# alexrozanski/llama.swift

Hardware: AMD Instinct MI355X
Metric: decode tokens/sec LLaMA-7B Q4_0 @1 GPU; % HBM-roofline on Q4_0 GEMV (higher is better)
Workload: dtype q4_0 x q4_0 -> int32 block sums, fp32 scales/accumulate; 1 GPU; LLaMA-7B Q4_0 single-token decode, greedy, n_ctx 512: `value` = 94 timed tokens at context positions 13 .. 106 (after 8 prompt + 5 warm-up tokens); BASELINE.json configs[1] proper -- the generation to the end of the 512-token context -- is config.full_context_tokens_per_s / roofline.full_context_* of bench.py --full; n_threads_semantics=8, parallelism=1 GPU

## Files before the change

llama.swift_amd/csrc/decode.hip:

```cpp
#define LH_DEFINE_PHASE_PROBE 1
#include <cmath>

#include "kcommon.hip.h"

namespace lh {

#ifndef LH_GEMV_SADDR
#define LH_GEMV_SADDR 0
#endif
#ifndef LH_GEMV_PAD
#define LH_GEMV_PAD 1
#endif

__device__ __forceinline__ float poll_tagged(const uint64_t *p, uint32_t tag, uint32_t *fault, bool short_fuse ) {
    uint64_t v;
    int spins = 0;
    for (;;) {
        v = __hip_atomic_load(p, __ATOMIC_RELAXED, __HIP_MEMORY_SCOPE_AGENT);
        if ((uint32_t) (v >> 32) == tag) break;
        __builtin_amdgcn_s_sleep(1);
        if (poll_give_up(spins, short_fuse ? (1 << 8) : (1 << 20), fault)) break;
    }
    return __builtin_bit_cast(float, (uint32_t) v);
}
__device__ __forceinline__ void store_tagged(uint64_t *p, float v, uint32_t tag) {
    __hip_atomic_store(p, (uint64_t) __builtin_bit_cast(uint32_t, v) | ((uint64_t) tag << 32), __ATOMIC_RELAXED, __HIP_MEMORY_SCOPE_WORKGROUP);
}


struct GemvArgs {
    const uint8_t *wt; int ngroups, nchunks, M, gmapF8;
    const uint32_t *qa_A; const float *qa_d;
    const float *in0, *in1; int K;
    float *y; const float *resid;
    const uint16_t *T_silu;
    uint32_t *out_A; float *out_d;
    const f64x2 *part_in; int npart; f64x2 *part_out;
    uint32_t *sync; int sync_blocks, sync_epoch;
    int lut_math;
    uint32_t *fault;
    const uint64_t *in_t;   int slot_in;
    const uint64_t *resid_t; int slot_resid;
    uint64_t *out_t;        int slot_out;
    const int32_t *pos_w;
    PickIO pick;
    int patience;
};
template <int PRE, int EPI, int D, bool RING, int PG>
__device__ __forceinline__ void gemv_body(const GemvArgs &ga, const int blk, const int nw, double *smem_d) {
    const uint8_t *__restrict__ wt = ga.wt;
    const int ngroups = ga.ngroups, nchunks = ga.nchunks, M = ga.M, gmapF8 = ga.gmapF8, K = ga.K, npart = ga.npart;
    const uint32_t *__restrict__ qa_A = ga.qa_A; const float *__restrict__ qa_d = ga.qa_d;
    const float *__restrict__ in0 = ga.in0; const float *__restrict__ in1 = ga.in1;
    float *__restrict__ y = ga.y; const float *__restrict__ resid = ga.resid;
    const uint16_t *__restrict__ T_silu = ga.T_silu;
    uint32_t *__restrict__ out_A = ga.out_A; float *__restrict__ out_d = ga.out_d;
    const f64x2 *__restrict__ part_in = ga.part_in; f64x2 *__restrict__ part_out = ga.part_out;
    constexpr bool TAGGED = (EPI == EPI_STORE_TAG || PRE == PREP_NORM_TAG || EPI == EPI_RESID_TAG || EPI == EPI_SILU_QAH);
    const uint32_t epoch_ = TAGGED ? __builtin_nontemporal_load(ga.sync) : 0u;
    const uint32_t store_tag = make_tag(epoch_, ga.sync_epoch + 1);
    const uint32_t mb_epoch_ = ((PRE == PREP_NORM_TAG || EPI == EPI_RESID_TAG) && ga.pos_w) ? (uint32_t) __builtin_nontemporal_load(ga.pos_w) + 1u : epoch_;
    const uint32_t tag_in = make_tag(mb_epoch_, ga.slot_in), tag_resid = make_tag(mb_epoch_, ga.slot_resid), tag_out = make_tag(mb_epoch_, ga.slot_out);
    uint32_t *ldsA = (uint32_t *) smem_d;
    constexpr int PADC = (LH_GEMV_PAD && RING) ? D : 0;
    float *ldsD = (float *) (ldsA + (nchunks + PADC) * 64);
    const int tid = threadIdx.x, lane = tid & 63, wave = LH_GEMV_SADDR ? __builtin_amdgcn_readfirstlane(tid >> 6) : (tid >> 6);
    constexpr bool active = true;
    const int qah_block = (blk >> 4) * 8 + (blk & 7), qah_half = (blk >> 3) & 1;
    const int g = EPI == EPI_SILU_QAH ? qah_block * 8 + (wave >> 1) * 4 + qah_half * 2 + (wave & 1) : blk * nw + wave;
    const bool valid = active && g < ngroups;
    const uint8_t *wbase = wt + (size_t) (valid ? g : 0) * (nchunks + 1) * TILE_BYTES;
    const uint32_t voff_w = (uint32_t) lane * 16u, voff_s = 1024u + (uint32_t) ((lane >> 3) * 8 + (lane & 3) * 2) * 4u;
    uint32_t vw_ = voff_w, vs_ = voff_s;
#define LH_OPAQUE_OFFSETS() { vw_ = voff_w; vs_ = voff_s; asm volatile("" : "+v"(vw_), "+v"(vs_)); }
#if LH_PHASE_PROBE == 3
    unsigned long long probe_t[5] = { 0, 0, 0, 0, 0 };
    const unsigned long long probe_wall = wall_clock64();
#elif LH_PHASE_PROBE
    unsigned long long *probe_e = nullptr;
    if (g_phase_probe && blk == (int) gridDim.x / 2 && threadIdx.x == 0) {
        unsigned long long *pb = g_phase_probe;
        const unsigned long long slot = atomicAdd(pb, 1ull);
        if (slot < pb[1]) { probe_e = pb + 8 * (1 + slot); probe_e[5] = ngroups; probe_e[6] = nchunks; probe_e[7] = PRE * 16 + EPI; }
    }
#endif
    LH_STAMP(0);

    u32x4 wq[D];
    f32x2 ws[D];
#define LH_LOADW(SLOT, CH)                                                                                   \
    {                                                                                                        \
        const int ch_ = min((CH), nchunks);         \
        const uint8_t *tp_ = wbase + (size_t) ch_ * TILE_BYTES;                                              \
        if (LH_GEMV_SADDR) {                                                                                 \
            wq[SLOT] = __builtin_nontemporal_load((const u32x4 *) (tp_ + (size_t) vw_));                     \
            ws[SLOT] = __builtin_nontemporal_load((const f32x2 *) (tp_ + (size_t) vs_));                     \
        } else {                                                                                             \
            wq[SLOT] = __builtin_nontemporal_load((const u32x4 *) (tp_ + lane * 16));                        \
            ws[SLOT] = __builtin_nontemporal_load((const f32x2 *) (tp_ + 1024 + ((lane >> 3) * 8 + (lane & 3) * 2) * 4)); \
        }                                                                                                    \
    }
    constexpr bool NORMTAG = (PRE == PREP_NORM_TAG);
    constexpr bool NORMLIKE = (PRE == PREP_NORM || PRE == PREP_NORMP || NORMTAG);
    constexpr bool REGPRE = (PRE == PRE_QA || NORMLIKE || PRE == PREP_PLAIN);
    constexpr int MAXH = (NORMLIKE || PRE == PREP_PLAIN) ? PG : 1;
    constexpr int MAXQA = (PRE == PRE_QA) ? PG : 1, MAXQD = (PG + 7) / 8;
    f32x4 xa[MAXH][4], xb[MAXH][4];
    u32x4 qg[MAXQA], qh[MAXQD];
    const int nt = nw * 64;
    const int nh = K >> 4;
    constexpr int PNP = (PRE == PREP_NORMP) ? 8 : 1;
    f64x2 pp[PNP];
    const int npl = (npart + 63) >> 6;
    float resid_v = 0.0f;
    uint64_t resid_g = 0;
    auto phase1 = [&]() {
    if ((NORMLIKE || PRE == PREP_PLAIN) && active) {
        const int ng = (nh + nt - 1) / nt;
#pragma unroll
        for (int u = 0; u < MAXH; u++) {
            if (u < ng && (tid & ~63) + u * nt < nh) {
                const int hi = min(tid + u * nt, nh - 1);
#pragma unroll
                for (int v = 0; v < 4; v++) {
                    if (!NORMTAG) xa[u][v] = ((const f32x4 *) in0)[hi * 4 + v];
                    if (NORMLIKE) xb[u][v] = ((const f32x4 *) in1)[hi * 4 + v];
                }
            } else {
#pragma unroll
                for (int v = 0; v < 4; v++) { xa[u][v] = f32x4{ 0.0f, 0.0f, 0.0f, 0.0f }; xb[u][v] = f32x4{ 0.0f, 0.0f, 0.0f, 0.0f }; }
            }
        }
        if (PRE == PREP_NORMP && wave == 0) {
#pragma unroll
            for (int u = 0; u < PNP; u++) if (u < npl) pp[u] = part_in[min(lane + u * 64, npart - 1)];
        }
    }
    if ((EPI == EPI_RESID || (EPI == EPI_RESID_TAG && !ga.resid_t)) && active) {
        int lg0 = g;
        if (gmapF8) { const int b8 = g >> 3, w8 = g & 7; lg0 = w8 < 4 ? b8 * 4 + w8 : gmapF8 + b8 * 4 + (w8 - 4); }
        resid_v = resid[min(lg0 * 8 + (lane >> 3), M - 1)];
    }
    if (EPI == EPI_RESID_TAG && ga.resid_t && active && (lane & 7) == 0) {
        int lg0 = g;
        if (gmapF8) { const int b8 = g >> 3, w8 = g & 7; lg0 = w8 < 4 ? b8 * 4 + w8 : gmapF8 + b8 * 4 + (w8 - 4); }
        resid_g = load_granule_sys(ga.resid_t + min(lg0 * 8 + (lane >> 3), M - 1));
    }
    if (PRE == PRE_QA && active) {
        const int nqa = (nchunks * 16 + nt - 1) / nt, nqd = (nchunks * 2 + nt - 1) / nt;
#pragma unroll
        for (int u = 0; u < MAXQA; u++) if (u < nqa) qg[u] = ((const u32x4 *) qa_A)[min(tid + u * nt, nchunks * 16 - 1)];
#pragma unroll
        for (int u = 0; u < MAXQD; u++) if (u < nqd) qh[u] = ((const u32x4 *) qa_d)[min(tid + u * nt, nchunks * 2 - 1)];
    }
    };
    phase1();
    __builtin_amdgcn_sched_barrier(0);
    if (active) {
#pragma unroll
        for (int i = 0; i < D; i++) LH_LOADW(i, i)
    }
    __builtin_amdgcn_sched_barrier(0);

    if (NORMTAG) {
        const uint64_t *__restrict__ xt = ga.in_t;
        const int give_up = (ga.lut_math & 0x1000) ? (1 << 8) : ((1 << 20) << ga.patience);
        if (wave == 0) {
            int spins = 0;
            for (;;) {
                bool ok = true;
                if (lane < LH_WATCH) ok = (uint32_t) (load_granule_sys(xt + ((2 * lane + 1) * K / (2 * LH_WATCH))) >> 32) == tag_in;
                if (__all(ok)) break;
                __builtin_amdgcn_s_sleep(8);
                if (++spins > (give_up >> 2) || ((spins & 255) == 0 && __hip_atomic_load(ga.fault, __ATOMIC_RELAXED, __HIP_MEMORY_SCOPE_SYSTEM) != 0u)) break;
            }
        }
        __syncthreads();
#pragma unroll
        for (int u = 0; u < MAXH; u++) {
            const int hi = tid + u * nt;
            if (active && hi < nh) {
                uint64_t gv[16];
                int spins = 0;
                for (;;) {
                    bool ok = true;
#pragma unroll
                    for (int i = 0; i < 16; i++) {
                        gv[i] = load_granule_sys(xt + hi * 16 + i);
                        ok = ok && (uint32_t) (gv[i] >> 32) == tag_in;
                    }
                    if (ok) break;
                    __builtin_amdgcn_s_sleep(1);
                    if (poll_give_up(spins, give_up, ga.fault)) break;
                }
#pragma unroll
                for (int v = 0; v < 4; v++)
                    xa[u][v] = f32x4{ __builtin_bit_cast(float, (uint32_t) gv[4 * v]), __builtin_bit_cast(float, (uint32_t) gv[4 * v + 1]),
                                      __builtin_bit_cast(float, (uint32_t) gv[4 * v + 2]), __builtin_bit_cast(float, (uint32_t) gv[4 * v + 3]) };
            } else {
#pragma unroll
                for (int v = 0; v < 4; v++) xa[u][v] = f32x4{ 0.0f, 0.0f, 0.0f, 0.0f };
            }
        }
    }

    LH_STAMP(1);
    double *red = (double *) (ldsD + (nchunks + PADC) * 8);
    for (int i = active ? tid : PADC * 72; i < PADC * 72; i += nt) {
        if (i < PADC * 64) ldsA[nchunks * 64 + i] = 0u;
        else ldsD[nchunks * 8 + (i - PADC * 64)] = 0.0f;
    }
    if (PRE == PRE_QA) {
#pragma unroll
        for (int u = 0; u < MAXQA; u++) { const int gi = tid + u * nt; if (active && gi < nchunks * 16) ((u32x4 *) ldsA)[gi] = qg[u]; }
#pragma unroll
        for (int u = 0; u < MAXQD; u++) { const int gi = tid + u * nt; if (active && gi < nchunks * 2) ((u32x4 *) ldsD)[gi] = qh[u]; }
        __syncthreads();
    } else if (REGPRE) {
        if (NORMLIKE) {
            double S1 = 0.0, S2 = 0.0;
            if (PRE == PREP_NORMP) {
                if (wave == 0) {
#pragma unroll
                    for (int u = 0; u < PNP; u++)
                        if (u < npl && lane + u * 64 < npart) { S1 += pp[u].x; S2 += pp[u].y; }
                    S1 = wave_sum_d(S1);
                    S2 = wave_sum_d(S2);
                    if (lane == 0) { red[0] = S1; red[1] = S2; }
                }
                __syncthreads();
                S1 = red[0]; S2 = red[1];
            } else {
#pragma unroll
                for (int u = 0; u < MAXH; u++)
                    if (active && tid + u * nt < nh) {
#pragma unroll
                        for (int v = 0; v < 4; v++) {
                            const double x0 = (double) xa[u][v].x, x1 = (double) xa[u][v].y, x2 = (double) xa[u][v].z, x3 = (double) xa[u][v].w;
                            S1 += x0; S1 += x1; S1 += x2; S1 += x3;
                            S2 = __builtin_fma(x0, x0, S2); S2 = __builtin_fma(x1, x1, S2); S2 = __builtin_fma(x2, x2, S2); S2 = __builtin_fma(x3, x3, S2);
                        }
                    }
                block_sum_d2(S1, S2, red, 0);
            }
            const double mean = S1 / (double) K;
            double sum2 = __builtin_fma(-mean, S1, S2);
            const bool fast = npart >= 0 && mean * S1 <= 0.25 * S2;
            LH_STAMP2(2);
            double s2 = 0.0;
#pragma unroll
            for (int u = 0; u < MAXH; u++)
                if (active && tid + u * nt < nh) {
#pragma unroll
                    for (int v = 0; v < 4; v++) {
                        const double v0 = (double) xa[u][v].x - mean, v1 = (double) xa[u][v].y - mean;
                        const double v2 = (double) xa[u][v].z - mean, v3 = (double) xa[u][v].w - mean;
                        xa[u][v].x = (float) v0; xa[u][v].y = (float) v1; xa[u][v].z = (float) v2; xa[u][v].w = (float) v3;
                        if (!fast) { s2 += v0 * v0; s2 += v1 * v1; s2 += v2 * v2; s2 += v3 * v3; }
                    }
                }
            if (!fast) sum2 = block_sum_d(s2, red, 1);
            const float scale = (float) (1.0 / sqrt(sum2 / (double) K + (double) 1e-5f));
            LH_STAMP2(3);
#pragma unroll
            for (int u = 0; u < MAXH; u++)
#pragma unroll
                for (int v = 0; v < 4; v++) {
                    xa[u][v].x = xb[u][v].x * (xa[u][v].x * scale); xa[u][v].y = xb[u][v].y * (xa[u][v].y * scale);
                    xa[u][v].z = xb[u][v].z * (xa[u][v].z * scale); xa[u][v].w = xb[u][v].w * (xa[u][v].w * scale);
                }
        }
        const int nbp = nchunks * 8;
#pragma unroll
        for (int u = 0; u < MAXH; u++) {
            const int hi = tid + u * nt;
            const bool live = active && hi < nh;
            float amax = 0.0f;
            if (live) {
#pragma unroll
                for (int v = 0; v < 4; v++)
                    amax = fmaxf(fmaxf(fmaxf(amax, fabsf(xa[u][v].x)), fabsf(xa[u][v].y)), fmaxf(fabsf(xa[u][v].z), fabsf(xa[u][v].w)));
            }
            amax = fmaxf(amax, dpp_f<DPP_QUAD_XOR1>(amax));
            const float dd = amax / 7.0f;
            const float id = (amax != 0.0f) ? 7.0f / amax : 0.0f;
            uint32_t pr[8];
#pragma unroll
            for (int v = 0; v < 4; v++) {
                const uint32_t n0 = (uint32_t) ((int) __builtin_rintf(xa[u][v].x * id)) & 0xF, n1 = (uint32_t) ((int) __builtin_rintf(xa[u][v].y * id)) & 0xF;
                const uint32_t n2 = (uint32_t) ((int) __builtin_rintf(xa[u][v].z * id)) & 0xF, n3 = (uint32_t) ((int) __builtin_rintf(xa[u][v].w * id)) & 0xF;
                pr[2 * v] = n0 | (n1 << 8);
                pr[2 * v + 1] = n2 | (n3 << 8);
            }
            const int half = hi & 1, b = hi >> 1, c = b >> 3, j = b & 7;
#pragma unroll
            for (int k = 0; k < 8; k++) {
                const uint32_t other = (uint32_t) __builtin_amdgcn_mov_dpp((int) pr[k], DPP_QUAD_XOR1, 0xF, 0xF, true);
                const uint32_t dw = (half ? (other | (pr[k] << 16)) : (pr[k] | (other << 16))) << (4 * (j & 1));
                if (live && (k >> 2) == half) ldsA[(c * 8 + k) * 8 + j] = dw;
            }
            if (live && half == 0) ldsD[b] = dd;
        }
        for (int b = active ? K / 32 + tid : nbp; b < nbp; b += nt) {
            const int c = b >> 3, j = b & 7;
#pragma unroll
            for (int k = 0; k < 8; k++) ldsA[(c * 8 + k) * 8 + j] = 0;
            ldsD[b] = 0.0f;
        }
        __syncthreads();
    } else {
        float *ybuf = (float *) (red + 32);
        make_y<PRE>(ybuf, red, in0, in1, K, T_silu);
        quantize_y(ybuf, K, nchunks * 256, ldsA, ldsD, nullptr);
        __syncthreads();
    }

    const int k = lane & 7;
    float acc = 0.0f;
    static_assert(D % 2 == 0, "the two-entry LDS operand buffer alternates by slot parity: ring depth must be even");
    u32x4 la0[2], la1[2];
    float ldl[2], ldh[2];
    const int tq = lane & 3;
#define LH_LDSLOAD(BUF, CH)                                                                        \
    {                                                                                              \
        const int cl_ = PADC ? (CH) : min((CH), nchunks - 1);                                      \
        const u32x4 *pa = (const u32x4 *) (ldsA + (cl_ * 8 + k) * 8);                              \
        la0[BUF] = pa[0]; la1[BUF] = pa[1];                                                        \
        ldl[BUF] = ldsD[cl_ * 8 + tq]; ldh[BUF] = ldsD[cl_ * 8 + 4 + tq];                          \
    }
#define LH_CONSUME(SLOT, CH)                                                                       \
    {                                                                                              \
        const u32x4 w = wq[SLOT];                                                                  \
        const f32x2 sw = ws[SLOT];                                                                 \
        const u32x4 a0 = la0[(SLOT) & 1], a1 = la1[(SLOT) & 1];                                    \
        const float plo_ = sw.x * ldl[(SLOT) & 1], phi_ = sw.y * ldh[(SLOT) & 1];                  \
        LH_LDSLOAD(((SLOT) + 1) & 1, (CH) + 1)                                                     \
         \
         \
         \
         \
        const int i0_ = __builtin_amdgcn_sdot8((int) w.x, (int) a0.x, 0x4B400000, true);           \
        const int i1_ = __builtin_amdgcn_sdot8((int) w.x, (int) a0.y, 0x4B400000, true);           \
        const int i2_ = __builtin_amdgcn_sdot8((int) w.y, (int) a0.z, 0x4B400000, true);           \
        const int i3_ = __builtin_amdgcn_sdot8((int) w.y, (int) a0.w, 0x4B400000, true);           \
        const int i4_ = __builtin_amdgcn_sdot8((int) w.z, (int) a1.x, 0x4B400000, true);           \
        const int i5_ = __builtin_amdgcn_sdot8((int) w.z, (int) a1.y, 0x4B400000, true);           \
        const int i6_ = __builtin_amdgcn_sdot8((int) w.w, (int) a1.z, 0x4B400000, true);           \
        const int i7_ = __builtin_amdgcn_sdot8((int) w.w, (int) a1.w, 0x4B400000, true);           \
        const f32x2 mg_ = { 12582912.0f, 12582912.0f };                                            \
        const f32x2 q01_ = f32x2{ __builtin_bit_cast(float, i0_), __builtin_bit_cast(float, i1_) } - mg_; \
        const f32x2 q23_ = f32x2{ __builtin_bit_cast(float, i2_), __builtin_bit_cast(float, i3_) } - mg_; \
        const f32x2 q45_ = f32x2{ __builtin_bit_cast(float, i4_), __builtin_bit_cast(float, i5_) } - mg_; \
        const f32x2 q67_ = f32x2{ __builtin_bit_cast(float, i6_), __builtin_bit_cast(float, i7_) } - mg_; \
        LH_FMAC8_DPP(acc, plo_, phi_, q01_, q23_, q45_, q67_);                                     \
    }
    LH_STAMP(2);
    LH_STAMP2(4);
    if (active) {
    LH_LDSLOAD(0, 0)
    int c0 = 0;
    if (RING) {
        do {
            if (LH_GEMV_SADDR) LH_OPAQUE_OFFSETS()
#pragma unroll
            for (int i = 0; i < D; i++) {
                LH_CONSUME(i, c0 + i)
                LH_LOADW(i, c0 + D + i)
                __builtin_amdgcn_sched_barrier(0);
            }
            c0 += D;
        } while (c0 + D < nchunks);
    }
#pragma unroll
    for (int i = 0; i < D; i++) {
        LH_CONSUME(i, c0 + i)
        __builtin_amdgcn_sched_barrier(0);
    }
    }
#undef LH_LDSLOAD
#undef LH_CONSUME
#undef LH_LOADW
#undef LH_OPAQUE_OFFSETS

    LH_STAMP(3);
    acc = fold8(acc);
    int lg = g;
    if (gmapF8) { const int b8 = g >> 3, w8 = g & 7; lg = w8 < 4 ? b8 * 4 + w8 : gmapF8 + b8 * 4 + (w8 - 4); }
    const int m = lg * 8 + (lane >> 3);
    if (EPI == EPI_SILU_QAH) {
        float *gu = (float *) red;
        __syncthreads();
        if (k == 0) gu[wave * 8 + (lane >> 3)] = acc;
        __syncthreads();
        if (wave == 0 && valid) {
            const int i = lane & 15;
            const uint16_t gh = f2h_bits(gu[i]);
            const float act = h2f_bits((ga.lut_math & 1) ? silu_math_bits(gh) : T_silu[gh]) * gu[16 + i];
            float amax = wave_max_f(lane < 16 ? fabsf(act) : 0.0f);
            uint64_t *at = (uint64_t *) ga.out_t;
            const int hb = qah_block * 2 + qah_half;
            float other = 0.0f;
            if (lane == 0) {
                store_tagged(at + hb, amax, store_tag ^ ((ga.lut_math & 0x1000) ? 1u : 0u));
                other = poll_tagged(at + (hb ^ 1), store_tag, ga.fault, (ga.lut_math & 0x1000) != 0);
            }
            other = __builtin_bit_cast(float, __builtin_amdgcn_readfirstlane(__builtin_bit_cast(int, other)));
            amax = fmaxf(amax, other);
            const float dd = amax / 7.0f;
            const float id = (amax != 0.0f) ? 7.0f / amax : 0.0f;
            const uint32_t nib = (uint32_t) ((int) __builtin_rintf(act * id)) & 0xF;
            const int kk = lane & 7;
            const uint32_t e0 = __shfl(nib, 2 * kk), e1 = __shfl(nib, 2 * kk + 1);
            const int b = qah_block, c = b >> 3, j = b & 7;
            if (lane < 8) ((uint16_t *) (out_A + (c * 8 + kk) * 8 + j))[qah_half] = (uint16_t) ((e0 | (e1 << 8)) << (4 * (j & 1)));
            if (lane == 0 && qah_half == 0) out_d[b] = dd;
        }
    } else
    if (EPI == EPI_SILU_QA) {
        float *gu = (float *) red;
        __syncthreads();
        if (k == 0) gu[wave * 8 + (lane >> 3)] = acc;
        __syncthreads();
        if (wave == 0) {
            const int i = lane & 31;
            const uint16_t gh = f2h_bits(gu[i]);
            const float act = h2f_bits((ga.lut_math & 1) ? silu_math_bits(gh) : T_silu[gh]) * gu[32 + i];
            float amax = fabsf(act);
            amax = max_lanes_0_31(amax);
            const float dd = amax / 7.0f;
            const float id = (amax != 0.0f) ? 7.0f / amax : 0.0f;
            const uint32_t nib = ((uint32_t) ((int) __builtin_rintf(act * id) + 8) - 8) & 0xF;
            const int kk = lane & 7;
            const uint32_t e0 = __shfl(nib, 2 * kk), e1 = __shfl(nib, 2 * kk + 1);
            const uint32_t e2 = __shfl(nib, 16 + 2 * kk), e3 = __shfl(nib, 17 + 2 * kk);
            const int b = blk, c = b >> 3, j = b & 7;
            const uint32_t dw = (e0 | (e1 << 8) | (e2 << 16) | (e3 << 24)) << (4 * (j & 1));
            {
                if (lane < 8) out_A[(c * 8 + kk) * 8 + j] = dw;
                if (lane == 0) out_d[b] = dd;
            }
            if (y && lane < 32) y[b * 32 + i] = act;
        }
    } else {
        const bool live = valid && k == 0 && m < M;
        if (EPI == EPI_RESID) acc = acc + resid_v;
        if (EPI == EPI_RESID_TAG) {
            float rv = resid_v;
            if (ga.resid_t) {
                rv = __builtin_bit_cast(float, (uint32_t) resid_g);
                if (live && (uint32_t) (resid_g >> 32) != tag_resid) {
                    int spins = 0;
                    uint64_t gq;
                    for (;;) {
                        gq = load_granule_sys(ga.resid_t + m);
                        if ((uint32_t) (gq >> 32) == tag_resid) break;
                        __builtin_amdgcn_s_sleep(4);
                        if (poll_give_up(spins, (ga.lut_math & 0x1000) ? (1 << 8) : ((1 << 20) << ga.patience), ga.fault)) break;
                    }
                    rv = __builtin_bit_cast(float, (uint32_t) gq);
                }
            }
            acc = acc + rv;
        }
        if (EPI == EPI_STORE_PICK) {
            if (live) y[m] = acc;
            unsigned long long key = 0ull;
            if (live && acc == acc) {
                const uint32_t b = __builtin_bit_cast(uint32_t, acc == 0.0f ? 0.0f : acc);
                const uint32_t ob = (b & 0x80000000u) ? ~b : (b | 0x80000000u);
                key = ((unsigned long long) ob << 32) | (unsigned long long) (0xFFFFFFFFu - (uint32_t) m);
            }
#pragma unroll
            for (int o = 32; o >= 1; o >>= 1) {
                const uint32_t lo_ = (uint32_t) __shfl_xor((int) (uint32_t) key, o), hi_ = (uint32_t) __shfl_xor((int) (uint32_t) (key >> 32), o);
                const unsigned long long ok = ((unsigned long long) hi_ << 32) | lo_;
                key = ok > key ? ok : key;
            }
            unsigned long long *wk = (unsigned long long *) red;
            __syncthreads();
            if (lane == 0) wk[wave] = key;
            __syncthreads();
            if (tid == 0) {
                unsigned long long k2 = wk[0];
                for (int w2_ = 1; w2_ < nw; w2_++) k2 = wk[w2_] > k2 ? wk[w2_] : k2;
                __hip_atomic_store(ga.pick.key + blk, k2, __ATOMIC_RELAXED, __HIP_MEMORY_SCOPE_AGENT);
                asm volatile("s_waitcnt vmcnt(0)" ::: "memory");
                const int nwg = (int) gridDim.x, shard = blk & 7, nsh = (nwg + 7 - shard) / 8, ntop = nwg < 8 ? nwg : 8;
                int lastwg = 0;
                if (atomicAdd(ga.pick.count + shard * 16, 1u) == (uint32_t) (nsh - 1))
                    lastwg = atomicAdd(ga.pick.count + 128, 1u) == (uint32_t) (ntop - 1);
                wk[15] = (unsigned long long) lastwg;
            }
            __syncthreads();
            if (wk[15] != 0ull) {
                unsigned long long best = 0ull;
                for (int i = tid; i < (int) gridDim.x; i += nw * 64) {
                    const unsigned long long kv = __hip_atomic_load(ga.pick.key + i, __ATOMIC_RELAXED, __HIP_MEMORY_SCOPE_AGENT);
                    best = kv > best ? kv : best;
                }
#pragma unroll
                for (int o = 32; o >= 1; o >>= 1) {
                    const uint32_t lo_ = (uint32_t) __shfl_xor((int) (uint32_t) best, o), hi_ = (uint32_t) __shfl_xor((int) (uint32_t) (best >> 32), o);
                    const unsigned long long ok = ((unsigned long long) hi_ << 32) | lo_;
                    best = ok > best ? ok : best;
                }
                __syncthreads();
                if (lane == 0) wk[wave] = best;
                __syncthreads();
                if (tid == 0) {
                    unsigned long long fin = wk[0];
                    for (int w2_ = 1; w2_ < nw; w2_++) fin = wk[w2_] > fin ? wk[w2_] : fin;
                    const int r = (fin >> 32) == 0ull ? 0 : (int) (0xFFFFFFFFu - (uint32_t) fin);
                    int32_t *st = ga.pick.state;
                    ga.pick.out[st[1]] = r;
                    if (ga.pick.next_token) *ga.pick.next_token = r;
                    st[0] += 1; st[1] += 1;
                    for (int sh = 0; sh < 8; sh++) __hip_atomic_store(ga.pick.count + sh * 16, 0u, __ATOMIC_RELAXED, __HIP_MEMORY_SCOPE_AGENT);
                    __hip_atomic_store(ga.pick.count + 128, 0u, __ATOMIC_RELAXED, __HIP_MEMORY_SCOPE_AGENT);
                    wk[14] = (unsigned long long) (r < ga.pick.n_vocab ? r : 0);
                }
                __syncthreads();
            }
            if (wk[15] != 0ull && ga.pick.emb) {
                const int tok = (int) wk[14];
                const int dE = K;
                __syncthreads();
                const uint8_t *row = ga.pick.emb + (size_t) tok * (dE / 32) * 20;
                double s1 = 0.0, s2 = 0.0;
                for (int i = tid; i < dE / 2; i += nw * 64) {
                    const int b = i >> 4, j = i & 15;
                    const uint8_t *blk_ = row + b * 20;
                    const uint32_t bits = blk_[0] | (blk_[1] << 8) | (blk_[2] << 16) | ((uint32_t) blk_[3] << 24);
                    const float dd = __builtin_bit_cast(float, bits);
                    const uint32_t q = blk_[4 + j];
                    const float v0 = (float) ((int) (q & 0xF) - 8) * dd, v1 = (float) ((int) (q >> 4) - 8) * dd;
                    ga.pick.x_next[2 * i + 0] = v0;
                    ga.pick.x_next[2 * i + 1] = v1;
                    s1 += (double) v0; s1 += (double) v1;
                    s2 += (double) v0 * (double) v0; s2 += (double) v1 * (double) v1;
                }
                s1 = block_sum_d(s1, red, 0);
                s2 = block_sum_d(s2, red, 1);
                if (tid == 0) {
                    ((f64x2 *) ga.pick.part_next)[0] = f64x2{ s1, s2 };
                    if (ga.pick.epoch) ga.pick.epoch[0] = next_epoch(ga.pick.epoch[0]);
                }
            }
        } else
        if (EPI == EPI_STORE_TAG) {
            if (live) store_tagged((uint64_t *) y + m, acc, store_tag ^ ((ga.lut_math & 0x1000) ? 1u : 0u));
        } else if (EPI == EPI_RESID_TAG) {
            if (live) {
                if (ga.out_t) store_tagged_sys(ga.out_t + m, __builtin_bit_cast(uint32_t, acc), tag_out ^ ((ga.lut_math & 0x2000) ? 1u : 0u));
                if (y) y[m] = acc;
            }
        } else
        if (live) y[m] = acc;
        if ((EPI == EPI_RESID || EPI == EPI_RESID_TAG) && part_out) {
            const double yd = live ? (double) acc : 0.0;
            const double s1 = wave_sum_d(yd), s2 = wave_sum_d(yd * yd);
            if (nw == 1) {
                if (lane == 0) part_out[blk] = f64x2{ s1, s2 };
            } else {
                if (lane == 0) { red[2 * wave] = s1; red[2 * wave + 1] = s2; }
                __syncthreads();
                if (tid == 0) {
                    double t1 = red[0], t2 = red[1];
                    for (int w2_ = 1; w2_ < nw; w2_++) { t1 += red[2 * w2_]; t2 += red[2 * w2_ + 1]; }
                    part_out[blk] = f64x2{ t1, t2 };
                }
            }
        }
    }
    LH_STAMP(4);
#if LH_PHASE_PROBE == 3
    if (g_phase_probe && threadIdx.x == 0) {
        unsigned long long *pb = g_phase_probe;
        const unsigned long long slot = atomicAdd(pb, 1ull);
        if (slot < pb[1]) {
            unsigned long long *e = pb + 8 * (1 + slot);
            for (int i = 0; i < 5; i++) e[i] = probe_t[i];
            e[5] = ((unsigned long long) (PRE * 16 + EPI) << 48) | ((unsigned long long) nchunks << 32) | (unsigned) blk;
            e[6] = wall_clock64();
            e[7] = probe_wall;
        }
    }
#endif
}


template <int PRE, int EPI, int D, bool RING, int PG>
__global__ void __launch_bounds__(EPI == EPI_SILU_QA ? 512 : 256, EPI == EPI_SILU_QA ? 4 : 1)
k_gemv(const GemvArgs ga) {
    extern __shared__ double smem_d[];
    gemv_body<PRE, EPI, D, RING, PG>(ga, blockIdx.x, blockDim.x >> 6, smem_d);
}


constexpr int DEC_TS = 32;

__global__ void __launch_bounds__(256)
k_dec_scores(const float *__restrict__ qkv, int d, int dh, const double *__restrict__ sincos_tab,
             float *__restrict__ Kc, float *__restrict__ Vc, float *__restrict__ sc, int n_ctx,
             float kq_scale, const int32_t *__restrict__ st) {
    extern __shared__ double smem_d[];
    float *qs = (float *) smem_d;
    float *kn = qs + dh;
    const int h = blockIdx.x;
#if LH_PHASE_PROBE == 3
    const unsigned long long probe_wall = wall_clock64(), probe_t0 = __builtin_readcyclecounter();
    unsigned long long probe_t1 = 0, probe_t2 = 0;
#endif
    const int n_past = st[0];
    const int t0 = blockIdx.y * DEC_TS;
    if (t0 > n_past) return;
    const int tid = threadIdx.x;
    const bool owns_new = n_past < t0 + DEC_TS;
    const double *tab = sincos_tab + (size_t) n_past * dh;
    const float *q = qkv + h * dh, *kk = qkv + d + h * dh, *vv = qkv + 2 * d + h * dh;
    const bool rot = tid < dh / 2;
    const int e = rot ? 2 * tid : 0;
    const double cs = tab[e], sn = tab[e + 1];
    const float q0 = q[e], q1 = q[e + 1];
    const float kr0 = kk[e], kr1 = kk[e + 1], vr0 = vv[e], vr1 = vv[e + 1];
    const int hw = tid >> 5, l = tid & 31;
    constexpr int KPH = DEC_TS / 8;
    const int tb = t0 + hw * KPH;
    float kv[KPH][8];
#pragma unroll
    for (int u = 0; u < KPH; u++) {
        const int t = min(tb + u, n_past);
        const float *kr = Kc + (size_t) t * d + h * dh;
#pragma unroll
        for (int i = 0; i < 8; i++) kv[u][i] = (i * 32 < dh) ? kr[min(i * 32, dh - 32) + l] : 0.0f;
    }
    if (rot) {
        const double x0 = (double) q0, x1 = (double) q1;
        qs[e] = (float) (x0 * cs - x1 * sn);
        qs[e + 1] = (float) (x0 * sn + x1 * cs);
        if (owns_new) {
            const double k0 = (double) kr0, k1 = (double) kr1;
            const float r0 = (float) (k0 * cs - k1 * sn), r1 = (float) (k0 * sn + k1 * cs);
            kn[e] = r0; kn[e + 1] = r1;
            Kc[(size_t) n_past * d + h * dh + e] = r0;
            Kc[(size_t) n_past * d + h * dh + e + 1] = r1;
            Vc[(size_t) n_past * d + h * dh + e] = vr0;
            Vc[(size_t) n_past * d + h * dh + e + 1] = vr1;
        }
    }
    __syncthreads();
#if LH_PHASE_PROBE == 3
    probe_t1 = __builtin_readcyclecounter();
#endif
#pragma unroll
    for (int u = 0; u < KPH; u++) {
        const int t = tb + u;
        float s = 0.0f;
#pragma unroll
        for (int i = 0; i < 8; i++) {
            if (i * 32 < dh) {
                const float kval = (t == n_past) ? kn[i * 32 + l] : kv[u][i];
                s = fmaf(kval, qs[i * 32 + l], s);
            }
        }
        s = tree32_to_lane0(s);
        if (l == 0 && t <= n_past) sc[(size_t) h * n_ctx + t] = s * kq_scale;
    }
#if LH_PHASE_PROBE == 3
    probe_t2 = __builtin_readcyclecounter();
    if (g_phase_probe && tid == 0) {
        unsigned long long *pb = g_phase_probe; const unsigned long long slot = atomicAdd(pb, 1ull);
        if (slot < pb[1]) { unsigned long long *e = pb + 8 * (1 + slot); e[0] = probe_t0; e[1] = probe_t1; e[2] = probe_t2; e[3] = e[4] = probe_t2;
            e[5] = (0xB2ull << 48) | ((unsigned long long) blockIdx.y << 32) | (unsigned) h; e[6] = wall_clock64(); e[7] = probe_wall; }
    }
#endif
}

__global__ void __launch_bounds__(256)
k_decn_scores(const float *__restrict__ qr, int d, int dh, const float *__restrict__ Kc, float *__restrict__ sc,
              int n_ctx, float kq_scale, int n_past, const SeqSet *__restrict__ set) {
    const int h = blockIdx.x, n = blockIdx.z, H = gridDim.x;
    const int np = set ? set->state[n][0] : n_past + n;
    if (set) Kc += set->kv_off[n];
    const int t0 = blockIdx.y * DEC_TS;
    if (t0 > np) return;
    const int tid = threadIdx.x, hw = tid >> 5, l = tid & 31;
    constexpr int KPH = DEC_TS / 8;
    const int tb = t0 + hw * KPH;
    const float *q = qr + (size_t) n * d + h * dh;
    float qv[8], kv[KPH][8];
#pragma unroll
    for (int i = 0; i < 8; i++) qv[i] = (i * 32 < dh) ? q[min(i * 32, dh - 32) + l] : 0.0f;
#pragma unroll
    for (int u = 0; u < KPH; u++) {
        const float *kr = Kc + (size_t) min(tb + u, np) * d + h * dh;
#pragma unroll
        for (int i = 0; i < 8; i++) kv[u][i] = (i * 32 < dh) ? kr[min(i * 32, dh - 32) + l] : 0.0f;
    }
#pragma unroll
    for (int u = 0; u < KPH; u++) {
        const int t = tb + u;
        float s = 0.0f;
#pragma unroll
        for (int i = 0; i < 8; i++)
            if (i * 32 < dh) s = fmaf(kv[u][i], qv[i], s);
        s = tree32_to_lane0(s);
        if (l == 0 && t <= np) sc[((size_t) n * H + h) * n_ctx + t] = s * kq_scale;
    }
}

template <bool MULTI>
__global__ void __launch_bounds__(1024)
k_dec_pv_blk(const float *__restrict__ sc, const float *__restrict__ Vc, int d, int dh, int n_ctx, int nth,
             float *__restrict__ merged, uint32_t *__restrict__ qa_A, float *__restrict__ qa_d,
             const uint16_t *__restrict__ T_exp, const int32_t *__restrict__ st,
             int n_past0, long qa_strideA, long qa_strideD, int lut_math, int chunk, const SeqSet *__restrict__ set, long m_stride) {
    extern __shared__ double smem_d[];
    double *red = smem_d;
    float *p = (float *) (smem_d + 32);
    float *part = p + n_ctx;
    const int h = blockIdx.x, cb = blockIdx.y, tid = threadIdx.x, nt = blockDim.x;
    const int n_past = MULTI ? (set ? set->state[blockIdx.z][0] : n_past0 + (int) blockIdx.z) : st[0];
    if (MULTI && set) Vc += set->kv_off[blockIdx.z];
    const int T = n_past + 1;
    const float *row = sc + (size_t) h * n_ctx;
    if (MULTI) {
        const int n = blockIdx.z;
        row = sc + ((size_t) n * gridDim.x + h) * n_ctx;
        if (merged) merged += (size_t) n * m_stride;
        qa_A += (size_t) n * qa_strideA;
        qa_d += (size_t) n * qa_strideD;
        if (h == (int) gridDim.x - 1 && cb == (int) gridDim.y - 1)
            for (int pb = d / 32 + tid; pb < (int) qa_strideD; pb += nt) {
                const int pc = pb >> 3, pj = pb & 7;
#pragma unroll
                for (int kk = 0; kk < 8; kk++) qa_A[(pc * 8 + kk) * 8 + pj] = 0;
                qa_d[pb] = 0.0f;
            }
    }
    pv_soft_max(row, p, T, tid, nt, red, T_exp, lut_math);
    const int Tpv = (MULTI && !set) ? (chunk > 0 ? n_past0 + min((int) gridDim.z, ((int) blockIdx.z / chunk + 1) * chunk) : n_past0 + (int) gridDim.z) : T;
    if (MULTI && !set)
        for (int t = T + tid; t < Tpv; t += nt) p[t] = 0.0f;
    __syncthreads();

    const int c = tid & 31, sub = tid >> 5, nsub = nt >> 5;
    const int dc = (Tpv + nth - 1) / nth;
    const int col = h * dh + cb * 32 + c;
    const float *vcol = Vc + col;
    for (int th = sub; th < nth; th += nsub) {
        const int t0 = dc * th, t1 = min(t0 + dc, Tpv);
        float acc = 0.0f;
        float va[16], vb[16];
#pragma unroll
        for (int u = 0; u < 16; u++) va[u] = vcol[(size_t) min(t0 + u, t1 - 1) * d];
        for (int tb = t0; tb < t1; tb += 32) {
#pragma unroll
            for (int u = 0; u < 16; u++) vb[u] = vcol[(size_t) min(tb + 16 + u, t1 - 1) * d];
#pragma unroll
            for (int u = 0; u < 16; u++) {
                const float pe = (tb + u < t1) ? p[min(tb + u, Tpv - 1)] : 0.0f;
                acc = fmaf(va[u], pe, acc);
            }
#pragma unroll
            for (int u = 0; u < 16; u++) va[u] = vcol[(size_t) min(tb + 32 + u, t1 - 1) * d];
#pragma unroll
            for (int u = 0; u < 16; u++) {
                const float pe = (tb + 16 + u < t1) ? p[min(tb + 16 + u, Tpv - 1)] : 0.0f;
                acc = fmaf(vb[u], pe, acc);
            }
        }
        part[th * 32 + c] = acc;
    }
    __syncthreads();
    pv_store_block(part, nth, tid, col, h, dh, cb, merged, qa_A, qa_d);
}

template <int NL>
__global__ void __launch_bounds__(1024)
k_dec_pv_stream(const float *__restrict__ sc, const float *__restrict__ Vc, int d, int dh, int n_ctx, int nth, int SR,
                float *__restrict__ merged, uint32_t *__restrict__ qa_A, float *__restrict__ qa_d,
                const uint16_t *__restrict__ T_exp, const int32_t *__restrict__ st, int lut_math,
                int H, int split, uint64_t *__restrict__ xpart, const uint32_t *__restrict__ epoch, int layer, uint32_t *__restrict__ fault) {
    typedef float f32x4 __attribute__((ext_vector_type(4)));
    extern __shared__ double smem_d[];
    double *red = smem_d;
    float *p = (float *) (smem_d + 32);
    float *part = p + ((n_ctx + 3) & ~3);
    f32x4 *stage = (f32x4 *) (part + nth * 32);
    const int tid = threadIdx.x;
#if LH_PHASE_PROBE == 3
    unsigned long long probe_t[10] = { 0, 0, 0, 0, 0, 0, 0, 0, 0, 0 };
    const unsigned long long probe_wall = wall_clock64();
#define LH_PSTAMP(IDX) do { probe_t[IDX] = __builtin_readcyclecounter(); } while (0)
#define LH_PFLUSH() do { if (g_phase_probe && tid == 0) { unsigned long long *pb = g_phase_probe; const unsigned long long wall_ = wall_clock64(); \
        for (int half_ = 0; half_ < 2; half_++) { const unsigned long long slot = atomicAdd(pb, 1ull); \
        if (slot < pb[1]) { unsigned long long *e = pb + 8 * (1 + slot); for (int i = 0; i < 5; i++) e[i] = probe_t[5 * half_ + i]; \
            e[5] = ((unsigned long long) (0xB0 + half_) << 48) | ((unsigned long long) z << 32) | (unsigned) base; e[6] = wall_; e[7] = probe_wall; } } } } while (0)
#else
#define LH_PSTAMP(IDX) do { } while (0)
#define LH_PFLUSH() do { } while (0)
#endif
    const int bid = blockIdx.x, z = (bid >> 3) % split, base = (bid / (8 * split)) * 8 + (bid & 7);
    const int h = base % H, cb = base / H;
    const int cpw = (nth + split - 1) / split, th_lo = z * cpw, nloc = min(nth, th_lo + cpw) - th_lo;
    LH_PSTAMP(0);
    const int T = st[0] + 1;
    const int dc = (T + nth - 1) / nth;
    const int nstage = (dc + SR - 1) / SR;
    const int col0 = h * dh + cb * 32;
    const int stage_quads = nloc * SR * 8;
    constexpr int PV_ROW = 4;
    const float *row = sc + (size_t) h * n_ctx;
    float rv[PV_ROW];
#pragma unroll
    for (int i = 0; i < PV_ROW; i++) rv[i] = row[min(i * 1024 + tid, T - 1)];
    auto fetch = [&](int sidx, f32x4 (&v)[NL]) {
#pragma unroll
        for (int i = 0; i < NL; i++) {
            const int e = min(i * 1024 + tid, stage_quads - 1);
            const int r = e >> 3, q = e & 7;
            const int lc = r / SR, u = r - lc * SR, th = th_lo + lc;
            const int t = min(min(dc * th + sidx * SR + u, dc * th + dc - 1), T - 1);
            v[i] = __builtin_nontemporal_load((const f32x4 *) (Vc + (size_t) t * d + col0 + q * 4));
        }
    };
    auto put = [&](int buf, const f32x4 (&v)[NL]) {
#pragma unroll
        for (int i = 0; i < NL; i++) {
            const int e = i * 1024 + tid;
            if (e < stage_quads) stage[(size_t) buf * stage_quads + e] = v[i];
        }
    };
    f32x4 va[NL], vb[NL];
    {
        float mx = -INFINITY;
#pragma unroll
        for (int i = 0; i < PV_ROW; i++) if (i * 1024 + tid < T) mx = fmaxf(mx, rv[i]);
        mx = block_max_f(mx, red, 0);
        LH_PSTAMP(1);
        fetch(0, va);
        if (nstage > 1) fetch(1, vb);
        double sum = 0.0;
#pragma unroll
        for (int i = 0; i < PV_ROW; i++) {
            if (i * 1024 + tid < T) {
                const uint16_t xh = f2h_bits(rv[i] - mx);
                rv[i] = h2f_bits((lut_math & 2) ? exp_math_bits(xh) : T_exp[xh]);
                sum += (double) rv[i];
            }
        }
        sum = block_sum_d(sum, red, 1);
        const float inv = (float) (1.0 / sum);
#pragma unroll
        for (int i = 0; i < PV_ROW; i++) if (i * 1024 + tid < T) p[i * 1024 + tid] = rv[i] * inv;
    }
    LH_PSTAMP(2);
    const int lc = tid >> 5, c = tid & 31, th = th_lo + lc;
    const bool owner = lc < nloc;
    const int t0 = dc * th, t1 = min(t0 + dc, T);
    float acc = 0.0f;
    auto consume = [&](int sidx, int buf) {
        if (!owner) return;
        const float *vs = (const float *) (stage + (size_t) buf * stage_quads) + (size_t) lc * SR * 32 + c;
        const int tb = t0 + sidx * SR, n = min(SR, t1 - tb);
        int u = 0;
        for (; u + 16 <= n; u += 16) {
            float v[16], w[16];
#pragma unroll
            for (int k = 0; k < 16; k++) { v[k] = vs[(u + k) * 32]; w[k] = p[tb + u + k]; }
#pragma unroll
            for (int k = 0; k < 16; k++) acc = fmaf(v[k], w[k], acc);
        }
        for (; u < n; u++) acc = fmaf(vs[u * 32], p[tb + u], acc);
    };
    for (int sidx = 0; sidx < nstage; sidx += 2) {
        put(0, va);
        __syncthreads();
        if (sidx == 0) LH_PSTAMP(3); else if (sidx == 2) LH_PSTAMP(7);
        if (sidx + 2 < nstage) fetch(sidx + 2, va);
        consume(sidx, 0);
        if (sidx == 0) LH_PSTAMP(4);
        if (sidx + 1 < nstage) {
            put(1, vb);
            __syncthreads();
            if (sidx == 0) LH_PSTAMP(5);
            if (sidx + 3 < nstage) fetch(sidx + 3, vb);
            consume(sidx + 1, 1);
            if (sidx == 0) LH_PSTAMP(6);
        }
    }
    LH_PSTAMP(8);
    if (z + 1 < split) {
        if (owner) store_tagged(xpart + ((size_t) base * nth + th) * 32 + c, acc, make_tag(epoch[0], layer + 1) ^ ((lut_math & 0x1000) ? 1u : 0u));
        LH_PSTAMP(9);
        LH_PFLUSH();
        return;
    }
    if (owner) part[th * 32 + c] = acc;
    if (split > 1 && tid < th_lo * 32)
        part[tid] = poll_tagged(xpart + (size_t) base * nth * 32 + tid, make_tag(epoch[0], layer + 1), fault, (lut_math & 0x1000) != 0);
    __syncthreads();
    pv_store_block(part, nth, tid, col0 + tid, h, dh, cb, merged, qa_A, qa_d);
    LH_PSTAMP(9);
    LH_PFLUSH();
}
#undef LH_PSTAMP
#undef LH_PFLUSH

#ifndef LH_PVD_ABLATE
#define LH_PVD_ABLATE 0
#endif
constexpr int PVD_SR = 8;
template <int N> __device__ __forceinline__ void pvd_wait_vmcnt() { asm volatile("s_waitcnt vmcnt(%0)" :: "n"(N) : "memory"); }
__device__ __forceinline__ void pvd_barrier() {
    asm volatile("s_waitcnt lgkmcnt(0)\n\ts_barrier" ::: "memory");
}
__device__ __forceinline__ void pvd_worker_barrier(uint32_t *ctr, uint32_t &round, int lane, uint32_t *fault) {
    round += 6;
    if (lane == 0) __hip_atomic_fetch_add(ctr, 1u, __ATOMIC_RELEASE, __HIP_MEMORY_SCOPE_WORKGROUP);
    int spins = 0;
    while (__hip_atomic_load(ctr, __ATOMIC_ACQUIRE, __HIP_MEMORY_SCOPE_WORKGROUP) < round) { __builtin_amdgcn_s_sleep(0); if (poll_give_up(spins, 1 << 24, fault)) break; }
}
__global__ void __launch_bounds__(512)
k_dec_pv_dma(const float *__restrict__ sc, const float *__restrict__ Vc, int d, int n_ctx, int nth, int NS,
             float *__restrict__ merged, uint32_t *__restrict__ qa_A, float *__restrict__ qa_d,
             const uint16_t *__restrict__ T_exp, const int32_t *__restrict__ st, int lut_math,
             int H, int split, uint64_t *__restrict__ xpart, const uint32_t *__restrict__ epoch, int layer, uint32_t *__restrict__ fault) {
    constexpr int dh = 128;
    extern __shared__ double smem_d[];
    double *red = smem_d;
    float *p = (float *) (smem_d + 32);
    float *part = p + ((n_ctx + 3) & ~3);
    uint32_t *flags = (uint32_t *) (part + nth * dh);
    float *ring = (float *) (flags + 16);
    const int tid = threadIdx.x, lane = tid & 63, wave = __builtin_amdgcn_readfirstlane(tid >> 6);
    const int bid = blockIdx.x, z = (bid >> 3) % split, h = (bid / (8 * split)) * 8 + (bid & 7);
    const int cpw = (nth + split - 1) / split, th_lo = z * cpw, nloc = min(nth, th_lo + cpw) - th_lo;
    const int T = st[0] + 1;
    const int dc = (T + nth - 1) / nth;
    const int nstage = (dc + PVD_SR - 1) / PVD_SR;
    const int col0 = h * dh;
    const int ncw = 2 * nloc;
    const int limit = (lut_math & 0x1000) ? (1 << 8) : (1 << 22);
    if (tid < 16) flags[tid] = 0u;
    constexpr int PV_ROW = 11, NWT = 384;
    const float *row = sc + (size_t) h * n_ctx;
    float rv[PV_ROW];
    const int wt = tid - 128;
    float mx = -INFINITY;
    if (wave > 1) {
#pragma unroll
        for (int i = 0; i < PV_ROW; i++) rv[i] = row[min(i * NWT + wt, T - 1)];
#pragma unroll
        for (int i = 0; i < PV_ROW; i++) if (i * NWT + wt < T) mx = fmaxf(mx, rv[i]);
        mx = wave_max_f(mx);
        if (lane == 0) ((float *) red)[wave] = mx;
    }
    pvd_barrier();
    if (wave < 2) {
        const uint32_t ring_lds = (uint32_t) (uintptr_t) (__attribute__((address_space(3))) float *) ring;
        const uint64_t vbase = (uint64_t) (uintptr_t) (Vc + col0);
        const int u = lane >> 5, q = lane & 31;
        uint32_t off[3];
#pragma unroll
        for (int j = 0; j < 3; j++) off[j] = (uint32_t) ((size_t) min(dc * (th_lo + min(j, nloc - 1)) + 2 * wave + u, n_ctx - 1) * d * 4 + q * 16);
        const uint32_t step = (uint32_t) ((size_t) PVD_SR * d * 4), four = (uint32_t) ((size_t) 4 * d * 4);
        const uint32_t off_max = (uint32_t) ((size_t) (n_ctx - 1) * d * 4 + q * 16);
        uint32_t pub = 0;
        int slot = 0;
        auto min_done = [&]() { uint32_t m = 0xffffffffu; for (int w = 0; w < ncw; w++) m = min(m, __hip_atomic_load(flags + 2 + w, __ATOMIC_ACQUIRE, __HIP_MEMORY_SCOPE_WORKGROUP)); return m; };
        const int F = 60 / (2 * nloc);
        for (int s = 0; s < nstage; s++) {
            if (s >= NS && min_done() < (uint32_t) (s - NS + 1)) {
                pvd_wait_vmcnt<0>();
                if ((uint32_t) s > pub) { pub = (uint32_t) s; __hip_atomic_store(flags + wave, pub, __ATOMIC_RELEASE, __HIP_MEMORY_SCOPE_WORKGROUP); }
                int spins = 0;
                while (min_done() < (uint32_t) (s - NS + 1)) { __builtin_amdgcn_s_sleep(1); if (poll_give_up(spins, limit, fault)) break; }
            }
            const bool tail = (s + 2) * PVD_SR + dc * nth > n_ctx;
#pragma unroll
            for (int j = 0; j < 3; j++) {
                if (j < nloc) {
#pragma unroll
                    for (int i = 0; i < 2; i++) {
                        const uint32_t o = off[j] + (i ? four : 0u);
                        const uint32_t voff = tail ? min(o, off_max) : o;
                        const uint32_t dst = ring_lds + (uint32_t) ((slot * nloc + j) * 4096 + (wave + 2 * i) * 1024);
                        uint32_t keep;
                        asm volatile("s_mov_b32 %0, m0\n\ts_mov_b32 m0, %2\n\ts_nop 0\n\tglobal_load_lds_dwordx4 %1, %3 nt\n\ts_mov_b32 m0, %0"
                                     : "=&s"(keep) : "v"(voff), "s"(dst), "s"(vbase) : "memory");
                    }
                    off[j] += step;
                }
            }
            slot = slot + 1 == NS ? 0 : slot + 1;
            if (s + 1 > F) {
                if (nloc == 1) pvd_wait_vmcnt<60>(); else if (nloc == 2) pvd_wait_vmcnt<60>(); else pvd_wait_vmcnt<60>();
                if ((uint32_t) (s + 1 - F) > pub) { pub = (uint32_t) (s + 1 - F); __hip_atomic_store(flags + wave, pub, __ATOMIC_RELEASE, __HIP_MEMORY_SCOPE_WORKGROUP); }
            }
        }
        pvd_wait_vmcnt<0>();
        __hip_atomic_store(flags + wave, (uint32_t) nstage, __ATOMIC_RELEASE, __HIP_MEMORY_SCOPE_WORKGROUP);
        return;
    }
    uint32_t wround = 0;
    {
        float m2 = ((float *) red)[2];
        for (int w = 3; w < 8; w++) m2 = fmaxf(m2, ((float *) red)[w]);
        double sum = 0.0;
#pragma unroll
        for (int i = 0; i < PV_ROW; i++) {
#if LH_PVD_ABLATE == 1
            if (i * NWT + wt < T && (i * NWT + wt < dc * th_lo || i * NWT + wt >= dc * (th_lo + nloc))) rv[i] = 0.0f; else
#endif
            if (i * NWT + wt < T) {
                const uint16_t xh = f2h_bits(rv[i] - m2);
                rv[i] = h2f_bits((lut_math & 2) ? exp_math_bits(xh) : T_exp[xh]);
                sum += (double) rv[i];
            }
        }
        sum = wave_sum_d(sum);
        if (lane == 0) red[8 + wave] = sum;
    }
    pvd_worker_barrier(flags + 8, wround, lane, fault);
    float acc = 0.0f;
    const int lc = (tid - 128) >> 7, c = (tid - 128) & 127, th = th_lo + lc;
    const bool owner = lc < nloc;
    {
        double tot = red[10];
        for (int w = 3; w < 8; w++) tot += red[8 + w];
        const float inv = (float) (1.0 / tot);
#pragma unroll
        for (int i = 0; i < PV_ROW; i++) if (i * NWT + wt < T) p[i * NWT + wt] = rv[i] * inv;
    }
    pvd_worker_barrier(flags + 8, wround, lane, fault);
    if (wave - 2 < ncw) {
        const int t0 = dc * th, t1 = min(t0 + dc, T);
        uint32_t landed_seen = 0;
        int slot = 0;
        for (int s = 0; s < nstage; s++) {
            if ((uint32_t) s >= landed_seen) {
                int spins = 0;
                for (;;) {
                    landed_seen = min(__hip_atomic_load(flags, __ATOMIC_ACQUIRE, __HIP_MEMORY_SCOPE_WORKGROUP), __hip_atomic_load(flags + 1, __ATOMIC_ACQUIRE, __HIP_MEMORY_SCOPE_WORKGROUP));
                    if (landed_seen > (uint32_t) s) break;
                    __builtin_amdgcn_s_sleep(1);
                    if (poll_give_up(spins, limit, fault)) break;
                }
            }
            {
                const float *vs = ring + (size_t) (slot * nloc + lc) * 1024 + c;
                const int tb = t0 + s * PVD_SR, n = min(PVD_SR, t1 - tb);
                if (n == PVD_SR) {
                    float v[PVD_SR], w[PVD_SR];
#pragma unroll
                    for (int k = 0; k < PVD_SR; k++) { v[k] = vs[k * dh]; w[k] = p[tb + k]; }
#pragma unroll
                    for (int k = 0; k < PVD_SR; k++) acc = fmaf(v[k], w[k], acc);
                } else {
                    for (int k = 0; k < n; k++) acc = fmaf(vs[k * dh], p[tb + k], acc);
                }
            }
            asm volatile("" ::: "memory");
            if (lane == 0) __hip_atomic_store(flags + wave, (uint32_t) (s + 1), __ATOMIC_RELEASE, __HIP_MEMORY_SCOPE_WORKGROUP);
            slot = slot + 1 == NS ? 0 : slot + 1;
        }
    }
    const uint32_t ptag = make_tag(epoch[0], layer + 1);
    if (z + 1 < split) {
        if (owner) store_tagged(xpart + ((size_t) h * nth + th) * dh + c, acc, ptag ^ ((lut_math & 0x1000) ? 1u : 0u));
        return;
    }
    if (owner) part[th * dh + c] = acc;
    for (int i = wt; i < th_lo * dh; i += NWT)
        part[i] = poll_tagged(xpart + (size_t) h * nth * dh + i, ptag, fault, (lut_math & 0x1000) != 0);
    pvd_worker_barrier(flags + 8, wround, lane, fault);
    if (wave >= 2 && wave < 6 && lane < 32) {
        const int cb = wave - 2, cc0 = cb * 32 + lane;
        float s_ = part[cc0];
        for (int t2 = 1; t2 < nth; t2++) s_ += part[t2 * dh + cc0];
        if (merged) merged[col0 + cc0] = s_;
        float amax = fabsf(s_);
        amax = max_lanes_0_31(amax);
        const float dd = amax / 7.0f;
        const float id = (amax != 0.0f) ? 7.0f / amax : 0.0f;
        const uint32_t nib = (uint32_t) ((int) __builtin_rintf(s_ * id)) & 0xF;
        const int kk = lane & 7;
        const uint32_t e0 = __shfl(nib, 2 * kk), e1 = __shfl(nib, 2 * kk + 1);
        const uint32_t e2 = __shfl(nib, 16 + 2 * kk), e3 = __shfl(nib, 17 + 2 * kk);
        const int b = h * (dh / 32) + cb, cc = b >> 3, j = b & 7;
        if (lane < 8) qa_A[(cc * 8 + kk) * 8 + j] = (e0 | (e1 << 8) | (e2 << 16) | (e3 << 24)) << (4 * (j & 1));
        if (lane == 0) qa_d[b] = dd;
    }
}

__device__ __forceinline__ float load_f32_sc1(const float *p) {
    return __builtin_bit_cast(float, __hip_atomic_load((const uint32_t *) p, __ATOMIC_RELAXED, __HIP_MEMORY_SCOPE_AGENT));
}

#ifndef LH_ATTN_ABLATE
#define LH_ATTN_ABLATE 0
#endif
struct AttnXArgs {
    const float *qkv; int d, dh; const double *sincos_tab; float *Kc, *Vc, *sc; int n_ctx, nth; float kq_scale;
    float *merged; uint32_t *qa_A; float *qa_d; const uint16_t *T_exp; const int32_t *st; uint32_t *sync, *fault; int lut_math;
    const uint64_t *qkv2; uint64_t *sc2; const uint32_t *epoch; int layer;
};
template <bool QKV_WAIT>
__device__ __forceinline__ void attn_x_body(const AttnXArgs &aa, const int h, const int yy, double *smem_d) {
    const float *__restrict__ qkv = aa.qkv; const int d = aa.d, dh = aa.dh; const double *__restrict__ sincos_tab = aa.sincos_tab;
    float *__restrict__ Kc = aa.Kc, *__restrict__ Vc = aa.Vc; float *sc = aa.sc; const int n_ctx = aa.n_ctx, nth = aa.nth; const float kq_scale = aa.kq_scale;
    float *__restrict__ merged = aa.merged; uint32_t *__restrict__ qa_A = aa.qa_A; float *__restrict__ qa_d = aa.qa_d;
    const uint16_t *__restrict__ T_exp = aa.T_exp; const int32_t *__restrict__ st = aa.st; uint32_t *sync = aa.sync, *fault = aa.fault; const int lut_math = aa.lut_math;
    const int ncb = dh / 32, tid = threadIdx.x;
#if LH_PHASE_PROBE == 3
    unsigned long long probe_t[5] = { 0, 0, 0, 0, 0 };
    const unsigned long long probe_wall = wall_clock64();
#define LH_ASTAMP(IDX) do { probe_t[IDX] = __builtin_readcyclecounter(); } while (0)
#define LH_AFLUSH(KIND) do { if (g_phase_probe && tid == 0) { unsigned long long *pb = g_phase_probe; const unsigned long long slot = atomicAdd(pb, 1ull); \
        if (slot < pb[1]) { unsigned long long *e = pb + 8 * (1 + slot); for (int i = 0; i < 5; i++) e[i] = probe_t[i]; \
            e[5] = ((unsigned long long) (KIND) << 48) | ((unsigned long long) yy << 32) | (unsigned) h; e[6] = wall_clock64(); e[7] = probe_wall; } } } while (0)
#else
#define LH_ASTAMP(IDX) do { } while (0)
#define LH_AFLUSH(KIND) do { } while (0)
#endif
    LH_ASTAMP(0);
    const int n_past = st[0];
    uint32_t *cnt = sync + h * 32;
    if (yy >= ncb) {
        const int t0 = (yy - ncb) * DEC_TS;
        if (t0 > n_past) return;
        float *qs = (float *) smem_d, *kn = qs + dh;
        const bool owns_new = n_past < t0 + DEC_TS;
        const double *tab = sincos_tab + (size_t) n_past * dh;
        const float *q = qkv + h * dh, *kk = qkv + d + h * dh, *vv = qkv + 2 * d + h * dh;
        const int hw = tid >> 5, l = tid & 31;
        constexpr int KPH = DEC_TS / 8;
        const int tb = t0 + hw * KPH;
        float kv[KPH][8];
        auto load_keys = [&]() {
#pragma unroll
            for (int u = 0; u < KPH; u++) {
                const int t = min(tb + u, n_past);
                const float *kr = Kc + (size_t) t * d + h * dh;
#pragma unroll
                for (int i = 0; i < 8; i++) kv[u][i] = (i * 32 < dh) ? kr[min(i * 32, dh - 32) + l] : 0.0f;
            }
        };
        const bool nowait = (lut_math & 0x1000) != 0;
        const uint32_t tag = QKV_WAIT ? (make_tag(aa.epoch[0], aa.layer + 1)) : 0u;
        if (QKV_WAIT) load_keys();
        if (tid < dh / 2) {
            const int e = 2 * tid;
            const double cs = tab[e], sn = tab[e + 1];
            const uint64_t *q2 = aa.qkv2 + h * dh, *k2 = q2 + d, *v2 = q2 + 2 * d;
            float gq0, gq1, gk0 = 0.0f, gk1 = 0.0f, gv0 = 0.0f, gv1 = 0.0f;
            if (QKV_WAIT) {
                uint64_t g_[6] = { 0, 0, 0, 0, 0, 0 };
                int spins = 0;
                for (;;) {
                    g_[0] = __hip_atomic_load(q2 + e, __ATOMIC_RELAXED, __HIP_MEMORY_SCOPE_AGENT);
                    g_[1] = __hip_atomic_load(q2 + e + 1, __ATOMIC_RELAXED, __HIP_MEMORY_SCOPE_AGENT);
                    if (owns_new) {
                        g_[2] = __hip_atomic_load(k2 + e, __ATOMIC_RELAXED, __HIP_MEMORY_SCOPE_AGENT);
                        g_[3] = __hip_atomic_load(k2 + e + 1, __ATOMIC_RELAXED, __HIP_MEMORY_SCOPE_AGENT);
                        g_[4] = __hip_atomic_load(v2 + e, __ATOMIC_RELAXED, __HIP_MEMORY_SCOPE_AGENT);
                        g_[5] = __hip_atomic_load(v2 + e + 1, __ATOMIC_RELAXED, __HIP_MEMORY_SCOPE_AGENT);
                    }
                    bool ok = (uint32_t) (g_[0] >> 32) == tag && (uint32_t) (g_[1] >> 32) == tag;
                    if (owns_new) ok = ok && (uint32_t) (g_[2] >> 32) == tag && (uint32_t) (g_[3] >> 32) == tag && (uint32_t) (g_[4] >> 32) == tag && (uint32_t) (g_[5] >> 32) == tag;
                    if (ok) break;
                    __builtin_amdgcn_s_sleep(1);
                    if (poll_give_up(spins, nowait ? (1 << 8) : (1 << 20), fault)) break;
                }
                gq0 = __builtin_bit_cast(float, (uint32_t) g_[0]); gq1 = __builtin_bit_cast(float, (uint32_t) g_[1]);
                gk0 = __builtin_bit_cast(float, (uint32_t) g_[2]); gk1 = __builtin_bit_cast(float, (uint32_t) g_[3]);
                gv0 = __builtin_bit_cast(float, (uint32_t) g_[4]); gv1 = __builtin_bit_cast(float, (uint32_t) g_[5]);
            } else {
                gq0 = q[e]; gq1 = q[e + 1];
                if (owns_new) { gk0 = kk[e]; gk1 = kk[e + 1]; gv0 = vv[e]; gv1 = vv[e + 1]; }
            }
            const double x0 = (double) gq0, x1 = (double) gq1;
            qs[e] = (float) (x0 * cs - x1 * sn);
            qs[e + 1] = (float) (x0 * sn + x1 * cs);
            if (owns_new) {
                const double k0 = (double) gk0, k1 = (double) gk1;
                const float r0 = (float) (k0 * cs - k1 * sn), r1 = (float) (k0 * sn + k1 * cs);
                kn[e] = r0; kn[e + 1] = r1;
                Kc[(size_t) n_past * d + h * dh + e] = r0;
                Kc[(size_t) n_past * d + h * dh + e + 1] = r1;
                Vc[(size_t) n_past * d + h * dh + e] = gv0;
                Vc[(size_t) n_past * d + h * dh + e + 1] = gv1;
                if (QKV_WAIT) asm volatile("s_waitcnt vmcnt(0)" ::: "memory");
            }
        }
        __syncthreads();
        LH_ASTAMP(1);
        if (!QKV_WAIT) load_keys();
#pragma unroll
        for (int u = 0; u < KPH; u++) {
            const int t = tb + u;
            float s = 0.0f;
#pragma unroll
            for (int i = 0; i < 8; i++) {
                if (i * 32 < dh) {
                    const float kval = (t == n_past) ? kn[i * 32 + l] : kv[u][i];
                    s = fmaf(kval, qs[i * 32 + l], s);
                }
            }
            s = tree32_to_lane0(s);
            if (l == 0 && t <= n_past) {
                if (QKV_WAIT) store_tagged(aa.sc2 + (size_t) h * n_ctx + t, s * kq_scale, tag);
                else sc[(size_t) h * n_ctx + t] = s * kq_scale;
            }
        }
        if (QKV_WAIT) { LH_ASTAMP(2); LH_ASTAMP(3); LH_ASTAMP(4); LH_AFLUSH(0xA0); return; }
        LH_ASTAMP(2);
        asm volatile("s_waitcnt vmcnt(0)" ::: "memory");
        __syncthreads();
        LH_ASTAMP(3);
        if (tid == 0) __hip_atomic_fetch_add(cnt, 1u, __ATOMIC_RELAXED, __HIP_MEMORY_SCOPE_WORKGROUP);
#if LH_PHASE_PROBE == 3
        asm volatile("s_waitcnt vmcnt(0)" ::: "memory");
#endif
        LH_ASTAMP(4);
        LH_AFLUSH(0xA0);
        return;
    }
    const int cb = yy, nt = 256;
    const int T = n_past + 1;
    const int c = tid & 31, sub = tid >> 5, nsub = nt >> 5;
    const int dc = (T + nth - 1) / nth;
    const int col = h * dh + cb * 32 + c;
    const float *vcol = Vc + col;
    const int ta0 = dc * sub, t10 = min(ta0 + dc, T);
    constexpr int VB = 16;
    const bool early = sub < nth && ta0 < t10 && min(ta0 + 2 * VB - 1, t10 - 1) < n_past;
    float va[VB], vb[VB];
    if (early) {
#pragma unroll
        for (int u = 0; u < VB; u++) va[u] = vcol[(size_t) min(ta0 + u, t10 - 1) * d];
#pragma unroll
        for (int u = 0; u < VB; u++) vb[u] = vcol[(size_t) min(ta0 + VB + u, t10 - 1) * d];
    }
    if (!QKV_WAIT) {
        if (tid == 0) {
            const uint32_t need = (uint32_t) (n_past / DEC_TS + 1);
            int spins = 0;
            while (__hip_atomic_load(cnt, __ATOMIC_RELAXED, __HIP_MEMORY_SCOPE_AGENT) < need) {
                __builtin_amdgcn_s_sleep(1);
                if (++spins > (1 << 20)) { __hip_atomic_store(fault, 1u, __ATOMIC_RELAXED, __HIP_MEMORY_SCOPE_SYSTEM); break; }
            }
        }
        __syncthreads();
    }
    LH_ASTAMP(1);
    double *red = smem_d;
    float *p = (float *) (smem_d + 32);
    float *part = p + n_ctx;
    const float *row = sc + (size_t) h * n_ctx;
    float mx = -INFINITY;
    if (QKV_WAIT) {
        const uint32_t tag = make_tag(aa.epoch[0], aa.layer + 1);
        const bool nowait = (lut_math & 0x1000) != 0;
#if LH_ATTN_ABLATE == 2
        for (int t0 = tid; t0 < T; t0 += nt) p[t0] = 0.0f;
        for (int t0 = T; t0 < T; t0 += 4 * nt) {
#else
        for (int t0 = tid; t0 < T; t0 += 4 * nt) {
#endif
            uint64_t g_[4] = { 0, 0, 0, 0 };
            int spins = 0;
            for (;;) {
                bool ok = true;
#pragma unroll
                for (int i = 0; i < 4; i++) {
                    const int t = t0 + i * nt;
                    if (t < T) { g_[i] = __hip_atomic_load(aa.sc2 + (size_t) h * n_ctx + t, __ATOMIC_RELAXED, __HIP_MEMORY_SCOPE_AGENT); ok = ok && (uint32_t) (g_[i] >> 32) == tag; }
                }
                if (ok) break;
                __builtin_amdgcn_s_sleep(1);
                if (poll_give_up(spins, nowait ? (1 << 8) : (1 << 20), fault)) break;
            }
#pragma unroll
            for (int i = 0; i < 4; i++) {
                const int t = t0 + i * nt;
                if (t < T) { const float v = __builtin_bit_cast(float, (uint32_t) g_[i]); p[t] = v; mx = fmaxf(mx, v); }
            }
        }
    } else
    for (int t = tid; t < T; t += nt) { const float v = load_f32_sc1(row + t); p[t] = v; mx = fmaxf(mx, v); }
#if LH_ATTN_ABLATE == 1 || LH_ATTN_ABLATE == 2
    if (!QKV_WAIT) {
#endif
    mx = block_max_f(mx, red, 0);
    double sum = 0.0;
    for (int t = tid; t < T; t += nt) {
        const uint16_t xh = f2h_bits(p[t] - mx);
        const float e = h2f_bits((lut_math & 2) ? exp_math_bits(xh) : T_exp[xh]);
        p[t] = e;
        sum += (double) e;
    }
    sum = block_sum_d(sum, red, 1);
    const float inv = (float) (1.0 / sum);
    for (int t = tid; t < T; t += nt) p[t] *= inv;
#if LH_ATTN_ABLATE == 1 || LH_ATTN_ABLATE == 2
    }
#endif
    __syncthreads();
    LH_ASTAMP(2);
    for (int th = sub; th < nth; th += nsub) {
        const int ta = dc * th, t1 = min(ta + dc, T);
        float acc = 0.0f;
        if (!(early && th == sub)) {
#pragma unroll
            for (int u = 0; u < VB; u++) va[u] = vcol[(size_t) min(ta + u, t1 - 1) * d];
#pragma unroll
            for (int u = 0; u < VB; u++) vb[u] = vcol[(size_t) min(ta + VB + u, t1 - 1) * d];
        }
        for (int tb = ta; tb < t1; tb += 2 * VB) {
#pragma unroll
            for (int u = 0; u < VB; u++) {
                const float pe = (tb + u < t1) ? p[min(tb + u, T - 1)] : 0.0f;
                acc = fmaf(va[u], pe, acc);
            }
#pragma unroll
            for (int u = 0; u < VB; u++) va[u] = vcol[(size_t) min(tb + 2 * VB + u, t1 - 1) * d];
#pragma unroll
            for (int u = 0; u < VB; u++) {
                const float pe = (tb + VB + u < t1) ? p[min(tb + VB + u, T - 1)] : 0.0f;
                acc = fmaf(vb[u], pe, acc);
            }
#pragma unroll
            for (int u = 0; u < VB; u++) vb[u] = vcol[(size_t) min(tb + 3 * VB + u, t1 - 1) * d];
        }
        part[th * 32 + c] = acc;
    }
    __syncthreads();
    LH_ASTAMP(3);
    if (tid < 32) {
        float s = part[tid];
        for (int th = 1; th < nth; th++) s += part[th * 32 + tid];
        if (merged) merged[col] = s;
        float amax = fabsf(s);
        amax = max_lanes_0_31(amax);
        const float dd = amax / 7.0f;
        const float id = (amax != 0.0f) ? 7.0f / amax : 0.0f;
        const uint32_t nib = (uint32_t) ((int) __builtin_rintf(s * id)) & 0xF;
        const int kk = tid & 7;
        const uint32_t e0 = __shfl(nib, 2 * kk), e1 = __shfl(nib, 2 * kk + 1);
        const uint32_t e2 = __shfl(nib, 16 + 2 * kk), e3 = __shfl(nib, 17 + 2 * kk);
        const int b = h * (dh / 32) + cb, cc = b >> 3, j = b & 7;
        const uint32_t dwq = (e0 | (e1 << 8) | (e2 << 16) | (e3 << 24)) << (4 * (j & 1));
        if (tid < 8) qa_A[(cc * 8 + kk) * 8 + j] = dwq;
        if (tid == 0) qa_d[b] = dd;
    }
    if (!QKV_WAIT && tid == 0) {
        const uint32_t done = __hip_atomic_fetch_add(cnt + 1, 1u, __ATOMIC_RELAXED, __HIP_MEMORY_SCOPE_WORKGROUP);
        if (done == (uint32_t) (ncb - 1)) {
            __hip_atomic_exchange(cnt, 0u, __ATOMIC_RELAXED, __HIP_MEMORY_SCOPE_WORKGROUP);
            __hip_atomic_exchange(cnt + 1, 0u, __ATOMIC_RELAXED, __HIP_MEMORY_SCOPE_WORKGROUP);
        }
    }
    LH_ASTAMP(4);
    LH_AFLUSH(0xA1);
}
#undef LH_ASTAMP
#undef LH_AFLUSH

__global__ void __launch_bounds__(256)
k_dec_attn_x(const AttnXArgs aa) {
    extern __shared__ double smem_d[];
    attn_x_body<false>(aa, blockIdx.x, blockIdx.y, smem_d);
}

template <int PRE, int D, int PG>
__global__ void __launch_bounds__(256) __attribute__((amdgpu_waves_per_eu(PRE == PREP_NORM ? (PG == 1 ? 3 : 2) : (PG == 1 ? 4 : 3))))
k_qkv_attn(const GemvArgs ga, const AttnXArgs aa, const int gridA, const int H) {
    extern __shared__ double smem_d[];
    const int b = blockIdx.x;
    if (b < gridA) {
        const int ncb = aa.dh / 32, wph = 3 * ncb;
        const int xcd = b & 7, slot = b >> 3, j = slot / wph, part = slot % wph, mat = part / ncb, sub = part % ncb;
        const int h = xcd + 8 * j;
        gemv_body<PRE, EPI_STORE_TAG, D, true, PG>(ga, mat * (aa.d / 32) + h * ncb + sub, 4, smem_d);
        return;
    }
    const int a = b - gridA, h = a % H, y = a / H;
    attn_x_body<true>(aa, h, y, smem_d);
}

__global__ void k_xcd_selftest(uint32_t *out) {
    if (threadIdx.x == 0) {
        uint32_t id;
        asm volatile("s_getreg_b32 %0, hwreg(HW_REG_XCC_ID)" : "=s"(id));
        out[blockIdx.x + gridDim.x * blockIdx.y] = id & 0xf;
    }
}

__device__ __forceinline__ void argmax_take(float &v, int &i, float ov, int oi) {
    if (ov > v || (ov == v && oi < i)) { v = ov; i = oi; }
}
template <int CTRL>
__device__ __forceinline__ void argmax_dpp(float &v, int &i) {
    const float ov = dpp_f<CTRL>(v);
    const int oi = __builtin_amdgcn_mov_dpp(i, CTRL, 0xF, 0xF, true);
    argmax_take(v, i, ov, oi);
}
__global__ void __launch_bounds__(1024)
k_argmax(const float *__restrict__ logits, int V, int32_t *__restrict__ out, int out_idx,
         int32_t *__restrict__ next_token, int32_t *__restrict__ st, uint64_t *token_mb) {
    __shared__ float bv[16];
    __shared__ int bi[16];
    const int tid = threadIdx.x, nt = blockDim.x;
    float best = -INFINITY;
    int idx = 0x7fffffff;
    for (int i0 = tid; i0 < V; i0 += 32 * nt) {
        float v[32];
#pragma unroll
        for (int u = 0; u < 32; u++) v[u] = logits[min(i0 + u * nt, V - 1)];
#pragma unroll
        for (int u = 0; u < 32; u++) {
            const int i = i0 + u * nt;
            if (i < V) argmax_take(best, idx, v[u], i);
        }
    }
    argmax_dpp<DPP_QUAD_XOR1>(best, idx);
    argmax_dpp<DPP_QUAD_XOR2>(best, idx);
    argmax_dpp<DPP_ROW_HALF_MIRROR>(best, idx);
    argmax_dpp<DPP_ROW_MIRROR>(best, idx);
    {
        const int vb = __builtin_bit_cast(int, best);
        float wv = __builtin_bit_cast(float, __builtin_amdgcn_readlane(vb, 0));
        int wi = __builtin_amdgcn_readlane(idx, 0);
        argmax_take(wv, wi, __builtin_bit_cast(float, __builtin_amdgcn_readlane(vb, 16)), __builtin_amdgcn_readlane(idx, 16));
        argmax_take(wv, wi, __builtin_bit_cast(float, __builtin_amdgcn_readlane(vb, 32)), __builtin_amdgcn_readlane(idx, 32));
        argmax_take(wv, wi, __builtin_bit_cast(float, __builtin_amdgcn_readlane(vb, 48)), __builtin_amdgcn_readlane(idx, 48));
        if ((tid & 63) == 0) { bv[tid >> 6] = wv; bi[tid >> 6] = wi; }
    }
    __syncthreads();
    if (tid == 0) {
        float v = bv[0];
        int i = bi[0];
        for (int w = 1; w < (nt >> 6); w++) argmax_take(v, i, bv[w], bi[w]);
        const int r = i == 0x7fffffff ? 0 : i;
        out[st ? st[1] : out_idx] = r;
        if (next_token) *next_token = r;
        if (token_mb && st) store_tagged_sys(token_mb, (uint32_t) r, make_tag((uint32_t) st[0] + 2u, 0));
        if (st) { st[0] += 1; st[1] += 1; }
    }
}

__device__ __forceinline__ unsigned long long dpp_max_u64(unsigned long long v, unsigned long long o) { return o > v ? o : v; }
template <int CTRL>
__device__ __forceinline__ unsigned long long dpp_u64(unsigned long long v) {
    const int lo = __builtin_amdgcn_mov_dpp((int) (uint32_t) v, CTRL, 0xF, 0xF, true);
    const int hi = __builtin_amdgcn_mov_dpp((int) (uint32_t) (v >> 32), CTRL, 0xF, 0xF, true);
    return ((unsigned long long) (uint32_t) hi << 32) | (uint32_t) lo;
}

__global__ void k_advance(int32_t *__restrict__ st) {
    if (threadIdx.x == 0) { st[0] += 1; st[1] += 1; }
}

__global__ void __launch_bounds__(1024)
k_argmax_set(const float *__restrict__ logits, int V, const SeqSet *__restrict__ set) {
    __shared__ float bv[16];
    __shared__ int bi[16];
    const int b = blockIdx.x, tid = threadIdx.x, nt = blockDim.x;
    logits += (size_t) b * V;
    float best = -INFINITY;
    int idx = 0x7fffffff;
    for (int i0 = tid; i0 < V; i0 += 32 * nt) {
        float v[32];
#pragma unroll
        for (int u = 0; u < 32; u++) v[u] = logits[min(i0 + u * nt, V - 1)];
#pragma unroll
        for (int u = 0; u < 32; u++) {
            const int i = i0 + u * nt;
            if (i < V) argmax_take(best, idx, v[u], i);
        }
    }
    argmax_dpp<DPP_QUAD_XOR1>(best, idx);
    argmax_dpp<DPP_QUAD_XOR2>(best, idx);
    argmax_dpp<DPP_ROW_HALF_MIRROR>(best, idx);
    argmax_dpp<DPP_ROW_MIRROR>(best, idx);
    {
        const int vb = __builtin_bit_cast(int, best);
        float wv = __builtin_bit_cast(float, __builtin_amdgcn_readlane(vb, 0));
        int wi = __builtin_amdgcn_readlane(idx, 0);
        argmax_take(wv, wi, __builtin_bit_cast(float, __builtin_amdgcn_readlane(vb, 16)), __builtin_amdgcn_readlane(idx, 16));
        argmax_take(wv, wi, __builtin_bit_cast(float, __builtin_amdgcn_readlane(vb, 32)), __builtin_amdgcn_readlane(idx, 32));
        argmax_take(wv, wi, __builtin_bit_cast(float, __builtin_amdgcn_readlane(vb, 48)), __builtin_amdgcn_readlane(idx, 48));
        if ((tid & 63) == 0) { bv[tid >> 6] = wv; bi[tid >> 6] = wi; }
    }
    __syncthreads();
    if (tid == 0) {
        float v = bv[0];
        int i = bi[0];
        for (int w = 1; w < (nt >> 6); w++) argmax_take(v, i, bv[w], bi[w]);
        const int r = i == 0x7fffffff ? 0 : i;
        int32_t *st = set->state[b];
        set->trace[b][st[1]] = r;
        if (set->tok_out[b]) *set->tok_out[b] = r;
        st[0] += 1; st[1] += 1;
    }
}
__global__ void k_advance_set(const SeqSet *__restrict__ set, int n) {
    const int b = threadIdx.x;
    if (b < n) { int32_t *st = set->state[b]; st[0] += 1; st[1] += 1; }
}

hipError_t set_phase_probe(unsigned long long *dev_buf) {
    return hipMemcpyToSymbol(HIP_SYMBOL(g_phase_probe), &dev_buf, sizeof(dev_buf));
}


static int pick_waves(int ngroups) {
    if (ngroups >= 4 * 512) return 4;
    if (ngroups >= 2 * 512) return 2;
    return 1;
}

static int pick_depth(int nchunks, int ngroups) {
    static const int very_shallow[] = { 4 }, shallow[] = { 10, 8 }, deep[] = { 10, 14, 16, 18, 22, 8 };
    const int *cand = ngroups >= 2048 ? very_shallow : ngroups >= 1024 ? shallow : deep;
    const int n = ngroups >= 2048 ? 1 : ngroups >= 1024 ? 2 : 6;
    int best = cand[0], best_waste = 1 << 30;
    for (int i = 0; i < n; i++) {
        const int d = cand[i];
        const int waste = (nchunks + d - 1) / d * d - nchunks;
        if (waste * 5 <= nchunks) return d;
        if (waste < best_waste) { best_waste = waste; best = d; }
    }
    return best;
}

GemvPlan gemv_plan(const QMat &w, int pre, int epi) {
    GemvPlan p = { 0, 0, 0, true, 0, 0 };
    const int need = pre == PRE_QA ? w.nchunks * 16 : w.K / 16;
    int nw = 0, pg = 0;
    if (epi == EPI_SILU_QA || epi == EPI_SILU_QAH) {
        if (!w.gmapF8 || w.ngroups % 8 != 0 || w.K / 16 > 512) return p;
        if (epi == EPI_SILU_QA) {
            if (pre == PRE_QA && need > 512) return p;
            nw = 8; pg = 1;
        } else {
            if (w.nchunks <= 4 || w.ngroups < 2048) return p;
            nw = 4; pg = need <= 256 ? 1 : 2;
        }
    } else if (pre == PRE_QA) {
        nw = w.ngroups >= 1024 ? 4 : w.ngroups >= 512 ? 2 : 1;
        while (!(pg = need <= 4 * nw * 64 ? 4 : need <= 12 * nw * 64 ? 12 : 0) && nw < 4) nw *= 2;
        if (!pg) return p;
    } else if (pre == PREP_SILU_MUL) {
        nw = pick_waves(w.ngroups); pg = 1;
    } else {
        nw = pick_waves(w.ngroups);
        while (nw < 4 && need > nw * 64) nw *= 2;
        pg = need <= nw * 64 ? 1 : need <= 2 * nw * 64 ? 2 : 0;
        if (!pg) return p;
    }
    p.ring = epi == EPI_SILU_QAH || w.nchunks > 16 || (w.nchunks == 16 && w.ngroups >= 1024);
    p.depth = p.ring ? pick_depth(w.nchunks, w.ngroups) : 16;
    if (epi == EPI_STORE_PICK && (nw != 4 || !p.ring || (p.depth != 4 && p.depth != 8 && p.depth != 10))) return p;
    p.grid = epi == EPI_SILU_QAH ? (w.ngroups / 8 + 7) / 8 * 16
                                 : (w.ngroups + nw - 1) / nw;
    p.lds = (size_t) w.nchunks * 64 * 4 + (size_t) w.nchunks * 8 * 4 + 32 * sizeof(double);
    if (pre == PREP_SILU_MUL) p.lds += prep_lds_bytes(w.K);
    p.lds = ((p.lds + 15) & ~(size_t) 15) + ((LH_GEMV_PAD && p.ring) ? (size_t) p.depth * 288 : 0);
    p.nw = nw; p.pg = pg;
    return p;
}

using GemvKernel = void (*)(const GemvArgs);
template <int PRE, int EPI, int PG>
static GemvKernel gemv_kernel_at(int depth, bool ring) {
    constexpr bool ALL = EPI != EPI_STORE_PICK && EPI != EPI_SILU_QAH;
    if (!ring) {
        if constexpr (ALL) if (depth == 16) return k_gemv<PRE, EPI, 16, false, PG>;
        return nullptr;
    }
    if (depth == 4) return k_gemv<PRE, EPI, 4, true, PG>;
    if constexpr (EPI != EPI_SILU_QAH) {
        if (depth == 8) return k_gemv<PRE, EPI, 8, true, PG>;
        if (depth == 10) return k_gemv<PRE, EPI, 10, true, PG>;
        if constexpr (ALL) {
            if (depth == 14) return k_gemv<PRE, EPI, 14, true, PG>;
            if (depth == 16) return k_gemv<PRE, EPI, 16, true, PG>;
            if (depth == 18) return k_gemv<PRE, EPI, 18, true, PG>;
            if (depth == 22) return k_gemv<PRE, EPI, 22, true, PG>;
        }
    }
    return nullptr;
}
template <int PRE, int EPI, int PG0, int PG1 = 0>
static GemvKernel gemv_kernel_pg(const GemvPlan &p) {
    if (p.pg == PG0) return gemv_kernel_at<PRE, EPI, PG0>(p.depth, p.ring);
    if constexpr (PG1 != 0) if (p.pg == PG1) return gemv_kernel_at<PRE, EPI, PG1>(p.depth, p.ring);
    return nullptr;
}
static GemvKernel gemv_kernel(int pre, int epi, const GemvPlan &p) {
    if (pre == PRE_QA && epi == EPI_STORE)             return gemv_kernel_pg<PRE_QA, EPI_STORE, 4, 12>(p);
    if (pre == PRE_QA && epi == EPI_RESID)             return gemv_kernel_pg<PRE_QA, EPI_RESID, 4, 12>(p);
    if (pre == PRE_QA && epi == EPI_RESID_TAG)         return gemv_kernel_pg<PRE_QA, EPI_RESID_TAG, 4, 12>(p);
    if (pre == PRE_QA && epi == EPI_SILU_QA)           return gemv_kernel_pg<PRE_QA, EPI_SILU_QA, 1>(p);
    if (pre == PREP_NORM && epi == EPI_STORE)          return gemv_kernel_pg<PREP_NORM, EPI_STORE, 1, 2>(p);
    if (pre == PREP_NORM && epi == EPI_SILU_QA)        return gemv_kernel_pg<PREP_NORM, EPI_SILU_QA, 1>(p);
    if (pre == PREP_NORM && epi == EPI_SILU_QAH)       return gemv_kernel_pg<PREP_NORM, EPI_SILU_QAH, 1, 2>(p);
    if (pre == PREP_NORM && epi == EPI_STORE_PICK)     return gemv_kernel_pg<PREP_NORM, EPI_STORE_PICK, 1, 2>(p);
    if (pre == PREP_NORMP && epi == EPI_STORE)         return gemv_kernel_pg<PREP_NORMP, EPI_STORE, 1, 2>(p);
    if (pre == PREP_NORMP && epi == EPI_SILU_QA)       return gemv_kernel_pg<PREP_NORMP, EPI_SILU_QA, 1>(p);
    if (pre == PREP_NORMP && epi == EPI_SILU_QAH)      return gemv_kernel_pg<PREP_NORMP, EPI_SILU_QAH, 1, 2>(p);
    if (pre == PREP_NORMP && epi == EPI_STORE_PICK)    return gemv_kernel_pg<PREP_NORMP, EPI_STORE_PICK, 1, 2>(p);
    if (pre == PREP_NORM_TAG && epi == EPI_STORE)      return gemv_kernel_pg<PREP_NORM_TAG, EPI_STORE, 1, 2>(p);
    if (pre == PREP_PLAIN && epi == EPI_RESID)         return gemv_kernel_pg<PREP_PLAIN, EPI_RESID, 1, 2>(p);
    if (pre == PREP_SILU_MUL && epi == EPI_RESID)      return gemv_kernel_pg<PREP_SILU_MUL, EPI_RESID, 1>(p);
    return nullptr;
}
bool gemv_plan_has_kernel(int pre, int epi, const GemvPlan &p) { return p.nw && gemv_kernel(pre, epi, p); }
int gemv_resid_parts(const QMat &w) { return gemv_plan(w, PRE_QA, EPI_RESID).grid; }

bool norm_mode_resolve(int *pre, NormPart *np) {
    static const int norm_mode = [] { const char *e = getenv("LLAMAHIP_NORM_MODE"); return e ? atoi(e) : 2; }();
    if (pre) {
        if (norm_mode < 2) *np = NormPart();
        if (*pre == PREP_NORM && np->in && np->n_in > 0 && np->n_in <= NORM_PART_MAX) *pre = PREP_NORMP;
        else { np->in = nullptr; np->n_in = norm_mode == 0 ? -1 : 0; }
    }
    return norm_mode >= 2;
}

static hipError_t launch_gemv_plan(const QMat &w, int pre, int epi, const NormPart *npp, const MailboxIO *mb, GemvArgs ga, hipStream_t st) {
    NormPart np = npp ? *npp : NormPart();
    norm_mode_resolve(&pre, &np);
    if (mb) {
        if (mb->in_t && (pre == PREP_NORM || pre == PREP_NORMP) && epi == EPI_STORE) pre = PREP_NORM_TAG;
        else if ((mb->resid_t || mb->out_t) && pre == PRE_QA && epi == EPI_RESID) epi = EPI_RESID_TAG;
        else return hipErrorInvalidValue;
        ga.in_t = mb->in_t; ga.resid_t = mb->resid_t; ga.out_t = mb->out_t;
        ga.pos_w = mb->pos_w; ga.patience = 3; ga.fault = mb->fault; ga.sync = mb->epoch; ga.lut_math = mb->test_bits;
    }
    const GemvPlan p = gemv_plan(w, pre, epi);
    const GemvKernel k = gemv_kernel(pre, epi, p);
    if (!p.nw || !k || (np.out && p.grid > NORM_PART_MAX)) return hipErrorInvalidValue;
    ga.wt = w.tiles; ga.ngroups = w.ngroups; ga.nchunks = w.nchunks; ga.M = w.M; ga.gmapF8 = w.gmapF8; ga.K = w.K;
    ga.part_in = (const f64x2 *) np.in; ga.npart = np.n_in; ga.part_out = (f64x2 *) np.out;
    ga.lut_math |= g_lut_math;
    hipLaunchKernelGGL(k, dim3(p.grid), dim3(p.nw * 64), p.lds, st, ga);
    LH_LAUNCH_CHECK();
    return hipSuccess;
}

hipError_t launch_gemv(const QMat &w, int pre, int epi, const uint32_t *qa_A, const float *qa_d,
                       const float *in0, const float *in1, float *y, const float *resid,
                       const uint16_t *T_silu,
                       uint32_t *out_A, float *out_d, hipStream_t st, const NormPart *np, const MailboxIO *mb) {
    if (pre == PREP_NORM_TAG || epi >= EPI_STORE_TAG) return hipErrorInvalidValue;
    GemvArgs ga = {};
    ga.qa_A = qa_A; ga.qa_d = qa_d; ga.in0 = in0; ga.in1 = in1; ga.y = y; ga.resid = resid; ga.T_silu = T_silu; ga.out_A = out_A; ga.out_d = out_d;
    return launch_gemv_plan(w, pre, epi, np, mb, ga, st);
}

bool gemv_pick_applies(const QMat &w) { return gemv_plan(w, PREP_NORM, EPI_STORE_PICK).nw != 0; }
hipError_t launch_gemv_pick(const QMat &w, const float *in0, const float *in1, float *y, const uint16_t *T_silu, hipStream_t st,
                            const NormPart *np, const PickIO &pick) {
    GemvArgs ga = {};
    ga.in0 = in0; ga.in1 = in1; ga.y = y; ga.T_silu = T_silu; ga.pick = pick;
    return launch_gemv_plan(w, PREP_NORM, EPI_STORE_PICK, np, nullptr, ga, st);
}
bool gemv_silu_half_applies(const QMat &w) {
    static const bool off = getenv("LLAMAHIP_NO_W13_HALF") != nullptr;
    static const bool force = getenv("LLAMAHIP_W13_HALF") && atoi(getenv("LLAMAHIP_W13_HALF")) == 1;
    static const int ncu = [] { int dev = 0; hipDeviceProp_t p; return (hipGetDevice(&dev) == hipSuccess && hipGetDeviceProperties(&p, dev) == hipSuccess && p.multiProcessorCount > 0) ? p.multiProcessorCount : 256; }();
    if (off || !gemv_plan(w, PREP_NORM, EPI_SILU_QAH).nw) return false;
    if (force) return true;
    const double nb = w.ngroups / 8.0;
    const double r_blocks = std::ceil(nb / ncu) / (nb / ncu), r_halves = std::ceil(2.0 * nb / ncu) / (2.0 * nb / ncu);
    return r_halves < r_blocks - 0.02;
}
hipError_t launch_gemv_silu_half(const QMat &w, const float *in0, const float *in1, const uint16_t *T_silu, uint32_t *out_A, float *out_d, hipStream_t st,
                                 const NormPart *np, uint64_t *amax_t, uint32_t *epoch, int layer, uint32_t *fault) {
    static const int fault_test = (getenv("LLAMAHIP_HANDOFF_FAULT_TEST") && atoi(getenv("LLAMAHIP_HANDOFF_FAULT_TEST")) == 6) ? 0x1000 : 0;
    GemvArgs ga = {};
    ga.in0 = in0; ga.in1 = in1; ga.T_silu = T_silu; ga.out_A = out_A; ga.out_d = out_d;
    ga.sync = epoch; ga.sync_epoch = layer; ga.lut_math = fault_test; ga.fault = fault; ga.out_t = amax_t;
    return launch_gemv_plan(w, PREP_NORM, EPI_SILU_QAH, np, nullptr, ga, st);
}

hipError_t launch_attn_short(const float *qr, const float *Kc, const float *Vc, float *sc, float *merged,
                             uint32_t *qa_A, float *qa_d, int n_past, int N, int d, int H, int n_ctx, int nth,
                             const uint16_t *T_exp, hipStream_t st, int chunk, const SeqSet *set, int set_keys, long merged_stride) {
    const int dh = d / H, T = set ? (set_keys > 0 && set_keys < n_ctx ? set_keys : n_ctx) : n_past + N;
    const float kq_scale = 1.0f / sqrtf((float) d / (float) H);
    const int Kp = (d + 255) / 256 * 256;
    hipLaunchKernelGGL(k_decn_scores, dim3(H, (T + DEC_TS - 1) / DEC_TS, N), dim3(256), 0, st, qr, d, dh, Kc, sc, n_ctx, kq_scale, n_past, set);
    LH_LAUNCH_CHECK();
    const int nt = (32 * (nth < 32 ? nth : 32) + 63) / 64 * 64;
    const size_t lds = 32 * sizeof(double) + ((size_t) n_ctx + (size_t) nth * 32 + 16) * sizeof(float);
    hipLaunchKernelGGL(k_dec_pv_blk<true>, dim3(H, dh / 32, N), dim3(nt), lds, st, sc, Vc, d, dh, n_ctx, nth, merged, qa_A, qa_d, T_exp,
                       (const int32_t *) nullptr, n_past, (long) Kp / 4, (long) Kp / 32, g_lut_math, chunk, set, merged_stride > 0 ? merged_stride : (long) d);
    LH_LAUNCH_CHECK();
    return hipSuccess;
}


bool xcd_selftest(int H, int Y, hipStream_t st) {
    uint32_t *d_out = nullptr;
    const size_t n = (size_t) H * Y;
    if (hipMalloc((void **) &d_out, n * 4) != hipSuccess) return false;
    std::vector<uint32_t> out(n, 0xffffffffu);
    bool ok = hipMemsetAsync(d_out, 0xff, n * 4, st) == hipSuccess;
    if (ok) {
        hipLaunchKernelGGL(k_xcd_selftest, dim3(H, Y), dim3(64), 0, st, d_out);
        ok = hipGetLastError() == hipSuccess && hipMemcpyAsync(out.data(), d_out, n * 4, hipMemcpyDeviceToHost, st) == hipSuccess &&
             hipStreamSynchronize(st) == hipSuccess;
    }
    if (ok) {
        for (int h = 0; h < H; h++)
            for (int y = 0; y < Y; y++)
                if (out[h + (size_t) H * y] != out[h] || out[h] > 15u) ok = false;
    }
    if (ok) {
        std::fill(out.begin(), out.end(), 0xffffffffu);
        ok = hipMemsetAsync(d_out, 0xff, n * 4, st) == hipSuccess;
        if (ok) {
            hipLaunchKernelGGL(k_xcd_selftest, dim3((unsigned) n), dim3(256), 0, st, d_out);
            ok = hipGetLastError() == hipSuccess && hipMemcpyAsync(out.data(), d_out, n * 4, hipMemcpyDeviceToHost, st) == hipSuccess &&
                 hipStreamSynchronize(st) == hipSuccess;
        }
        for (size_t b = 0; ok && b < n; b++)
            if (out[b] != out[b & 7] || out[b] > 15u) ok = false;
    }
    (void) hipFree(d_out);
    return ok;
}

static const int g_pv_fault_test = (getenv("LLAMAHIP_HANDOFF_FAULT_TEST") && atoi(getenv("LLAMAHIP_HANDOFF_FAULT_TEST")) == 4) ? 0x1000 : 0;
static bool th_split_ok(int nth, int split, int cpw) { return split >= 1 && cpw >= 1 && (split - 1) * cpw < nth; }
static_assert(DEC_ATTN_TS == DEC_TS, "dec_attn_plan.h mirrors the keys per score workgroup");

hipError_t launch_dec_attn(const float *qkv, int d, int H, int n_ctx, int nth, const double *tab, float *Kc, float *Vc,
                           float *sc, float *part, float *merged, uint32_t *qa_A, float *qa_d,
                           const uint16_t *T_exp, const int32_t *state, hipStream_t st, uint32_t *xsync, uint32_t *fault, bool long_ctx,
                           uint64_t *xpart, const uint32_t *epoch, int layer, const DecAttnForce *force) {
    const int dh = d / H;
    const float kq_scale = 1.0f / sqrtf((float) d / (float) H);
    (void) part;
    const DecAttnPlan p = dec_attn_plan(d, H, n_ctx, nth, long_ctx, xsync && fault, xpart && epoch && fault, force);
    if (p.kernel < 0) return hipErrorInvalidValue;
    if (p.kernel == DEC_ATTN_X) {
        const AttnXArgs aa = { qkv, d, dh, tab, Kc, Vc, sc, n_ctx, nth, kq_scale, merged, qa_A, qa_d, T_exp, state, xsync, fault, g_lut_math, nullptr, nullptr, nullptr, 0 };
        hipLaunchKernelGGL(k_dec_attn_x, dim3(p.gx, p.gy), dim3(p.threads), p.lds, st, aa);
        LH_LAUNCH_CHECK();
        return hipSuccess;
    }
    const int nsl = (n_ctx + DEC_TS - 1) / DEC_TS;
    hipLaunchKernelGGL(k_dec_scores, dim3(H, nsl), dim3(256), 2 * dh * sizeof(float), st, qkv, d, dh, tab, Kc, Vc, sc, n_ctx, kq_scale, state);
    LH_LAUNCH_CHECK();
    if (p.kernel == DEC_ATTN_PV_DMA)
        hipLaunchKernelGGL(k_dec_pv_dma, dim3(p.gx), dim3(p.threads), p.lds, st, sc, Vc, d, n_ctx, nth, p.NS, merged, qa_A, qa_d, T_exp, state, g_lut_math | g_pv_fault_test, H, p.split, xpart, epoch, layer, fault);
    else if (p.kernel == DEC_ATTN_PV_STREAM)
        hipLaunchKernelGGL(k_dec_pv_stream<4>, dim3(p.gx), dim3(p.threads), p.lds, st, sc, Vc, d, dh, n_ctx, nth, p.SR, merged, qa_A, qa_d, T_exp, state, g_lut_math | g_pv_fault_test, H, p.split, xpart, epoch, layer, fault);
    else
        hipLaunchKernelGGL(k_dec_pv_blk<false>, dim3(p.gx, p.gy), dim3(p.threads), p.lds, st, sc, Vc, d, dh, n_ctx, nth, merged, qa_A, qa_d, T_exp, state, 0, 0L, 0L, g_lut_math, 0, (const SeqSet *) nullptr, 0L);
    LH_LAUNCH_CHECK();
    return hipSuccess;
}

using QkvAttnKernel = void (*)(const GemvArgs, const AttnXArgs, const int, const int);
template <int PRE>
static QkvAttnKernel qkv_attn_kernel_at(int depth, int pg) {
    if (depth == 8 && pg == 1) return k_qkv_attn<PRE, 8, 1>;
    if (depth == 10 && pg == 2) return k_qkv_attn<PRE, 10, 2>;
    if (depth == 4 && pg == 2) return k_qkv_attn<PRE, 4, 2>;
    return nullptr;
}
static QkvAttnKernel qkv_attn_kernel(int pre, int depth, int pg) {
    return pre == PREP_NORM ? qkv_attn_kernel_at<PREP_NORM>(depth, pg) : pre == PREP_NORMP ? qkv_attn_kernel_at<PREP_NORMP>(depth, pg)
         : pre == PREP_NORM_TAG ? qkv_attn_kernel_at<PREP_NORM_TAG>(depth, pg) : nullptr;
}
static GemvPlan qkv_attn_plan(const QMat &w) {
    GemvPlan p = gemv_plan(w, PREP_NORM, EPI_STORE);
    if (!qkv_attn_instance(p.nw, p.ring, p.depth, p.pg) || !qkv_attn_kernel(PREP_NORM, p.depth, p.pg)) p.nw = 0;
    return p;
}
bool qkv_attn_applies(const QMat &w, int d, int H, int nth) {
    static const bool off = getenv("LLAMAHIP_NO_QKV_ATTN") != nullptr;
    if (off || !qkv_attn_shape_ok(d, H, nth, w.M, w.K, w.ngroups, w.gmapF8)) return false;
    return qkv_attn_plan(w).nw != 0;
}
bool qkv_attn_launch_query(const QMat &w, const NormPart &npp, int d, int H, int n_ctx, int nth, long out[5]) {
    const GemvPlan p = qkv_attn_plan(w);
    NormPart np = npp;
    int pre = PREP_NORM;
    norm_mode_resolve(&pre, &np);
    if (!p.nw || !qkv_attn_kernel(pre, p.depth, p.pg)) return false;
    const QkvAttnGeom g = qkv_attn_geom(p.grid, p.lds, d, H, n_ctx, nth);
    out[0] = pre; out[1] = p.depth; out[2] = p.pg; out[3] = g.grid; out[4] = (long) g.lds;
    return true;
}
hipError_t launch_qkv_attn(const QMat &w, const float *x, const float *norm_w, const NormPart &npp, uint64_t *qkv2, uint64_t *sc2, uint32_t *epoch, int layer,
                           int d, int H, int n_ctx, int nth, const double *tab, float *Kc, float *Vc, float *merged, uint32_t *qa_A, float *qa_d,
                           const uint16_t *T_silu, const uint16_t *T_exp, const int32_t *state, uint32_t *fault, hipStream_t st,
                           const MailboxIO *mb) {
    const uint64_t *x_t = mb ? mb->in_t : nullptr;
    const GemvPlan p = qkv_attn_plan(w);
    NormPart np = npp;
    int pre = x_t ? PREP_NORM_TAG : PREP_NORM;
    norm_mode_resolve(&pre, &np);
    const QkvAttnKernel k = qkv_attn_kernel(pre, p.depth, p.pg);
    if (!p.nw || !k) return hipErrorInvalidValue;
    const int dh = d / H, gridA = p.grid;
    const float kq_scale = 1.0f / sqrtf((float) d / (float) H);
    const QkvAttnGeom g = qkv_attn_geom(p.grid, p.lds, d, H, n_ctx, nth);
    static const int fault_test = (getenv("LLAMAHIP_HANDOFF_FAULT_TEST") && atoi(getenv("LLAMAHIP_HANDOFF_FAULT_TEST")) < 2) ? 0x1000 : 0;
    GemvArgs ga = { w.tiles, w.ngroups, w.nchunks, w.M, w.gmapF8, nullptr, nullptr, x, norm_w, w.K, (float *) qkv2, nullptr, T_silu, nullptr, nullptr,
                    (const f64x2 *) np.in, np.n_in, nullptr, epoch, 0, layer, g_lut_math | fault_test, fault };
    if (x_t) { ga.in_t = x_t; ga.slot_in = 0; ga.pos_w = mb->pos_w; ga.patience = 3; ga.lut_math |= mb->test_bits; }
    const AttnXArgs aa = { nullptr, d, dh, tab, Kc, Vc, nullptr, n_ctx, nth, kq_scale, merged, qa_A, qa_d, T_exp, state, nullptr, fault, g_lut_math | fault_test,
                           qkv2, sc2, epoch, layer };
    hipLaunchKernelGGL(k, dim3(g.grid), dim3(256), g.lds, st, ga, aa, gridA, H);
    LH_LAUNCH_CHECK();
    return hipSuccess;
}

__global__ void k_bump_epoch(uint32_t *epoch) { epoch[0] = next_epoch(epoch[0]); }
hipError_t launch_bump_epoch(uint32_t *epoch, hipStream_t st) {
    hipLaunchKernelGGL(k_bump_epoch, dim3(1), dim3(1), 0, st, epoch);
    LH_LAUNCH_CHECK();
    return hipSuccess;
}


__device__ __forceinline__ void
topk_keys_row(const float *__restrict__ logits, int V, const int32_t *__restrict__ window, int n_window, double scale, double repeat_penalty,
              unsigned long long *__restrict__ keys, unsigned long long *__restrict__ gmax, uint32_t *__restrict__ badw) {
    __shared__ uint32_t seen[1024];
    const int tid = threadIdx.x, i = blockIdx.x * 1024 + tid;
    seen[tid] = 0u;
    __syncthreads();
    if (tid < n_window) { const int id = window[tid]; if (id >= 0 && id < V) atomicOr(&seen[id >> 5], 1u << (id & 31)); }
    __syncthreads();
    unsigned long long kk = 0ull;
    if (i < V) {
        const float lf = logits[i];
        double sc;
        if ((seen[i >> 5] >> (i & 31)) & 1u) sc = lf < 0.0f ? (double) lf * scale * repeat_penalty : (double) lf * scale / repeat_penalty;
        else sc = (double) lf * scale;
        if (sc != sc) atomicOr(badw, 1u);
        const unsigned long long b = (unsigned long long) __double_as_longlong(sc);
        kk = (b >> 63) ? ~b : (b | 0x8000000000000000ull);
        if (kk == 0ull) kk = 1ull;
    }
    keys[i] = kk;
    unsigned long long best = kk;
    best = dpp_max_u64(best, dpp_u64<DPP_QUAD_XOR1>(best));
    best = dpp_max_u64(best, dpp_u64<DPP_QUAD_XOR2>(best));
    best = dpp_max_u64(best, dpp_u64<DPP_ROW_HALF_MIRROR>(best));
    best = dpp_max_u64(best, dpp_u64<DPP_ROW_MIRROR>(best));
    if ((tid & 15) == 0 && best != 0ull) atomicMax(&gmax[tid >> 4], best);
}

__global__ void __launch_bounds__(1024)
k_topk_keys(const float *__restrict__ logits, int V, const int32_t *__restrict__ window, int n_window, double scale, double repeat_penalty,
            unsigned long long *__restrict__ keys, unsigned long long *__restrict__ gmax, uint32_t *__restrict__ badw) {
    topk_keys_row(logits, V, window, n_window, scale, repeat_penalty, keys, gmax, badw);
}

__device__ __forceinline__ void
topk_select_row(int V, int k, unsigned long long *__restrict__ keys, unsigned long long *__restrict__ gmax, uint32_t *__restrict__ badw,
                double *__restrict__ out_score, int32_t *__restrict__ out_id, int32_t *__restrict__ flags, bool force_host) {
    constexpr int NPT = 32, LCAP = 768;
    constexpr unsigned long long KEY_PZ = 0x8000000000000000ull, KEY_NZ = 0x7fffffffffffffffull;
    __shared__ unsigned long long list_key[LCAP];
    __shared__ int32_t list_id[LCAP];
    __shared__ uint32_t n_list, bad;
    const int tid = threadIdx.x;
    if (tid == 0) { n_list = 0u; bad = badw[0]; }
    unsigned long long key[NPT];
#pragma unroll
    for (int u = 0; u < NPT; u++) key[u] = keys[tid + u * 1024];
    __shared__ unsigned long long s_T;
    if (tid == 0) s_T = 0ull;
    __syncthreads();
    if (tid < 64) {
        const unsigned long long v = gmax[tid];
        int r = 0;
#pragma unroll
        for (int j = 0; j < 64; j++) { const unsigned long long o = gmax[j]; r += (o > v || (o == v && j < tid)) ? 1 : 0; }
        if (r == k - 1) s_T = v;
    }
    __syncthreads();
    const unsigned long long T = s_T == KEY_PZ ? KEY_NZ : s_T;
    if (tid < 64) gmax[tid] = 0ull;
    if (tid == 0) badw[0] = 0u;
    if (T == 0ull || force_host) {
        if (tid == 0) { flags[0] = 0; flags[1] = 0; }
        return;
    }
    {
        uint32_t cnt = 0;
        unsigned long long pass[NPT];
#pragma unroll
        for (int u = 0; u < NPT; u++) { pass[u] = __ballot(key[u] >= T); cnt += (uint32_t) __popcll(pass[u]); }
        uint32_t base = 0;
        if ((tid & 63) == 0 && cnt) base = atomicAdd(&n_list, cnt);
        base = (uint32_t) __builtin_amdgcn_readfirstlane((int) base);
        const unsigned long long lt = (1ull << (tid & 63)) - 1ull;
#pragma unroll
        for (int u = 0; u < NPT; u++) {
            if (key[u] >= T) {
                const uint32_t at = base + (uint32_t) __popcll(pass[u] & lt);
                if (at < (uint32_t) LCAP) { list_key[at] = key[u] == KEY_NZ ? KEY_PZ : key[u]; list_id[at] = tid + u * 1024; }
            }
            base += (uint32_t) __popcll(pass[u]);
        }
    }
    __syncthreads();
    const int n = (int) (n_list < (uint32_t) LCAP ? n_list : (uint32_t) LCAP);
    if (n_list > (uint32_t) LCAP) bad = 1u;
    if (tid < n) {
        const unsigned long long mine = list_key[tid];
        const int my_id = list_id[tid];
        int rank = 0;
        bool dup = false;
        int j = 0;
        for (; j + 8 <= n; j += 8) {
            unsigned long long o[8]; int oid[8];
#pragma unroll
            for (int u = 0; u < 8; u++) { o[u] = list_key[j + u]; oid[u] = list_id[j + u]; }
#pragma unroll
            for (int u = 0; u < 8; u++) {
                dup = dup || (j + u != tid && o[u] == mine);
                rank += (o[u] > mine || (o[u] == mine && oid[u] < my_id)) ? 1 : 0;
            }
        }
        for (; j < n; j++) {
            const unsigned long long o = list_key[j];
            dup = dup || (j != tid && o == mine);
            rank += (o > mine || (o == mine && list_id[j] < my_id)) ? 1 : 0;
        }
        if (rank <= k && dup) bad = 1u;
        if (rank < k) {
            const unsigned long long own = mine == KEY_PZ ? keys[my_id] : mine;
            const unsigned long long b = (own >> 63) ? (own & 0x7fffffffffffffffull) : ~own;
            out_score[rank] = __longlong_as_double((long long) b);
            out_id[rank] = my_id;
        }
    }
    __syncthreads();
    if (tid == 0) { flags[0] = (bad == 0u && n >= k) ? 1 : 0; flags[1] = n; }
}

__global__ void __launch_bounds__(1024)
k_topk_select(int V, int k, unsigned long long *__restrict__ keys, unsigned long long *__restrict__ gmax, uint32_t *__restrict__ badw,
              double *__restrict__ out_score, int32_t *__restrict__ out_id, int32_t *__restrict__ flags) {
    topk_select_row(V, k, keys, gmax, badw, out_score, out_id, flags, false);
}

__global__ void __launch_bounds__(1024)
k_topk_keys_rows(const float *__restrict__ logits, int V, const int32_t *__restrict__ windows, const int32_t *__restrict__ n_last, double scale,
                 double repeat_penalty, char *__restrict__ ws) {
    const int r = blockIdx.y;
    unsigned long long *keys = (unsigned long long *) (ws + (size_t) r * TOPK_WS_BYTES), *gmax = keys + 32768;
    const int nw = n_last[r];
    topk_keys_row(logits + (size_t) r * V, V, windows + (size_t) r * 1024, nw < 0 ? 0 : (nw > 1024 ? 1024 : nw), scale, repeat_penalty,
                  keys, gmax, (uint32_t *) (gmax + 64));
}

__global__ void __launch_bounds__(1024)
k_topk_keys_slide(const float *__restrict__ logits, int V, const int32_t *__restrict__ ids, int n_last, double scale, double repeat_penalty,
                  char *__restrict__ ws) {
    const int r = blockIdx.y;
    unsigned long long *keys = (unsigned long long *) (ws + (size_t) r * TOPK_WS_BYTES), *gmax = keys + 32768;
    topk_keys_row(logits + (size_t) r * V, V, ids + r, n_last, scale, repeat_penalty, keys, gmax, (uint32_t *) (gmax + 64));
}

__global__ void __launch_bounds__(1024)
k_topk_keys_slide_set(const float *__restrict__ logits, int V, const int32_t *__restrict__ ids, const int32_t *__restrict__ row_off,
                      const int32_t *__restrict__ row_n_last, double scale, double repeat_penalty, char *__restrict__ ws) {
    const int r = blockIdx.y;
    unsigned long long *keys = (unsigned long long *) (ws + (size_t) r * TOPK_WS_BYTES), *gmax = keys + 32768;
    const int nw = row_n_last[r];
    topk_keys_row(logits + (size_t) r * V, V, ids + row_off[r], nw < 0 || nw > 1024 ? 0 : nw, scale, repeat_penalty, keys, gmax,
                  (uint32_t *) (gmax + 64));
}

__global__ void __launch_bounds__(1024)
k_topk_select_rows(int V, int k, const int32_t *__restrict__ n_last, char *__restrict__ ws, TopkOut *__restrict__ out) {
    const int r = blockIdx.x;
    unsigned long long *keys = (unsigned long long *) (ws + (size_t) r * TOPK_WS_BYTES), *gmax = keys + 32768;
    const int nw = n_last ? n_last[r] : 0;
    topk_select_row(V, k, keys, gmax, (uint32_t *) (gmax + 64), out[r].sc, out[r].id, out[r].fl, nw < 0 || nw > 1024);
}

__global__ void __launch_bounds__(1024)
k_topk_spill(const float *__restrict__ logits, int V, const TopkOut *__restrict__ out, float *__restrict__ spill) {
    const int r = blockIdx.y;
    if (out[r].fl[0] != 0) return;
    const float *src = logits + (size_t) r * V;
    float *dst = spill + (size_t) r * V;
    const int i0 = blockIdx.x * 4096 + threadIdx.x;
#pragma unroll
    for (int u = 0; u < 4; u++) { const int i = i0 + u * 1024; if (i < V) dst[i] = src[i]; }
}

hipError_t launch_topk_rows(const float *logits, int R, int V, const int32_t *windows, const int32_t *n_last, double scale, double repeat_penalty,
                            int k, TopkOut *out, float *spill, hipStream_t st, void *ws) {
    if (R < 1 || V < 1 || V > 32768 || k < 1 || k > 64 || !ws || !out) return hipErrorInvalidValue;
    hipLaunchKernelGGL(k_topk_keys_rows, dim3((V + 1023) / 1024, R), dim3(1024), 0, st, logits, V, windows, n_last, scale, repeat_penalty, (char *) ws);
    LH_LAUNCH_CHECK();
    hipLaunchKernelGGL(k_topk_select_rows, dim3(R), dim3(1024), 0, st, V, k, n_last, (char *) ws, out);
    LH_LAUNCH_CHECK();
    if (spill) {
        hipLaunchKernelGGL(k_topk_spill, dim3((V + 4095) / 4096, R), dim3(1024), 0, st, logits, V, out, spill);
        LH_LAUNCH_CHECK();
    }
    return hipSuccess;
}

hipError_t launch_topk_slide(const float *logits, int R, int V, const int32_t *ids, int n_last, double scale, double repeat_penalty, int k,
                             TopkOut *out, hipStream_t st, void *ws) {
    if (R < 1 || V < 1 || V > 32768 || k < 1 || k > 64 || n_last < 0 || n_last > 1024 || !ws || !out || !logits || (!ids && n_last > 0)) return hipErrorInvalidValue;
    hipLaunchKernelGGL(k_topk_keys_slide, dim3((V + 1023) / 1024, R), dim3(1024), 0, st, logits, V, ids, n_last, scale, repeat_penalty, (char *) ws);
    LH_LAUNCH_CHECK();
    hipLaunchKernelGGL(k_topk_select_rows, dim3(R), dim3(1024), 0, st, V, k, (const int32_t *) nullptr, (char *) ws, out);
    LH_LAUNCH_CHECK();
    return hipSuccess;
}

hipError_t launch_topk_slide_set(const float *logits, int R, int V, const int32_t *ids, const int32_t *row_off, const int32_t *row_n_last, double scale,
                                 double repeat_penalty, int k, TopkOut *out, hipStream_t st, void *ws) {
    if (R < 1 || R > 16 || V < 1 || V > 32768 || k < 1 || k > 64 || !ws || !out || !logits || !row_off || !row_n_last) return hipErrorInvalidValue;
    hipLaunchKernelGGL(k_topk_keys_slide_set, dim3((V + 1023) / 1024, R), dim3(1024), 0, st, logits, V, ids, row_off, row_n_last, scale, repeat_penalty, (char *) ws);
    LH_LAUNCH_CHECK();
    hipLaunchKernelGGL(k_topk_select_rows, dim3(R), dim3(1024), 0, st, V, k, row_n_last, (char *) ws, out);
    LH_LAUNCH_CHECK();
    return hipSuccess;
}

hipError_t launch_topk_candidates(const float *logits, int V, const int32_t *window, int n_window, double scale, double repeat_penalty, int k,
                                  double *out_score, int32_t *out_id, int32_t *flags, hipStream_t st, void *ws) {
    if (V > 32768 || k < 1 || k > 64 || n_window > 1024) return hipErrorInvalidValue;
    if (!ws) return hipErrorInvalidValue;
    unsigned long long *keys = (unsigned long long *) ws, *gmax = keys + 32768;
    uint32_t *badw = (uint32_t *) (gmax + 64);
    hipLaunchKernelGGL(k_topk_keys, dim3((V + 1023) / 1024), dim3(1024), 0, st, logits, V, window, n_window, scale, repeat_penalty, keys, gmax, badw);
    LH_LAUNCH_CHECK();
    hipLaunchKernelGGL(k_topk_select, dim3(1), dim3(1024), 0, st, V, k, keys, gmax, badw, out_score, out_id, flags);
    LH_LAUNCH_CHECK();
    return hipSuccess;
}

hipError_t launch_argmax(const float *logits, int V, int32_t *out, int out_idx, int32_t *next_token, int32_t *state, hipStream_t st, uint64_t *token_mb) {
    hipLaunchKernelGGL(k_argmax, dim3(1), dim3(1024), 0, st, logits, V, out, out_idx, next_token, state, token_mb);
    LH_LAUNCH_CHECK();
    return hipSuccess;
}


hipError_t launch_argmax_set(const float *logits, int V, const SeqSet *set, int n, hipStream_t st) {
    hipLaunchKernelGGL(k_argmax_set, dim3(n), dim3(1024), 0, st, logits, V, set);
    LH_LAUNCH_CHECK();
    return hipSuccess;
}
hipError_t launch_advance_set(const SeqSet *set, int n, hipStream_t st) {
    hipLaunchKernelGGL(k_advance_set, dim3(1), dim3(64), 0, st, set, n);
    LH_LAUNCH_CHECK();
    return hipSuccess;
}
hipError_t launch_advance(int32_t *state, hipStream_t st) {
    hipLaunchKernelGGL(k_advance, dim3(1), dim3(64), 0, st, state);
    LH_LAUNCH_CHECK();
    return hipSuccess;
}


hipError_t init_attrs_prep();
hipError_t init_attrs_prompt_attn();
hipError_t init_attrs_rows_attn();
hipError_t init_attrs_decode();
hipError_t init_kernel_attrs() {
    hipError_t e;
    if ((e = init_attrs_prep()) != hipSuccess) return e;
    if ((e = init_attrs_decode()) != hipSuccess) return e;
    if ((e = init_attrs_gemv_set()) != hipSuccess) return e;
    if ((e = init_attrs_rows_attn()) != hipSuccess) return e;
    if ((e = init_attrs_dense()) != hipSuccess) return e;
    return init_attrs_prompt_attn();
}

hipError_t init_attrs_decode() {
    const int cap = 160 * 1024;
    auto raise = [](const void *kernel) { return kernel ? hipFuncSetAttribute(kernel, hipFuncAttributeMaxDynamicSharedMemorySize, cap) : hipSuccess; };
    hipError_t e;
    for (int pre = PRE_QA; pre <= PREP_NORM_TAG; pre++)
        for (int depth = 4; depth <= 22; depth += 2)
            for (int pg : { 1, 2, 4, 12 }) {
                for (int epi = EPI_STORE; epi <= EPI_SILU_QAH; epi++)
                    for (int ring = 0; ring < 2; ring++)
                        if ((e = raise((const void *) gemv_kernel(pre, epi, GemvPlan{ 4, pg, depth, ring != 0, 0, 0 }))) != hipSuccess) return e;
                if ((e = raise((const void *) qkv_attn_kernel(pre, depth, pg))) != hipSuccess) return e;
            }
    for (const void *kernel : { (const void *) k_dec_pv_blk<false>, (const void *) k_dec_pv_blk<true>, (const void *) k_dec_pv_stream<4>, (const void *) k_dec_pv_dma, (const void *) k_dec_attn_x })
        if ((e = raise(kernel)) != hipSuccess) return e;
    return hipSuccess;
}

}
```

llama.swift_amd/csrc/kcommon.hip.h:

```cpp
#pragma once
#include <hip/hip_runtime.h>
#include <hip/hip_fp16.h>
#include <stdint.h>
#include <stdio.h>
#include <stdlib.h>

#include <algorithm>
#include <vector>

#include "llamahip_internal.h"

namespace lh {

typedef uint32_t u32x4 __attribute__((ext_vector_type(4)));
typedef float    f32x4 __attribute__((ext_vector_type(4)));
typedef float    f32x2 __attribute__((ext_vector_type(2)));
typedef double   f64x2 __attribute__((ext_vector_type(2)));

#define LH_LAUNCH_CHECK() do { hipError_t e_ = hipGetLastError(); if (e_ != hipSuccess) return e_; } while (0)


__device__ __forceinline__ uint16_t f2h_bits(float f) {
    return __half_as_ushort(__float2half_rn(f));
}
__device__ __forceinline__ float h2f_bits(uint16_t h) {
    return __half2float(__ushort_as_half(h));
}

__device__ __forceinline__ uint16_t silu_math_bits(uint16_t h) {
    const float f = h2f_bits(h);
    return f2h_bits((float) ((double) f / (1.0 + exp((double) -f))));
}
__device__ __forceinline__ uint16_t exp_math_bits(uint16_t h) {
    return f2h_bits((float) exp((double) h2f_bits(h)));
}

__device__ __forceinline__ void store_tagged_agent(uint64_t *p, uint32_t bits, uint32_t tag) {
    __hip_atomic_store(p, (uint64_t) bits | ((uint64_t) tag << 32), __ATOMIC_RELAXED, __HIP_MEMORY_SCOPE_AGENT);
}
__device__ __forceinline__ bool poll_give_up(int &spins, int limit, uint32_t *fault) {
    if (++spins > limit) { __hip_atomic_store(fault, 1u, __ATOMIC_RELAXED, __HIP_MEMORY_SCOPE_SYSTEM); return true; }
    return (spins & 1023) == 0 && __hip_atomic_load(fault, __ATOMIC_RELAXED, __HIP_MEMORY_SCOPE_SYSTEM) != 0u;
}
__device__ __forceinline__ void store_tagged_sys(uint64_t *p, uint32_t bits, uint32_t tag) {
    __hip_atomic_store(p, (uint64_t) bits | ((uint64_t) tag << 32), __ATOMIC_RELAXED, __HIP_MEMORY_SCOPE_SYSTEM);
}
__device__ __forceinline__ uint64_t load_granule_sys(const uint64_t *p) {
    return __hip_atomic_load(p, __ATOMIC_RELAXED, __HIP_MEMORY_SCOPE_SYSTEM);
}
#ifndef LH_WATCH
#define LH_WATCH 4
#endif
__device__ __forceinline__ uint32_t make_tag(uint32_t epoch, int slot) { return (epoch << 8) | (uint32_t) slot; }
__device__ __forceinline__ uint32_t next_epoch(uint32_t e) { e += 1u; if ((e & 0xFFFFFFu) == 0u) e += 1u; return e; }

template <int Q>
__device__ __forceinline__ float quad_bcast(float v) {
    return __builtin_bit_cast(float, __builtin_amdgcn_mov_dpp(__builtin_bit_cast(int, v), Q | (Q << 2) | (Q << 4) | (Q << 6), 0xF, 0xF, true));
}

__device__ __forceinline__ double shfl_xor_d(double v, int m) {
    int lo = __double2loint(v), hi = __double2hiint(v);
    lo = __shfl_xor(lo, m);
    hi = __shfl_xor(hi, m);
    return __hiloint2double(hi, lo);
}

template <int CTRL>
__device__ __forceinline__ double dpp_d(double v) {
    const int lo = __builtin_amdgcn_mov_dpp(__double2loint(v), CTRL, 0xF, 0xF, true);
    const int hi = __builtin_amdgcn_mov_dpp(__double2hiint(v), CTRL, 0xF, 0xF, true);
    return __hiloint2double(hi, lo);
}
template <int CTRL>
__device__ __forceinline__ float dpp_f(float v) {
    return __builtin_bit_cast(float, __builtin_amdgcn_mov_dpp(__builtin_bit_cast(int, v), CTRL, 0xF, 0xF, true));
}
constexpr int DPP_QUAD_XOR1 = 0xB1;
constexpr int DPP_QUAD_XOR2 = 0x4E;
constexpr int DPP_ROW_HALF_MIRROR = 0x141;
constexpr int DPP_ROW_MIRROR = 0x140;

__device__ __forceinline__ double wave_sum_d(double v) {
    v += dpp_d<DPP_QUAD_XOR1>(v);
    v += dpp_d<DPP_QUAD_XOR2>(v);
    v += dpp_d<DPP_ROW_HALF_MIRROR>(v);
    v += dpp_d<DPP_ROW_MIRROR>(v);
    const int lo = __double2loint(v), hi = __double2hiint(v);
    const double r0 = __hiloint2double(__builtin_amdgcn_readlane(hi, 0), __builtin_amdgcn_readlane(lo, 0));
    const double r1 = __hiloint2double(__builtin_amdgcn_readlane(hi, 16), __builtin_amdgcn_readlane(lo, 16));
    const double r2 = __hiloint2double(__builtin_amdgcn_readlane(hi, 32), __builtin_amdgcn_readlane(lo, 32));
    const double r3 = __hiloint2double(__builtin_amdgcn_readlane(hi, 48), __builtin_amdgcn_readlane(lo, 48));
    return (r0 + r1) + (r2 + r3);
}
__device__ __forceinline__ float wave_max_f(float v) {
    v = fmaxf(v, dpp_f<DPP_QUAD_XOR1>(v));
    v = fmaxf(v, dpp_f<DPP_QUAD_XOR2>(v));
    v = fmaxf(v, dpp_f<DPP_ROW_HALF_MIRROR>(v));
    v = fmaxf(v, dpp_f<DPP_ROW_MIRROR>(v));
    const int b = __builtin_bit_cast(int, v);
    const float r0 = __builtin_bit_cast(float, __builtin_amdgcn_readlane(b, 0)), r1 = __builtin_bit_cast(float, __builtin_amdgcn_readlane(b, 16));
    const float r2 = __builtin_bit_cast(float, __builtin_amdgcn_readlane(b, 32)), r3 = __builtin_bit_cast(float, __builtin_amdgcn_readlane(b, 48));
    return fmaxf(fmaxf(r0, r1), fmaxf(r2, r3));
}

__device__ __forceinline__ float tree32_to_lane0(float s) {
    s += dpp_f<0x108>(s);
    s += __shfl_xor(s, 16);
    s += dpp_f<0x104>(s);
    s += dpp_f<DPP_QUAD_XOR1>(s);
    s += dpp_f<DPP_QUAD_XOR2>(s);
    return s;
}

__device__ __forceinline__ float max_lanes_0_31(float v) {
    v = fmaxf(v, dpp_f<DPP_QUAD_XOR1>(v));
    v = fmaxf(v, dpp_f<DPP_QUAD_XOR2>(v));
    v = fmaxf(v, dpp_f<DPP_ROW_HALF_MIRROR>(v));
    v = fmaxf(v, dpp_f<DPP_ROW_MIRROR>(v));
    const int b = __builtin_bit_cast(int, v);
    return fmaxf(__builtin_bit_cast(float, __builtin_amdgcn_readlane(b, 0)), __builtin_bit_cast(float, __builtin_amdgcn_readlane(b, 16)));
}

static __device__ double block_sum_d(double v, double *red, int phase = 0) {
    v = wave_sum_d(v);
    const int w = threadIdx.x >> 6, nw = (blockDim.x + 63) >> 6;
    double *r = red + (phase & 1) * 16;
    if ((threadIdx.x & 63) == 0) r[w] = v;
    __syncthreads();
    double s = 0.0;
    for (int i = 0; i < nw; i++) s += r[i];
    return s;
}
static __device__ void block_sum_d2(double &a, double &b, double *red, int phase = 0) {
    a = wave_sum_d(a);
    b = wave_sum_d(b);
    const int w = threadIdx.x >> 6, nw = (blockDim.x + 63) >> 6;
    double *r = red + (phase & 1) * 16;
    if ((threadIdx.x & 63) == 0) { r[2 * w] = a; r[2 * w + 1] = b; }
    __syncthreads();
    double sa = 0.0, sb = 0.0;
    for (int i = 0; i < nw; i++) { sa += r[2 * i]; sb += r[2 * i + 1]; }
    a = sa; b = sb;
}
static __device__ float block_max_f(float v, double *red, int phase = 0) {
    v = wave_max_f(v);
    const int w = threadIdx.x >> 6, nw = (blockDim.x + 63) >> 6;
    float *r = (float *) (red + (phase & 1) * 16);
    if ((threadIdx.x & 63) == 0) r[w] = v;
    __syncthreads();
    float s = r[0];
    for (int i = 1; i < nw; i++) s = fmaxf(s, r[i]);
    return s;
}

__device__ __forceinline__ float quant_block(const float *v, int parity, uint32_t *chain , uint8_t *raw ) {
    float amax = 0.0f;
#pragma unroll
    for (int l = 0; l < 32; l++) amax = fmaxf(amax, fabsf(v[l]));
    const float d = amax / 7.0f;
    const float id = (amax != 0.0f) ? 7.0f / amax : 0.0f;
    uint32_t q[32];
#pragma unroll
    for (int l = 0; l < 32; l++) q[l] = (uint32_t) ((int) __builtin_rintf(v[l] * id) + 8);
#pragma unroll
    for (int k = 0; k < 8; k++) {
        const uint32_t e0 = (q[2 * k] - 8) & 0xF, e1 = (q[2 * k + 1] - 8) & 0xF;
        const uint32_t e2 = (q[16 + 2 * k] - 8) & 0xF, e3 = (q[17 + 2 * k] - 8) & 0xF;
        chain[k] = (e0 | (e1 << 8) | (e2 << 16) | (e3 << 24)) << (4 * parity);
    }
    if (raw) {
#pragma unroll
        for (int j = 0; j < 16; j++) raw[j] = (uint8_t) (q[2 * j] | (q[2 * j + 1] << 4));
    }
    return d;
}

__device__ __forceinline__ int pidx(int i) { return i + (i >> 5); }

constexpr int LB_DEFAULT = 8;

#ifdef LH_DEFINE_PHASE_PROBE
__device__ unsigned long long *g_phase_probe = nullptr;
#endif
#if LH_PHASE_PROBE
#if LH_PHASE_PROBE == 3
#define LH_STAMP(IDX) do { probe_t[IDX] = __builtin_readcyclecounter(); } while (0)
#define LH_STAMP2(IDX) do { } while (0)
#elif LH_PHASE_PROBE == 2
#define LH_STAMP(IDX) do { if (probe_e && (IDX) < 2) probe_e[IDX] = __builtin_readcyclecounter(); } while (0)
#define LH_STAMP2(IDX) do { if (probe_e) probe_e[IDX] = __builtin_readcyclecounter(); } while (0)
#else
#define LH_STAMP(IDX) do { if (probe_e) probe_e[IDX] = __builtin_readcyclecounter(); } while (0)
#define LH_STAMP2(IDX) do { } while (0)
#endif
#else
#define LH_STAMP(IDX) do { } while (0)
#define LH_STAMP2(IDX) do { } while (0)
#endif


template <int MODE, int LB = LB_DEFAULT>
static __device__ void make_y(float *ybuf, double *red, const float *__restrict__ in0, const float *__restrict__ in1,
                       int K, const uint16_t *__restrict__ T_silu) {
    const int tid = threadIdx.x, nt = blockDim.x;
    const int n4 = K >> 2;
    const f32x4 *a4 = (const f32x4 *) in0;
    const f32x4 *b4 = (const f32x4 *) in1;
    if (MODE == PREP_PLAIN) {
        for (int base = tid; base < n4; base += nt * LB) {
            f32x4 v[LB];
#pragma unroll
            for (int u = 0; u < LB; u++) v[u] = a4[min(base + u * nt, n4 - 1)];
#pragma unroll
            for (int u = 0; u < LB; u++) {
                const int g = base + u * nt;
                if (g < n4) { float *o = ybuf + pidx(4 * g); o[0] = v[u].x; o[1] = v[u].y; o[2] = v[u].z; o[3] = v[u].w; }
            }
        }
    } else if (MODE == PREP_SILU_MUL) {
        for (int base = tid; base < n4; base += nt * LB) {
            f32x4 ga[LB], up[LB];
#pragma unroll
            for (int u = 0; u < LB; u++) { const int g = min(base + u * nt, n4 - 1); ga[u] = a4[g]; up[u] = b4[g]; }
            uint16_t lut[LB][4];
#pragma unroll
            for (int u = 0; u < LB; u++) {
                lut[u][0] = T_silu[f2h_bits(ga[u].x)]; lut[u][1] = T_silu[f2h_bits(ga[u].y)];
                lut[u][2] = T_silu[f2h_bits(ga[u].z)]; lut[u][3] = T_silu[f2h_bits(ga[u].w)];
            }
#pragma unroll
            for (int u = 0; u < LB; u++) {
                const int g = base + u * nt;
                if (g < n4) {
                    float *o = ybuf + pidx(4 * g);
                    o[0] = h2f_bits(lut[u][0]) * up[u].x; o[1] = h2f_bits(lut[u][1]) * up[u].y;
                    o[2] = h2f_bits(lut[u][2]) * up[u].z; o[3] = h2f_bits(lut[u][3]) * up[u].w;
                }
            }
        }
    } else {
        double s = 0.0;
        for (int base = tid; base < n4; base += nt * LB) {
            f32x4 v[LB];
#pragma unroll
            for (int u = 0; u < LB; u++) v[u] = a4[min(base + u * nt, n4 - 1)];
#pragma unroll
            for (int u = 0; u < LB; u++) {
                const int g = base + u * nt;
                if (g < n4) {
                    float *o = ybuf + pidx(4 * g);
                    o[0] = v[u].x; o[1] = v[u].y; o[2] = v[u].z; o[3] = v[u].w;
                    s += (double) v[u].x; s += (double) v[u].y; s += (double) v[u].z; s += (double) v[u].w;
                }
            }
        }
        const double mean = block_sum_d(s, red, 0) / (double) K;
        double s2 = 0.0;
        for (int i = tid; i < K; i += nt) {
            const double v = (double) ybuf[pidx(i)] - mean;
            ybuf[pidx(i)] = (float) v;
            s2 += v * v;
        }
        const double sum2 = block_sum_d(s2, red, 1);
        const float scale = (float) (1.0 / sqrt(sum2 / (double) K + (double) 1e-5f));
        for (int base = tid; base < n4; base += nt * LB) {
            f32x4 w[LB];
#pragma unroll
            for (int u = 0; u < LB; u++) w[u] = b4[min(base + u * nt, n4 - 1)];
#pragma unroll
            for (int u = 0; u < LB; u++) {
                const int g = base + u * nt;
                if (g < n4) {
                    float *o = ybuf + pidx(4 * g);
                    o[0] = w[u].x * (o[0] * scale); o[1] = w[u].y * (o[1] * scale);
                    o[2] = w[u].z * (o[2] * scale); o[3] = w[u].w * (o[3] * scale);
                }
            }
        }
    }
    __syncthreads();
}

__device__ __forceinline__ void copy_g2l(uint32_t *dst, const uint32_t *__restrict__ src, int n4) {
    constexpr int LB = LB_DEFAULT;
    const u32x4 *s4 = (const u32x4 *) src;
    u32x4 *d4 = (u32x4 *) dst;
    for (int base = threadIdx.x; base < n4; base += blockDim.x * LB) {
        u32x4 v[LB];
#pragma unroll
        for (int u = 0; u < LB; u++) v[u] = s4[min(base + u * (int) blockDim.x, n4 - 1)];
#pragma unroll
        for (int u = 0; u < LB; u++) { const int g = base + u * (int) blockDim.x; if (g < n4) d4[g] = v[u]; }
    }
}

static __device__ void quantize_y(const float *ybuf, int K, int Kp, uint32_t *A, float *da, uint8_t *raw_out) {
    const int nb = K / 32, nbp = Kp / 32;
    for (int b = threadIdx.x; b < nbp; b += blockDim.x) {
        const int c = b >> 3, j = b & 7;
        const float *v = ybuf + b * 33;
        float d = 0.0f, id = 0.0f;
        if (b < nb) {
            float amax = 0.0f;
#pragma unroll 8
            for (int l = 0; l < 32; l++) amax = fmaxf(amax, fabsf(v[l]));
            d = amax / 7.0f;
            id = (amax != 0.0f) ? 7.0f / amax : 0.0f;
        }
        uint8_t *o = raw_out ? raw_out + (size_t) b * 20 : nullptr;
        if (o && b < nb) {
            const uint32_t bits = __builtin_bit_cast(uint32_t, d);
            o[0] = bits & 0xFF; o[1] = (bits >> 8) & 0xFF; o[2] = (bits >> 16) & 0xFF; o[3] = bits >> 24;
        }
#pragma unroll
        for (int k = 0; k < 8; k++) {
            uint32_t dw = 0;
            if (b < nb) {
                const int q0 = (int) __builtin_rintf(v[2 * k] * id), q1 = (int) __builtin_rintf(v[2 * k + 1] * id);
                const int q2 = (int) __builtin_rintf(v[16 + 2 * k] * id), q3 = (int) __builtin_rintf(v[17 + 2 * k] * id);
                dw = ((uint32_t) (q0 & 0xF) | ((uint32_t) (q1 & 0xF) << 8) | ((uint32_t) (q2 & 0xF) << 16) | ((uint32_t) (q3 & 0xF) << 24)) << (4 * (j & 1));
                if (o) {
                    o[4 + k] = (uint8_t) ((q0 + 8) | ((q1 + 8) << 4));
                    o[12 + k] = (uint8_t) ((q2 + 8) | ((q3 + 8) << 4));
                }
            }
            A[(c * 8 + k) * 8 + j] = dw;
        }
        da[b] = d;
    }
}

#define LH_FMAC8_DPP(ACC, PLO, PHI, Q01, Q23, Q45, Q67)                                            \
    asm("s_nop 1\n\t"                                                                              \
        "v_fmac_f32_dpp %0, %1, %3 quad_perm:[0,0,0,0] row_mask:0xf bank_mask:0xf\n\t"             \
        "v_fmac_f32_dpp %0, %1, %4 quad_perm:[1,1,1,1] row_mask:0xf bank_mask:0xf\n\t"             \
        "v_fmac_f32_dpp %0, %1, %5 quad_perm:[2,2,2,2] row_mask:0xf bank_mask:0xf\n\t"             \
        "v_fmac_f32_dpp %0, %1, %6 quad_perm:[3,3,3,3] row_mask:0xf bank_mask:0xf\n\t"             \
        "v_fmac_f32_dpp %0, %2, %7 quad_perm:[0,0,0,0] row_mask:0xf bank_mask:0xf\n\t"             \
        "v_fmac_f32_dpp %0, %2, %8 quad_perm:[1,1,1,1] row_mask:0xf bank_mask:0xf\n\t"             \
        "v_fmac_f32_dpp %0, %2, %9 quad_perm:[2,2,2,2] row_mask:0xf bank_mask:0xf\n\t"             \
        "v_fmac_f32_dpp %0, %2, %10 quad_perm:[3,3,3,3] row_mask:0xf bank_mask:0xf"                 \
        : "+v"(ACC)                                                                                \
        : "v"(PLO), "v"(PHI), "v"((Q01).x), "v"((Q01).y), "v"((Q23).x), "v"((Q23).y),              \
          "v"((Q45).x), "v"((Q45).y), "v"((Q67).x), "v"((Q67).y))

#define LH_STEP(J, WD, AD, DA)                                                                     \
    {                                                                                              \
        const float sc_ = quad_bcast<((J) & 3)>((J) < 4 ? sw.x : sw.y) * (DA);                     \
         \
         \
         \
        const int p_ = __builtin_amdgcn_sdot8((int) (WD), (int) (AD), 0x4B400000, true);           \
        acc = fmaf(sc_, __builtin_bit_cast(float, p_) - 12582912.0f, acc);                         \
    }

__device__ __forceinline__ float fold8(float acc) {
    acc += dpp_f<0x104>(acc);
    acc += dpp_f<DPP_QUAD_XOR2>(acc);
    acc += dpp_f<DPP_QUAD_XOR1>(acc);
    return acc;
}

static __device__ __forceinline__ void pv_soft_max(const float *__restrict__ row, float *p, int T, int tid, int nt, double *red,
                                                   const uint16_t *__restrict__ T_exp, int lut_math) {
    float mx = -INFINITY;
    for (int t = tid; t < T; t += nt) { const float v = row[t]; p[t] = v; mx = fmaxf(mx, v); }
    mx = block_max_f(mx, red, 0);
    double sum = 0.0;
    for (int t = tid; t < T; t += nt) {
        const uint16_t xh = f2h_bits(p[t] - mx);
        const float e = h2f_bits((lut_math & 2) ? exp_math_bits(xh) : T_exp[xh]);
        p[t] = e;
        sum += (double) e;
    }
    sum = block_sum_d(sum, red, 1);
    const float inv = (float) (1.0 / sum);
    for (int t = tid; t < T; t += nt) p[t] *= inv;
}
static __device__ __forceinline__ void pv_store_block(const float *part, int nth, int tid, int col, int h, int dh, int cb,
                                                      float *__restrict__ merged, uint32_t *__restrict__ qa_A, float *__restrict__ qa_d) {
    if (tid < 32) {
        float s = part[tid];
        for (int th = 1; th < nth; th++) s += part[th * 32 + tid];
        if (merged) merged[col] = s;
        float amax = fabsf(s);
        amax = max_lanes_0_31(amax);
        const float dd = amax / 7.0f;
        const float id = (amax != 0.0f) ? 7.0f / amax : 0.0f;
        const uint32_t nib = (uint32_t) ((int) __builtin_rintf(s * id)) & 0xF;
        const int kk = tid & 7;
        const uint32_t e0 = __shfl(nib, 2 * kk), e1 = __shfl(nib, 2 * kk + 1);
        const uint32_t e2 = __shfl(nib, 16 + 2 * kk), e3 = __shfl(nib, 17 + 2 * kk);
        const int b = h * (dh / 32) + cb, cc = b >> 3, j = b & 7;
        if (tid < 8) qa_A[(cc * 8 + kk) * 8 + j] = (e0 | (e1 << 8) | (e2 << 16) | (e3 << 24)) << (4 * (j & 1));
        if (tid == 0) qa_d[b] = dd;
    }
}


}
```

Measured before the change: 767.9 tokens/s.

## Split GEMV kernel arguments into aligned hot and cold blocks

Reorganizes the mat-vec (and fused QKV/attention) kernel arguments into a 64-byte-aligned hot struct that fits two scalar-cache lines, plus a cold struct passed only to variants that need tagged handoff or pick state. It also removes several redundant bound clamps and derived counts, and passes the wave count explicitly instead of reading blockDim. The aim is to cut kernarg scalar loads and per-kernel prologue latency in the many small decode launches. The change touches many launch sites and kernel signatures, so mismatched argument packing is a correctness risk.

```diff
diff --git a/llama.swift_amd/csrc/decode.hip b/llama.swift_amd/csrc/decode.hip
--- a/llama.swift_amd/csrc/decode.hip
+++ b/llama.swift_amd/csrc/decode.hip
@@ -28,39 +28,55 @@
 }
 
 
-struct GemvArgs {
-    const uint8_t *wt; int ngroups, nchunks, M, gmapF8;
-    const uint32_t *qa_A; const float *qa_d;
-    const float *in0, *in1; int K;
+struct alignas(64) GemvHot {
+    const uint8_t *wt;
+    const void *op0, *op1;
     float *y; const float *resid;
     const uint16_t *T_silu;
     uint32_t *out_A; float *out_d;
-    const f64x2 *part_in; int npart; f64x2 *part_out;
-    uint32_t *sync; int sync_blocks, sync_epoch;
+    const f64x2 *part_in; f64x2 *part_out;
+    const uint32_t *epoch;
+    uint64_t *amax_t;
+    int ngroups, nchunks, M, gmapF8, K, npart;
     int lut_math;
+    uint16_t layer, nw;
+};
+static_assert(sizeof(GemvHot) <= 128 && alignof(GemvHot) == 64, "the hot block of a decode mat-vec is two scalar-cache lines");
+struct GemvCold {
     uint32_t *fault;
     const uint64_t *in_t;   int slot_in;
     const uint64_t *resid_t; int slot_resid;
     uint64_t *out_t;        int slot_out;
     const int32_t *pos_w;
     PickIO pick;
+    int nwg;
     int patience;
 };
+constexpr bool gemv_needs_cold(int pre, int epi) { return pre == PREP_NORM_TAG || epi == EPI_RESID_TAG || epi == EPI_STORE_PICK || epi == EPI_SILU_QAH; }
+
+__device__ __forceinline__ void gemv_entry(const GemvHot &gh) {
+    asm volatile("" :: "s"(gh.wt), "s"(gh.op0), "s"(gh.op1), "s"(gh.y), "s"(gh.resid), "s"(gh.T_silu), "s"(gh.out_A), "s"(gh.out_d),
+                       "s"(gh.part_in), "s"(gh.part_out), "s"(gh.epoch), "s"(gh.amax_t),
+                       "s"(gh.ngroups), "s"(gh.nchunks), "s"(gh.M), "s"(gh.gmapF8), "s"(gh.K), "s"(gh.npart), "s"(gh.lut_math),
+                       "s"((uint32_t) gh.layer | ((uint32_t) gh.nw << 16)));
+}
+
 template <int PRE, int EPI, int D, bool RING, int PG>
-__device__ __forceinline__ void gemv_body(const GemvArgs &ga, const int blk, const int nw, double *smem_d) {
-    const uint8_t *__restrict__ wt = ga.wt;
-    const int ngroups = ga.ngroups, nchunks = ga.nchunks, M = ga.M, gmapF8 = ga.gmapF8, K = ga.K, npart = ga.npart;
-    const uint32_t *__restrict__ qa_A = ga.qa_A; const float *__restrict__ qa_d = ga.qa_d;
-    const float *__restrict__ in0 = ga.in0; const float *__restrict__ in1 = ga.in1;
-    float *__restrict__ y = ga.y; const float *__restrict__ resid = ga.resid;
-    const uint16_t *__restrict__ T_silu = ga.T_silu;
-    uint32_t *__restrict__ out_A = ga.out_A; float *__restrict__ out_d = ga.out_d;
-    const f64x2 *__restrict__ part_in = ga.part_in; f64x2 *__restrict__ part_out = ga.part_out;
+__device__ __forceinline__ void gemv_body(const GemvHot &gh, const GemvCold &gc, const int blk, const int nw, double *smem_d) {
+    const uint8_t *__restrict__ wt = gh.wt;
+    const int ngroups = gh.ngroups, nchunks = gh.nchunks, M = gh.M, gmapF8 = gh.gmapF8, K = gh.K, npart = gh.npart, lut_math = gh.lut_math;
+    const uint32_t *__restrict__ qa_A = (const uint32_t *) gh.op0; const float *__restrict__ qa_d = (const float *) gh.op1;
+    const float *__restrict__ in0 = (const float *) gh.op0; const float *__restrict__ in1 = (const float *) gh.op1;
+    float *__restrict__ y = gh.y; const float *__restrict__ resid = gh.resid;
+    const uint16_t *__restrict__ T_silu = gh.T_silu;
+    uint32_t *__restrict__ out_A = gh.out_A; float *__restrict__ out_d = gh.out_d;
+    const f64x2 *__restrict__ part_in = gh.part_in; f64x2 *__restrict__ part_out = gh.part_out;
+    uint64_t *amax_t = gh.amax_t;
     constexpr bool TAGGED = (EPI == EPI_STORE_TAG || PRE == PREP_NORM_TAG || EPI == EPI_RESID_TAG || EPI == EPI_SILU_QAH);
-    const uint32_t epoch_ = TAGGED ? __builtin_nontemporal_load(ga.sync) : 0u;
-    const uint32_t store_tag = make_tag(epoch_, ga.sync_epoch + 1);
-    const uint32_t mb_epoch_ = ((PRE == PREP_NORM_TAG || EPI == EPI_RESID_TAG) && ga.pos_w) ? (uint32_t) __builtin_nontemporal_load(ga.pos_w) + 1u : epoch_;
-    const uint32_t tag_in = make_tag(mb_epoch_, ga.slot_in), tag_resid = make_tag(mb_epoch_, ga.slot_resid), tag_out = make_tag(mb_epoch_, ga.slot_out);
+    const uint32_t epoch_ = TAGGED ? __builtin_nontemporal_load(gh.epoch) : 0u;
+    const uint32_t store_tag = make_tag(epoch_, (int) gh.layer + 1);
+    const uint32_t mb_epoch_ = ((PRE == PREP_NORM_TAG || EPI == EPI_RESID_TAG) && gc.pos_w) ? (uint32_t) __builtin_nontemporal_load(gc.pos_w) + 1u : epoch_;
+    const uint32_t tag_in = make_tag(mb_epoch_, gc.slot_in), tag_resid = make_tag(mb_epoch_, gc.slot_resid), tag_out = make_tag(mb_epoch_, gc.slot_out);
     uint32_t *ldsA = (uint32_t *) smem_d;
     constexpr int PADC = (LH_GEMV_PAD && RING) ? D : 0;
     float *ldsD = (float *) (ldsA + (nchunks + PADC) * 64);
@@ -111,15 +127,13 @@
     const int nh = K >> 4;
     constexpr int PNP = (PRE == PREP_NORMP) ? 8 : 1;
     f64x2 pp[PNP];
-    const int npl = (npart + 63) >> 6;
     float resid_v = 0.0f;
     uint64_t resid_g = 0;
     auto phase1 = [&]() {
     if ((NORMLIKE || PRE == PREP_PLAIN) && active) {
-        const int ng = (nh + nt - 1) / nt;
 #pragma unroll
         for (int u = 0; u < MAXH; u++) {
-            if (u < ng && (tid & ~63) + u * nt < nh) {
+            if ((tid & ~63) + u * nt < nh) {
                 const int hi = min(tid + u * nt, nh - 1);
 #pragma unroll
                 for (int v = 0; v < 4; v++) {
@@ -133,25 +147,24 @@
         }
         if (PRE == PREP_NORMP && wave == 0) {
 #pragma unroll
-            for (int u = 0; u < PNP; u++) if (u < npl) pp[u] = part_in[min(lane + u * 64, npart - 1)];
-        }
-    }
-    if ((EPI == EPI_RESID || (EPI == EPI_RESID_TAG && !ga.resid_t)) && active) {
+            for (int u = 0; u < PNP; u++) if (lane + u * 64 < npart) pp[u] = part_in[lane + u * 64];
+        }
+    }
+    if ((EPI == EPI_RESID || (EPI == EPI_RESID_TAG && !gc.resid_t)) && active) {
         int lg0 = g;
         if (gmapF8) { const int b8 = g >> 3, w8 = g & 7; lg0 = w8 < 4 ? b8 * 4 + w8 : gmapF8 + b8 * 4 + (w8 - 4); }
         resid_v = resid[min(lg0 * 8 + (lane >> 3), M - 1)];
     }
-    if (EPI == EPI_RESID_TAG && ga.resid_t && active && (lane & 7) == 0) {
+    if (EPI == EPI_RESID_TAG && gc.resid_t && active && (lane & 7) == 0) {
         int lg0 = g;
         if (gmapF8) { const int b8 = g >> 3, w8 = g & 7; lg0 = w8 < 4 ? b8 * 4 + w8 : gmapF8 + b8 * 4 + (w8 - 4); }
-        resid_g = load_granule_sys(ga.resid_t + min(lg0 * 8 + (lane >> 3), M - 1));
+        resid_g = load_granule_sys(gc.resid_t + min(lg0 * 8 + (lane >> 3), M - 1));
     }
     if (PRE == PRE_QA && active) {
-        const int nqa = (nchunks * 16 + nt - 1) / nt, nqd = (nchunks * 2 + nt - 1) / nt;
-#pragma unroll
-        for (int u = 0; u < MAXQA; u++) if (u < nqa) qg[u] = ((const u32x4 *) qa_A)[min(tid + u * nt, nchunks * 16 - 1)];
-#pragma unroll
-        for (int u = 0; u < MAXQD; u++) if (u < nqd) qh[u] = ((const u32x4 *) qa_d)[min(tid + u * nt, nchunks * 2 - 1)];
+#pragma unroll
+        for (int u = 0; u < MAXQA; u++) if (tid + u * nt < nchunks * 16) qg[u] = ((const u32x4 *) qa_A)[tid + u * nt];
+#pragma unroll
+        for (int u = 0; u < MAXQD; u++) if (tid + u * nt < nchunks * 2) qh[u] = ((const u32x4 *) qa_d)[tid + u * nt];
     }
     };
     phase1();
@@ -163,8 +176,8 @@
     __builtin_amdgcn_sched_barrier(0);
 
     if (NORMTAG) {
-        const uint64_t *__restrict__ xt = ga.in_t;
-        const int give_up = (ga.lut_math & 0x1000) ? (1 << 8) : ((1 << 20) << ga.patience);
+        const uint64_t *__restrict__ xt = gc.in_t;
+        const int give_up = (lut_math & 0x1000) ? (1 << 8) : ((1 << 20) << gc.patience);
         if (wave == 0) {
             int spins = 0;
             for (;;) {
@@ -172,7 +185,7 @@
                 if (lane < LH_WATCH) ok = (uint32_t) (load_granule_sys(xt + ((2 * lane + 1) * K / (2 * LH_WATCH))) >> 32) == tag_in;
                 if (__all(ok)) break;
                 __builtin_amdgcn_s_sleep(8);
-                if (++spins > (give_up >> 2) || ((spins & 255) == 0 && __hip_atomic_load(ga.fault, __ATOMIC_RELAXED, __HIP_MEMORY_SCOPE_SYSTEM) != 0u)) break;
+                if (++spins > (give_up >> 2) || ((spins & 255) == 0 && __hip_atomic_load(gc.fault, __ATOMIC_RELAXED, __HIP_MEMORY_SCOPE_SYSTEM) != 0u)) break;
             }
         }
         __syncthreads();
@@ -191,7 +204,7 @@
                     }
                     if (ok) break;
                     __builtin_amdgcn_s_sleep(1);
-                    if (poll_give_up(spins, give_up, ga.fault)) break;
+                    if (poll_give_up(spins, give_up, gc.fault)) break;
                 }
 #pragma unroll
                 for (int v = 0; v < 4; v++)
@@ -223,7 +236,7 @@
                 if (wave == 0) {
 #pragma unroll
                     for (int u = 0; u < PNP; u++)
-                        if (u < npl && lane + u * 64 < npart) { S1 += pp[u].x; S2 += pp[u].y; }
+                        if (lane + u * 64 < npart) { S1 += pp[u].x; S2 += pp[u].y; }
                     S1 = wave_sum_d(S1);
                     S2 = wave_sum_d(S2);
                     if (lane == 0) { red[0] = S1; red[1] = S2; }
@@ -241,7 +254,7 @@
                             S2 = __builtin_fma(x0, x0, S2); S2 = __builtin_fma(x1, x1, S2); S2 = __builtin_fma(x2, x2, S2); S2 = __builtin_fma(x3, x3, S2);
                         }
                     }
-                block_sum_d2(S1, S2, red, 0);
+                block_sum_d2(S1, S2, red, 0, nw);
             }
             const double mean = S1 / (double) K;
             double sum2 = __builtin_fma(-mean, S1, S2);
@@ -259,7 +272,7 @@
                         if (!fast) { s2 += v0 * v0; s2 += v1 * v1; s2 += v2 * v2; s2 += v3 * v3; }
                     }
                 }
-            if (!fast) sum2 = block_sum_d(s2, red, 1);
+            if (!fast) sum2 = block_sum_d(s2, red, 1, nw);
             const float scale = (float) (1.0 / sqrt(sum2 / (double) K + (double) 1e-5f));
             LH_STAMP2(3);
 #pragma unroll
@@ -395,14 +408,14 @@
         if (wave == 0 && valid) {
             const int i = lane & 15;
             const uint16_t gh = f2h_bits(gu[i]);
-            const float act = h2f_bits((ga.lut_math & 1) ? silu_math_bits(gh) : T_silu[gh]) * gu[16 + i];
+            const float act = h2f_bits((lut_math & 1) ? silu_math_bits(gh) : T_silu[gh]) * gu[16 + i];
             float amax = wave_max_f(lane < 16 ? fabsf(act) : 0.0f);
-            uint64_t *at = (uint64_t *) ga.out_t;
+            uint64_t *at = amax_t;
             const int hb = qah_block * 2 + qah_half;
             float other = 0.0f;
             if (lane == 0) {
-                store_tagged(at + hb, amax, store_tag ^ ((ga.lut_math & 0x1000) ? 1u : 0u));
-                other = poll_tagged(at + (hb ^ 1), store_tag, ga.fault, (ga.lut_math & 0x1000) != 0);
+                store_tagged(at + hb, amax, store_tag ^ ((lut_math & 0x1000) ? 1u : 0u));
+                other = poll_tagged(at + (hb ^ 1), store_tag, gc.fault, (lut_math & 0x1000) != 0);
             }
             other = __builtin_bit_cast(float, __builtin_amdgcn_readfirstlane(__builtin_bit_cast(int, other)));
             amax = fmaxf(amax, other);
@@ -424,7 +437,7 @@
         if (wave == 0) {
             const int i = lane & 31;
             const uint16_t gh = f2h_bits(gu[i]);
-            const float act = h2f_bits((ga.lut_math & 1) ? silu_math_bits(gh) : T_silu[gh]) * gu[32 + i];
+            const float act = h2f_bits((lut_math & 1) ? silu_math_bits(gh) : T_silu[gh]) * gu[32 + i];
             float amax = fabsf(act);
             amax = max_lanes_0_31(amax);
             const float dd = amax / 7.0f;
@@ -446,16 +459,16 @@
         if (EPI == EPI_RESID) acc = acc + resid_v;
         if (EPI == EPI_RESID_TAG) {
             float rv = resid_v;
-            if (ga.resid_t) {
+            if (gc.resid_t) {
                 rv = __builtin_bit_cast(float, (uint32_t) resid_g);
                 if (live && (uint32_t) (resid_g >> 32) != tag_resid) {
                     int spins = 0;
                     uint64_t gq;
                     for (;;) {
-                        gq = load_granule_sys(ga.resid_t + m);
+                        gq = load_granule_sys(gc.resid_t + m);
                         if ((uint32_t) (gq >> 32) == tag_resid) break;
                         __builtin_amdgcn_s_sleep(4);
-                        if (poll_give_up(spins, (ga.lut_math & 0x1000) ? (1 << 8) : ((1 << 20) << ga.patience), ga.fault)) break;
+                        if (poll_give_up(spins, (lut_math & 0x1000) ? (1 << 8) : ((1 << 20) << gc.patience), gc.fault)) break;
                     }
                     rv = __builtin_bit_cast(float, (uint32_t) gq);
                 }
@@ -483,19 +496,19 @@
             if (tid == 0) {
                 unsigned long long k2 = wk[0];
                 for (int w2_ = 1; w2_ < nw; w2_++) k2 = wk[w2_] > k2 ? wk[w2_] : k2;
-                __hip_atomic_store(ga.pick.key + blk, k2, __ATOMIC_RELAXED, __HIP_MEMORY_SCOPE_AGENT);
+                __hip_atomic_store(gc.pick.key + blk, k2, __ATOMIC_RELAXED, __HIP_MEMORY_SCOPE_AGENT);
                 asm volatile("s_waitcnt vmcnt(0)" ::: "memory");
-                const int nwg = (int) gridDim.x, shard = blk & 7, nsh = (nwg + 7 - shard) / 8, ntop = nwg < 8 ? nwg : 8;
+                const int nwg = gc.nwg, shard = blk & 7, nsh = (nwg + 7 - shard) / 8, ntop = nwg < 8 ? nwg : 8;
                 int lastwg = 0;
-                if (atomicAdd(ga.pick.count + shard * 16, 1u) == (uint32_t) (nsh - 1))
-                    lastwg = atomicAdd(ga.pick.count + 128, 1u) == (uint32_t) (ntop - 1);
+                if (atomicAdd(gc.pick.count + shard * 16, 1u) == (uint32_t) (nsh - 1))
+                    lastwg = atomicAdd(gc.pick.count + 128, 1u) == (uint32_t) (ntop - 1);
                 wk[15] = (unsigned long long) lastwg;
             }
             __syncthreads();
             if (wk[15] != 0ull) {
                 unsigned long long best = 0ull;
-                for (int i = tid; i < (int) gridDim.x; i += nw * 64) {
-                    const unsigned long long kv = __hip_atomic_load(ga.pick.key + i, __ATOMIC_RELAXED, __HIP_MEMORY_SCOPE_AGENT);
+                for (int i = tid; i < gc.nwg; i += nw * 64) {
+                    const unsigned long long kv = __hip_atomic_load(gc.pick.key + i, __ATOMIC_RELAXED, __HIP_MEMORY_SCOPE_AGENT);
                     best = kv > best ? kv : best;
                 }
 #pragma unroll
@@ -511,21 +524,21 @@
                     unsigned long long fin = wk[0];
                     for (int w2_ = 1; w2_ < nw; w2_++) fin = wk[w2_] > fin ? wk[w2_] : fin;
                     const int r = (fin >> 32) == 0ull ? 0 : (int) (0xFFFFFFFFu - (uint32_t) fin);
-                    int32_t *st = ga.pick.state;
-                    ga.pick.out[st[1]] = r;
-                    if (ga.pick.next_token) *ga.pick.next_token = r;
+                    int32_t *st = gc.pick.state;
+                    gc.pick.out[st[1]] = r;
+                    if (gc.pick.next_token) *gc.pick.next_token = r;
                     st[0] += 1; st[1] += 1;
-                    for (int sh = 0; sh < 8; sh++) __hip_atomic_store(ga.pick.count + sh * 16, 0u, __ATOMIC_RELAXED, __HIP_MEMORY_SCOPE_AGENT);
-                    __hip_atomic_store(ga.pick.count + 128, 0u, __ATOMIC_RELAXED, __HIP_MEMORY_SCOPE_AGENT);
-                    wk[14] = (unsigned long long) (r < ga.pick.n_vocab ? r : 0);
+                    for (int sh = 0; sh < 8; sh++) __hip_atomic_store(gc.pick.count + sh * 16, 0u, __ATOMIC_RELAXED, __HIP_MEMORY_SCOPE_AGENT);
+                    __hip_atomic_store(gc.pick.count + 128, 0u, __ATOMIC_RELAXED, __HIP_MEMORY_SCOPE_AGENT);
+                    wk[14] = (unsigned long long) (r < gc.pick.n_vocab ? r : 0);
                 }
                 __syncthreads();
             }
-            if (wk[15] != 0ull && ga.pick.emb) {
+            if (wk[15] != 0ull && gc.pick.emb) {
                 const int tok = (int) wk[14];
                 const int dE = K;
                 __syncthreads();
-                const uint8_t *row = ga.pick.emb + (size_t) tok * (dE / 32) * 20;
+                const uint8_t *row = gc.pick.emb + (size_t) tok * (dE / 32) * 20;
                 double s1 = 0.0, s2 = 0.0;
                 for (int i = tid; i < dE / 2; i += nw * 64) {
                     const int b = i >> 4, j = i & 15;
@@ -534,24 +547,24 @@
                     const float dd = __builtin_bit_cast(float, bits);
                     const uint32_t q = blk_[4 + j];
                     const float v0 = (float) ((int) (q & 0xF) - 8) * dd, v1 = (float) ((int) (q >> 4) - 8) * dd;
-                    ga.pick.x_next[2 * i + 0] = v0;
-                    ga.pick.x_next[2 * i + 1] = v1;
+                    gc.pick.x_next[2 * i + 0] = v0;
+                    gc.pick.x_next[2 * i + 1] = v1;
                     s1 += (double) v0; s1 += (double) v1;
                     s2 += (double) v0 * (double) v0; s2 += (double) v1 * (double) v1;
                 }
-                s1 = block_sum_d(s1, red, 0);
-                s2 = block_sum_d(s2, red, 1);
+                s1 = block_sum_d(s1, red, 0, nw);
+                s2 = block_sum_d(s2, red, 1, nw);
                 if (tid == 0) {
-                    ((f64x2 *) ga.pick.part_next)[0] = f64x2{ s1, s2 };
-                    if (ga.pick.epoch) ga.pick.epoch[0] = next_epoch(ga.pick.epoch[0]);
+                    ((f64x2 *) gc.pick.part_next)[0] = f64x2{ s1, s2 };
+                    if (gc.pick.epoch) gc.pick.epoch[0] = next_epoch(gc.pick.epoch[0]);
                 }
             }
         } else
         if (EPI == EPI_STORE_TAG) {
-            if (live) store_tagged((uint64_t *) y + m, acc, store_tag ^ ((ga.lut_math & 0x1000) ? 1u : 0u));
+            if (live) store_tagged((uint64_t *) y + m, acc, store_tag ^ ((lut_math & 0x1000) ? 1u : 0u));
         } else if (EPI == EPI_RESID_TAG) {
             if (live) {
-                if (ga.out_t) store_tagged_sys(ga.out_t + m, __builtin_bit_cast(uint32_t, acc), tag_out ^ ((ga.lut_math & 0x2000) ? 1u : 0u));
+                if (gc.out_t) store_tagged_sys(gc.out_t + m, __builtin_bit_cast(uint32_t, acc), tag_out ^ ((lut_math & 0x2000) ? 1u : 0u));
                 if (y) y[m] = acc;
             }
         } else
@@ -591,9 +604,18 @@
 
 template <int PRE, int EPI, int D, bool RING, int PG>
 __global__ void __launch_bounds__(EPI == EPI_SILU_QA ? 512 : 256, EPI == EPI_SILU_QA ? 4 : 1)
-k_gemv(const GemvArgs ga) {
+k_gemv(const GemvHot gh) {
     extern __shared__ double smem_d[];
-    gemv_body<PRE, EPI, D, RING, PG>(ga, blockIdx.x, blockDim.x >> 6, smem_d);
+    gemv_entry(gh);
+    const GemvCold none = {};
+    gemv_body<PRE, EPI, D, RING, PG>(gh, none, blockIdx.x, gh.nw, smem_d);
+}
+template <int PRE, int EPI, int D, bool RING, int PG>
+__global__ void __launch_bounds__(EPI == EPI_SILU_QA ? 512 : 256, EPI == EPI_SILU_QA ? 4 : 1)
+k_gemv(const GemvHot gh, const GemvCold gc) {
+    extern __shared__ double smem_d[];
+    gemv_entry(gh);
+    gemv_body<PRE, EPI, D, RING, PG>(gh, gc, blockIdx.x, gh.nw, smem_d);
 }
 
 
@@ -1102,17 +1124,29 @@
 #ifndef LH_ATTN_ABLATE
 #define LH_ATTN_ABLATE 0
 #endif
-struct AttnXArgs {
-    const float *qkv; int d, dh; const double *sincos_tab; float *Kc, *Vc, *sc; int n_ctx, nth; float kq_scale;
-    float *merged; uint32_t *qa_A; float *qa_d; const uint16_t *T_exp; const int32_t *st; uint32_t *sync, *fault; int lut_math;
-    const uint64_t *qkv2; uint64_t *sc2; const uint32_t *epoch; int layer;
+struct alignas(64) AttnHot {
+    const int32_t *st;
+    uint32_t *word;
+    float *Kc, *Vc; const double *sincos_tab;
+    const void *qkv; void *sc;
+    const uint16_t *T_exp; float *merged; uint32_t *qa_A; float *qa_d; uint32_t *fault;
+    int n_ctx; float kq_scale; int lut_math;
+    int gridA;
+    uint16_t d, dh, H, nth, layer;
 };
+static_assert(sizeof(AttnHot) <= 128 && alignof(AttnHot) == 64, "the hot block of a decode attention launch is two scalar-cache lines");
+__device__ __forceinline__ void attn_entry(const AttnHot &aa) {
+    asm volatile("" :: "s"(aa.st), "s"(aa.word), "s"(aa.Kc), "s"(aa.Vc), "s"(aa.sincos_tab), "s"(aa.qkv), "s"(aa.sc), "s"(aa.T_exp),
+                       "s"(aa.merged), "s"(aa.qa_A), "s"(aa.qa_d), "s"(aa.fault), "s"(aa.n_ctx), "s"(aa.kq_scale), "s"(aa.lut_math), "s"(aa.gridA),
+                       "s"((uint32_t) aa.d | ((uint32_t) aa.dh << 16)), "s"((uint32_t) aa.H | ((uint32_t) aa.nth << 16)), "s"((uint32_t) aa.layer));
+}
 template <bool QKV_WAIT>
-__device__ __forceinline__ void attn_x_body(const AttnXArgs &aa, const int h, const int yy, double *smem_d) {
-    const float *__restrict__ qkv = aa.qkv; const int d = aa.d, dh = aa.dh; const double *__restrict__ sincos_tab = aa.sincos_tab;
-    float *__restrict__ Kc = aa.Kc, *__restrict__ Vc = aa.Vc; float *sc = aa.sc; const int n_ctx = aa.n_ctx, nth = aa.nth; const float kq_scale = aa.kq_scale;
+__device__ __forceinline__ void attn_x_body(const AttnHot &aa, const int h, const int yy, double *smem_d) {
+    const float *__restrict__ qkv = (const float *) aa.qkv; const int d = aa.d, dh = aa.dh; const double *__restrict__ sincos_tab = aa.sincos_tab;
+    float *__restrict__ Kc = aa.Kc, *__restrict__ Vc = aa.Vc; float *sc = (float *) aa.sc; const int n_ctx = aa.n_ctx, nth = aa.nth; const float kq_scale = aa.kq_scale;
     float *__restrict__ merged = aa.merged; uint32_t *__restrict__ qa_A = aa.qa_A; float *__restrict__ qa_d = aa.qa_d;
-    const uint16_t *__restrict__ T_exp = aa.T_exp; const int32_t *__restrict__ st = aa.st; uint32_t *sync = aa.sync, *fault = aa.fault; const int lut_math = aa.lut_math;
+    const uint16_t *__restrict__ T_exp = aa.T_exp; const int32_t *__restrict__ st = aa.st; uint32_t *sync = aa.word, *fault = aa.fault; const int lut_math = aa.lut_math;
+    const uint64_t *qkv2 = (const uint64_t *) aa.qkv; uint64_t *sc2 = (uint64_t *) aa.sc;
     const int ncb = dh / 32, tid = threadIdx.x;
 #if LH_PHASE_PROBE == 3
     unsigned long long probe_t[5] = { 0, 0, 0, 0, 0 };
@@ -1127,6 +1161,7 @@
 #endif
     LH_ASTAMP(0);
     const int n_past = st[0];
+    const uint32_t epoch_ = QKV_WAIT ? __builtin_nontemporal_load(aa.word) : 0u;
     uint32_t *cnt = sync + h * 32;
     if (yy >= ncb) {
         const int t0 = (yy - ncb) * DEC_TS;
@@ -1149,12 +1184,12 @@
             }
         };
         const bool nowait = (lut_math & 0x1000) != 0;
-        const uint32_t tag = QKV_WAIT ? (make_tag(aa.epoch[0], aa.layer + 1)) : 0u;
+        const uint32_t tag = make_tag(epoch_, (int) aa.layer + 1);
         if (QKV_WAIT) load_keys();
         if (tid < dh / 2) {
             const int e = 2 * tid;
             const double cs = tab[e], sn = tab[e + 1];
-            const uint64_t *q2 = aa.qkv2 + h * dh, *k2 = q2 + d, *v2 = q2 + 2 * d;
+            const uint64_t *q2 = qkv2 + h * dh, *k2 = q2 + d, *v2 = q2 + 2 * d;
             float gq0, gq1, gk0 = 0.0f, gk1 = 0.0f, gv0 = 0.0f, gv1 = 0.0f;
             if (QKV_WAIT) {
                 uint64_t g_[6] = { 0, 0, 0, 0, 0, 0 };
@@ -1211,7 +1246,7 @@
             }
             s = tree32_to_lane0(s);
             if (l == 0 && t <= n_past) {
-                if (QKV_WAIT) store_tagged(aa.sc2 + (size_t) h * n_ctx + t, s * kq_scale, tag);
+                if (QKV_WAIT) store_tagged(sc2 + (size_t) h * n_ctx + t, s * kq_scale, tag);
                 else sc[(size_t) h * n_ctx + t] = s * kq_scale;
             }
         }
@@ -1262,7 +1297,7 @@
     const float *row = sc + (size_t) h * n_ctx;
     float mx = -INFINITY;
     if (QKV_WAIT) {
-        const uint32_t tag = make_tag(aa.epoch[0], aa.layer + 1);
+        const uint32_t tag = make_tag(epoch_, (int) aa.layer + 1);
         const bool nowait = (lut_math & 0x1000) != 0;
 #if LH_ATTN_ABLATE == 2
         for (int t0 = tid; t0 < T; t0 += nt) p[t0] = 0.0f;
@@ -1277,7 +1312,7 @@
 #pragma unroll
                 for (int i = 0; i < 4; i++) {
                     const int t = t0 + i * nt;
-                    if (t < T) { g_[i] = __hip_atomic_load(aa.sc2 + (size_t) h * n_ctx + t, __ATOMIC_RELAXED, __HIP_MEMORY_SCOPE_AGENT); ok = ok && (uint32_t) (g_[i] >> 32) == tag; }
+                    if (t < T) { g_[i] = __hip_atomic_load(sc2 + (size_t) h * n_ctx + t, __ATOMIC_RELAXED, __HIP_MEMORY_SCOPE_AGENT); ok = ok && (uint32_t) (g_[i] >> 32) == tag; }
                 }
                 if (ok) break;
                 __builtin_amdgcn_s_sleep(1);
@@ -1294,7 +1329,7 @@
 #if LH_ATTN_ABLATE == 1 || LH_ATTN_ABLATE == 2
     if (!QKV_WAIT) {
 #endif
-    mx = block_max_f(mx, red, 0);
+    mx = block_max_f(mx, red, 0, nt / 64);
     double sum = 0.0;
     for (int t = tid; t < T; t += nt) {
         const uint16_t xh = f2h_bits(p[t] - mx);
@@ -1302,7 +1337,7 @@
         p[t] = e;
         sum += (double) e;
     }
-    sum = block_sum_d(sum, red, 1);
+    sum = block_sum_d(sum, red, 1, nt / 64);
     const float inv = (float) (1.0 / sum);
     for (int t = tid; t < T; t += nt) p[t] *= inv;
 #if LH_ATTN_ABLATE == 1 || LH_ATTN_ABLATE == 2
@@ -1370,26 +1405,42 @@
 #undef LH_AFLUSH
 
 __global__ void __launch_bounds__(256)
-k_dec_attn_x(const AttnXArgs aa) {
+k_dec_attn_x(const AttnHot aa) {
     extern __shared__ double smem_d[];
+    attn_entry(aa);
     attn_x_body<false>(aa, blockIdx.x, blockIdx.y, smem_d);
 }
 
+#define LH_QKV_ATTN_OCC __launch_bounds__(256) __attribute__((amdgpu_waves_per_eu(PRE == PREP_NORM ? (PG == 1 ? 3 : 2) : (PG == 1 ? 4 : 3))))
 template <int PRE, int D, int PG>
-__global__ void __launch_bounds__(256) __attribute__((amdgpu_waves_per_eu(PRE == PREP_NORM ? (PG == 1 ? 3 : 2) : (PG == 1 ? 4 : 3))))
-k_qkv_attn(const GemvArgs ga, const AttnXArgs aa, const int gridA, const int H) {
-    extern __shared__ double smem_d[];
+__device__ __forceinline__ void qkv_attn_body(const AttnHot &aa, const GemvHot &gh, const GemvCold &gc, double *smem_d) {
+    attn_entry(aa);
+    gemv_entry(gh);
     const int b = blockIdx.x;
-    if (b < gridA) {
+    if (b < aa.gridA) {
         const int ncb = aa.dh / 32, wph = 3 * ncb;
         const int xcd = b & 7, slot = b >> 3, j = slot / wph, part = slot % wph, mat = part / ncb, sub = part % ncb;
         const int h = xcd + 8 * j;
-        gemv_body<PRE, EPI_STORE_TAG, D, true, PG>(ga, mat * (aa.d / 32) + h * ncb + sub, 4, smem_d);
+        gemv_body<PRE, EPI_STORE_TAG, D, true, PG>(gh, gc, mat * (aa.d / 32) + h * ncb + sub, 4, smem_d);
         return;
     }
-    const int a = b - gridA, h = a % H, y = a / H;
+    const int H = aa.H, a = b - aa.gridA, h = a % H, y = a / H;
     attn_x_body<true>(aa, h, y, smem_d);
 }
+template <int PRE, int D, int PG>
+__global__ void LH_QKV_ATTN_OCC
+k_qkv_attn(const AttnHot aa, const GemvHot gh) {
+    extern __shared__ double smem_d[];
+    const GemvCold none = {};
+    qkv_attn_body<PRE, D, PG>(aa, gh, none, smem_d);
+}
+template <int PRE, int D, int PG>
+__global__ void LH_QKV_ATTN_OCC
+k_qkv_attn(const AttnHot aa, const GemvHot gh, const GemvCold gc) {
+    extern __shared__ double smem_d[];
+    qkv_attn_body<PRE, D, PG>(aa, gh, gc, smem_d);
+}
+#undef LH_QKV_ATTN_OCC
 
 __global__ void k_xcd_selftest(uint32_t *out) {
     if (threadIdx.x == 0) {
@@ -1574,23 +1625,28 @@
     return p;
 }
 
-using GemvKernel = void (*)(const GemvArgs);
+using GemvKernel = const void *;
+template <int PRE, int EPI, int D, bool RING, int PG>
+static GemvKernel gemv_instance() {
+    if constexpr (gemv_needs_cold(PRE, EPI)) return (const void *) (void (*)(const GemvHot, const GemvCold)) k_gemv<PRE, EPI, D, RING, PG>;
+    else return (const void *) (void (*)(const GemvHot)) k_gemv<PRE, EPI, D, RING, PG>;
+}
 template <int PRE, int EPI, int PG>
 static GemvKernel gemv_kernel_at(int depth, bool ring) {
     constexpr bool ALL = EPI != EPI_STORE_PICK && EPI != EPI_SILU_QAH;
     if (!ring) {
-        if constexpr (ALL) if (depth == 16) return k_gemv<PRE, EPI, 16, false, PG>;
+        if constexpr (ALL) if (depth == 16) return gemv_instance<PRE, EPI, 16, false, PG>();
         return nullptr;
     }
-    if (depth == 4) return k_gemv<PRE, EPI, 4, true, PG>;
+    if (depth == 4) return gemv_instance<PRE, EPI, 4, true, PG>();
     if constexpr (EPI != EPI_SILU_QAH) {
-        if (depth == 8) return k_gemv<PRE, EPI, 8, true, PG>;
-        if (depth == 10) return k_gemv<PRE, EPI, 10, true, PG>;
+        if (depth == 8) return gemv_instance<PRE, EPI, 8, true, PG>();
+        if (depth == 10) return gemv_instance<PRE, EPI, 10, true, PG>();
         if constexpr (ALL) {
-            if (depth == 14) return k_gemv<PRE, EPI, 14, true, PG>;
-            if (depth == 16) return k_gemv<PRE, EPI, 16, true, PG>;
-            if (depth == 18) return k_gemv<PRE, EPI, 18, true, PG>;
-            if (depth == 22) return k_gemv<PRE, EPI, 22, true, PG>;
+            if (depth == 14) return gemv_instance<PRE, EPI, 14, true, PG>();
+            if (depth == 16) return gemv_instance<PRE, EPI, 16, true, PG>();
+            if (depth == 18) return gemv_instance<PRE, EPI, 18, true, PG>();
+            if (depth == 22) return gemv_instance<PRE, EPI, 22, true, PG>();
         }
     }
     return nullptr;
@@ -1632,23 +1688,27 @@
     return norm_mode >= 2;
 }
 
-static hipError_t launch_gemv_plan(const QMat &w, int pre, int epi, const NormPart *npp, const MailboxIO *mb, GemvArgs ga, hipStream_t st) {
+static hipError_t launch_gemv_plan(const QMat &w, int pre, int epi, const NormPart *npp, const MailboxIO *mb, GemvHot gh, GemvCold gc, hipStream_t st) {
     NormPart np = npp ? *npp : NormPart();
     norm_mode_resolve(&pre, &np);
     if (mb) {
         if (mb->in_t && (pre == PREP_NORM || pre == PREP_NORMP) && epi == EPI_STORE) pre = PREP_NORM_TAG;
         else if ((mb->resid_t || mb->out_t) && pre == PRE_QA && epi == EPI_RESID) epi = EPI_RESID_TAG;
         else return hipErrorInvalidValue;
-        ga.in_t = mb->in_t; ga.resid_t = mb->resid_t; ga.out_t = mb->out_t;
-        ga.pos_w = mb->pos_w; ga.patience = 3; ga.fault = mb->fault; ga.sync = mb->epoch; ga.lut_math = mb->test_bits;
+        gc.in_t = mb->in_t; gc.resid_t = mb->resid_t; gc.out_t = mb->out_t;
+        gc.pos_w = mb->pos_w; gc.patience = 3; gc.fault = mb->fault; gh.epoch = mb->epoch; gh.lut_math = mb->test_bits;
     }
     const GemvPlan p = gemv_plan(w, pre, epi);
     const GemvKernel k = gemv_kernel(pre, epi, p);
     if (!p.nw || !k || (np.out && p.grid > NORM_PART_MAX)) return hipErrorInvalidValue;
-    ga.wt = w.tiles; ga.ngroups = w.ngroups; ga.nchunks = w.nchunks; ga.M = w.M; ga.gmapF8 = w.gmapF8; ga.K = w.K;
-    ga.part_in = (const f64x2 *) np.in; ga.npart = np.n_in; ga.part_out = (f64x2 *) np.out;
-    ga.lut_math |= g_lut_math;
-    hipLaunchKernelGGL(k, dim3(p.grid), dim3(p.nw * 64), p.lds, st, ga);
+    gh.wt = w.tiles; gh.ngroups = w.ngroups; gh.nchunks = w.nchunks; gh.M = w.M; gh.gmapF8 = w.gmapF8; gh.K = w.K;
+    gh.part_in = (const f64x2 *) np.in; gh.npart = np.n_in; gh.part_out = (f64x2 *) np.out;
+    gh.lut_math |= g_lut_math;
+    gh.nw = (uint16_t) p.nw;
+    gc.nwg = p.grid;
+    void *args[] = { &gh, &gc };
+    const hipError_t le = hipLaunchKernel(k, dim3(p.grid), dim3(p.nw * 64), args, p.lds, st);
+    if (le != hipSuccess) return le;
     LH_LAUNCH_CHECK();
     return hipSuccess;
 }
@@ -1658,17 +1718,19 @@
                        const uint16_t *T_silu,
                        uint32_t *out_A, float *out_d, hipStream_t st, const NormPart *np, const MailboxIO *mb) {
     if (pre == PREP_NORM_TAG || epi >= EPI_STORE_TAG) return hipErrorInvalidValue;
-    GemvArgs ga = {};
-    ga.qa_A = qa_A; ga.qa_d = qa_d; ga.in0 = in0; ga.in1 = in1; ga.y = y; ga.resid = resid; ga.T_silu = T_silu; ga.out_A = out_A; ga.out_d = out_d;
-    return launch_gemv_plan(w, pre, epi, np, mb, ga, st);
+    GemvHot gh = {};
+    if (pre == PRE_QA) { gh.op0 = qa_A; gh.op1 = qa_d; } else { gh.op0 = in0; gh.op1 = in1; }
+    gh.y = y; gh.resid = resid; gh.T_silu = T_silu; gh.out_A = out_A; gh.out_d = out_d;
+    return launch_gemv_plan(w, pre, epi, np, mb, gh, GemvCold{}, st);
 }
 
 bool gemv_pick_applies(const QMat &w) { return gemv_plan(w, PREP_NORM, EPI_STORE_PICK).nw != 0; }
 hipError_t launch_gemv_pick(const QMat &w, const float *in0, const float *in1, float *y, const uint16_t *T_silu, hipStream_t st,
                             const NormPart *np, const PickIO &pick) {
-    GemvArgs ga = {};
-    ga.in0 = in0; ga.in1 = in1; ga.y = y; ga.T_silu = T_silu; ga.pick = pick;
-    return launch_gemv_plan(w, PREP_NORM, EPI_STORE_PICK, np, nullptr, ga, st);
+    GemvHot gh = {};
+    GemvCold gc = {};
+    gh.op0 = in0; gh.op1 = in1; gh.y = y; gh.T_silu = T_silu; gc.pick = pick;
+    return launch_gemv_plan(w, PREP_NORM, EPI_STORE_PICK, np, nullptr, gh, gc, st);
 }
 bool gemv_silu_half_applies(const QMat &w) {
     static const bool off = getenv("LLAMAHIP_NO_W13_HALF") != nullptr;
@@ -1683,10 +1745,11 @@
 hipError_t launch_gemv_silu_half(const QMat &w, const float *in0, const float *in1, const uint16_t *T_silu, uint32_t *out_A, float *out_d, hipStream_t st,
                                  const NormPart *np, uint64_t *amax_t, uint32_t *epoch, int layer, uint32_t *fault) {
     static const int fault_test = (getenv("LLAMAHIP_HANDOFF_FAULT_TEST") && atoi(getenv("LLAMAHIP_HANDOFF_FAULT_TEST")) == 6) ? 0x1000 : 0;
-    GemvArgs ga = {};
-    ga.in0 = in0; ga.in1 = in1; ga.T_silu = T_silu; ga.out_A = out_A; ga.out_d = out_d;
-    ga.sync = epoch; ga.sync_epoch = layer; ga.lut_math = fault_test; ga.fault = fault; ga.out_t = amax_t;
-    return launch_gemv_plan(w, PREP_NORM, EPI_SILU_QAH, np, nullptr, ga, st);
+    GemvHot gh = {};
+    GemvCold gc = {};
+    gh.op0 = in0; gh.op1 = in1; gh.T_silu = T_silu; gh.out_A = out_A; gh.out_d = out_d;
+    gh.epoch = epoch; gh.layer = (uint16_t) layer; gh.lut_math = fault_test; gc.fault = fault; gh.amax_t = amax_t;
+    return launch_gemv_plan(w, PREP_NORM, EPI_SILU_QAH, np, nullptr, gh, gc, st);
 }
 
 hipError_t launch_attn_short(const float *qr, const float *Kc, const float *Vc, float *sc, float *merged,
@@ -1751,7 +1814,10 @@
     const DecAttnPlan p = dec_attn_plan(d, H, n_ctx, nth, long_ctx, xsync && fault, xpart && epoch && fault, force);
     if (p.kernel < 0) return hipErrorInvalidValue;
     if (p.kernel == DEC_ATTN_X) {
-        const AttnXArgs aa = { qkv, d, dh, tab, Kc, Vc, sc, n_ctx, nth, kq_scale, merged, qa_A, qa_d, T_exp, state, xsync, fault, g_lut_math, nullptr, nullptr, nullptr, 0 };
+        AttnHot aa = {};
+        aa.st = state; aa.word = xsync; aa.Kc = Kc; aa.Vc = Vc; aa.sincos_tab = tab; aa.qkv = qkv; aa.sc = sc; aa.T_exp = T_exp;
+        aa.merged = merged; aa.qa_A = qa_A; aa.qa_d = qa_d; aa.fault = fault; aa.n_ctx = n_ctx; aa.kq_scale = kq_scale; aa.lut_math = g_lut_math;
+        aa.d = (uint16_t) d; aa.dh = (uint16_t) dh; aa.H = (uint16_t) H; aa.nth = (uint16_t) nth;
         hipLaunchKernelGGL(k_dec_attn_x, dim3(p.gx, p.gy), dim3(p.threads), p.lds, st, aa);
         LH_LAUNCH_CHECK();
         return hipSuccess;
@@ -1769,12 +1835,17 @@
     return hipSuccess;
 }
 
-using QkvAttnKernel = void (*)(const GemvArgs, const AttnXArgs, const int, const int);
+using QkvAttnKernel = const void *;
+template <int PRE, int D, int PG>
+static QkvAttnKernel qkv_attn_instance_at() {
+    if constexpr (gemv_needs_cold(PRE, EPI_STORE_TAG)) return (const void *) (void (*)(const AttnHot, const GemvHot, const GemvCold)) k_qkv_attn<PRE, D, PG>;
+    else return (const void *) (void (*)(const AttnHot, const GemvHot)) k_qkv_attn<PRE, D, PG>;
+}
 template <int PRE>
 static QkvAttnKernel qkv_attn_kernel_at(int depth, int pg) {
-    if (depth == 8 && pg == 1) return k_qkv_attn<PRE, 8, 1>;
-    if (depth == 10 && pg == 2) return k_qkv_attn<PRE, 10, 2>;
-    if (depth == 4 && pg == 2) return k_qkv_attn<PRE, 4, 2>;
+    if (depth == 8 && pg == 1) return qkv_attn_instance_at<PRE, 8, 1>();
+    if (depth == 10 && pg == 2) return qkv_attn_instance_at<PRE, 10, 2>();
+    if (depth == 4 && pg == 2) return qkv_attn_instance_at<PRE, 4, 2>();
     return nullptr;
 }
 static QkvAttnKernel qkv_attn_kernel(int pre, int depth, int pg) {
@@ -1816,12 +1887,20 @@
     const float kq_scale = 1.0f / sqrtf((float) d / (float) H);
     const QkvAttnGeom g = qkv_attn_geom(p.grid, p.lds, d, H, n_ctx, nth);
     static const int fault_test = (getenv("LLAMAHIP_HANDOFF_FAULT_TEST") && atoi(getenv("LLAMAHIP_HANDOFF_FAULT_TEST")) < 2) ? 0x1000 : 0;
-    GemvArgs ga = { w.tiles, w.ngroups, w.nchunks, w.M, w.gmapF8, nullptr, nullptr, x, norm_w, w.K, (float *) qkv2, nullptr, T_silu, nullptr, nullptr,
-                    (const f64x2 *) np.in, np.n_in, nullptr, epoch, 0, layer, g_lut_math | fault_test, fault };
-    if (x_t) { ga.in_t = x_t; ga.slot_in = 0; ga.pos_w = mb->pos_w; ga.patience = 3; ga.lut_math |= mb->test_bits; }
-    const AttnXArgs aa = { nullptr, d, dh, tab, Kc, Vc, nullptr, n_ctx, nth, kq_scale, merged, qa_A, qa_d, T_exp, state, nullptr, fault, g_lut_math | fault_test,
-                           qkv2, sc2, epoch, layer };
-    hipLaunchKernelGGL(k, dim3(g.grid), dim3(256), g.lds, st, ga, aa, gridA, H);
+    GemvHot gh = {};
+    GemvCold gc = {};
+    gh.wt = w.tiles; gh.ngroups = w.ngroups; gh.nchunks = w.nchunks; gh.M = w.M; gh.gmapF8 = w.gmapF8; gh.K = w.K;
+    gh.op0 = x; gh.op1 = norm_w; gh.y = (float *) qkv2; gh.T_silu = T_silu;
+    gh.part_in = (const f64x2 *) np.in; gh.npart = np.n_in; gh.epoch = epoch; gh.layer = (uint16_t) layer; gh.nw = 4;
+    gh.lut_math = g_lut_math | fault_test; gc.fault = fault;
+    if (x_t) { gc.in_t = x_t; gc.slot_in = 0; gc.pos_w = mb->pos_w; gc.patience = 3; gh.lut_math |= mb->test_bits; }
+    AttnHot aa = {};
+    aa.st = state; aa.word = epoch; aa.Kc = Kc; aa.Vc = Vc; aa.sincos_tab = tab; aa.qkv = qkv2; aa.sc = sc2; aa.T_exp = T_exp;
+    aa.merged = merged; aa.qa_A = qa_A; aa.qa_d = qa_d; aa.fault = fault; aa.n_ctx = n_ctx; aa.kq_scale = kq_scale; aa.lut_math = g_lut_math | fault_test;
+    aa.gridA = gridA; aa.d = (uint16_t) d; aa.dh = (uint16_t) dh; aa.H = (uint16_t) H; aa.nth = (uint16_t) nth; aa.layer = (uint16_t) layer;
+    void *args[] = { &aa, &gh, &gc };
+    const hipError_t le = hipLaunchKernel(k, dim3(g.grid), dim3(256), args, g.lds, st);
+    if (le != hipSuccess) return le;
     LH_LAUNCH_CHECK();
     return hipSuccess;
 }
diff --git a/llama.swift_amd/csrc/kcommon.hip.h b/llama.swift_amd/csrc/kcommon.hip.h
--- a/llama.swift_amd/csrc/kcommon.hip.h
+++ b/llama.swift_amd/csrc/kcommon.hip.h
@@ -122,9 +122,9 @@
     return fmaxf(__builtin_bit_cast(float, __builtin_amdgcn_readlane(b, 0)), __builtin_bit_cast(float, __builtin_amdgcn_readlane(b, 16)));
 }
 
-static __device__ double block_sum_d(double v, double *red, int phase = 0) {
+static __device__ double block_sum_d(double v, double *red, int phase, int nw) {
     v = wave_sum_d(v);
-    const int w = threadIdx.x >> 6, nw = (blockDim.x + 63) >> 6;
+    const int w = threadIdx.x >> 6;
     double *r = red + (phase & 1) * 16;
     if ((threadIdx.x & 63) == 0) r[w] = v;
     __syncthreads();
@@ -132,10 +132,11 @@
     for (int i = 0; i < nw; i++) s += r[i];
     return s;
 }
-static __device__ void block_sum_d2(double &a, double &b, double *red, int phase = 0) {
+static __device__ double block_sum_d(double v, double *red, int phase = 0) { return block_sum_d(v, red, phase, (int) (blockDim.x + 63) >> 6); }
+static __device__ void block_sum_d2(double &a, double &b, double *red, int phase, int nw) {
     a = wave_sum_d(a);
     b = wave_sum_d(b);
-    const int w = threadIdx.x >> 6, nw = (blockDim.x + 63) >> 6;
+    const int w = threadIdx.x >> 6;
     double *r = red + (phase & 1) * 16;
     if ((threadIdx.x & 63) == 0) { r[2 * w] = a; r[2 * w + 1] = b; }
     __syncthreads();
@@ -143,9 +144,10 @@
     for (int i = 0; i < nw; i++) { sa += r[2 * i]; sb += r[2 * i + 1]; }
     a = sa; b = sb;
 }
-static __device__ float block_max_f(float v, double *red, int phase = 0) {
+static __device__ void block_sum_d2(double &a, double &b, double *red, int phase = 0) { block_sum_d2(a, b, red, phase, (int) (blockDim.x + 63) >> 6); }
+static __device__ float block_max_f(float v, double *red, int phase, int nw) {
     v = wave_max_f(v);
-    const int w = threadIdx.x >> 6, nw = (blockDim.x + 63) >> 6;
+    const int w = threadIdx.x >> 6;
     float *r = (float *) (red + (phase & 1) * 16);
     if ((threadIdx.x & 63) == 0) r[w] = v;
     __syncthreads();
@@ -153,6 +155,7 @@
     for (int i = 1; i < nw; i++) s = fmaxf(s, r[i]);
     return s;
 }
+static __device__ float block_max_f(float v, double *red, int phase = 0) { return block_max_f(v, red, phase, (int) (blockDim.x + 63) >> 6); }
 
 __device__ __forceinline__ float quant_block(const float *v, int parity, uint32_t *chain , uint8_t *raw ) {
     float amax = 0.0f;
```

Result: faster. 785.0 tokens/s, median of 6 (+2.2%).
